# zai-org/SCAIL

Hardware: AMD Instinct MI355X
Metric: denoising-step latent tokens/sec (higher is better)
Workload: dtype bf16

## Files before the change

### include/scail_dit.h

```cpp
#ifndef SCAIL_DIT_H
#define SCAIL_DIT_H

#include "scail_hip.h"

#ifdef __cplusplus
extern "C" {
#endif

typedef struct scail_dit_config {
    int32_t hidden_size;
    int32_t num_heads;
    int32_t inner_hidden_size;
    int32_t num_layers;
    int32_t text_dim;
    int32_t clip_dim;
    int32_t time_freq_dim;
    int32_t time_embed_dim;
    float layernorm_epsilon;
} scail_dit_config;

typedef struct scail_dit_layer {
    const scail_bf16* qkv_w; const float* qkv_b;
    const scail_bf16* o_w; const float* o_b;
    const float* qn; const float* kn;
    const scail_bf16* cq_w; const float* cq_b;
    const scail_bf16* co_w; const float* co_b;
    const float* cqn;
    const float* ln_w; const float* ln_b;
    const scail_bf16* w1; const float* b1;
    const scail_bf16* w2; const float* b2;
} scail_dit_layer;

typedef struct scail_dit_weights {
    const scail_bf16* patch_w; const float* patch_b;
    const scail_bf16* pose_w; const float* pose_b;
    const scail_bf16* time0_w; const float* time0_b;
    const scail_bf16* time2_w; const float* time2_b;
    const scail_bf16* adaln_w; const float* adaln_b;
    const float* adaln_tables;
    const float* final_table;
    const scail_bf16* final_w; const float* final_b;
    const scail_dit_layer* layers;
} scail_dit_weights;

typedef struct scail_dit_cond {
    const scail_bf16* k_text;
    const scail_bf16* vt_text;
    const scail_bf16* k_clip;
    const scail_bf16* vt_clip;
    int64_t Lt, Lc, Bc;
} scail_dit_cond;

typedef struct scail_dit scail_dit;

int scail_dit_create(const scail_dit_config* cfg, const scail_dit_weights* w, scail_dit** out);
void scail_dit_destroy(scail_dit* h);

int64_t scail_dit_workspace_bytes(const scail_dit* h, int64_t B, int64_t T, int64_t H, int64_t W);

#define SCAIL_DIT_CFG_PAIR 1u
int scail_dit_step(scail_dit* h, const float* x, const float* timesteps, const scail_dit_cond* cond,
                   const scail_bf16* ref, int64_t n_ref, const scail_bf16* pose, int64_t n_pose,
                   const float* rope_cos, const float* rope_sin, float* out,
                   int64_t B, int64_t T, int64_t H, int64_t W, uint32_t flags, void* workspace, int64_t workspace_bytes, void* stream);

int64_t scail_dit_chars_workspace_bytes(const scail_dit* h, int64_t B, int64_t T, int64_t H, int64_t W, int64_t n_char);
int scail_dit_step_chars(scail_dit* h, const float* x, const float* timesteps, const scail_dit_cond* cond,
                         const scail_bf16* ref, int64_t n_ref, const scail_bf16* pose, int64_t n_pose, int64_t n_char, int64_t pose_frames,
                         const float* rope_cos, const float* rope_sin, float* out,
                         int64_t B, int64_t T, int64_t H, int64_t W, uint32_t flags, void* workspace, int64_t workspace_bytes, void* stream);

int64_t scail_dit_block_workspace_bytes(const scail_dit* h, int64_t B, int64_t Ltok);
int scail_dit_block(scail_dit* h, int64_t layer, scail_bf16* hidden, const float* mod, const scail_dit_cond* cond,
                    const float* rope_cos, const float* rope_sin, int64_t B, int64_t Ltok,
                    void* workspace, int64_t workspace_bytes, void* stream);

#define SCAIL_SP_ALLGATHER 0
#define SCAIL_SP_ULYSSES 1
#define SCAIL_SP_FWD_START 0
#define SCAIL_SP_FWD_WAIT 1
#define SCAIL_SP_BACK_START 2
#define SCAIL_SP_BACK_WAIT 3
typedef int (*scail_sp_exchange_fn)(void* user, int32_t op, int32_t layer, int32_t element, void* stream);
typedef struct scail_dit_sp {
    int32_t ranks;
    int32_t mode;
    scail_bf16* send;
    scail_bf16* recv;
    scail_bf16* ofull;
    scail_bf16* back;
    scail_sp_exchange_fn exchange;
    void* user;
    void* side_stream[2];
} scail_dit_sp;

int64_t scail_dit_sp_workspace_bytes(const scail_dit* h, int32_t mode, int32_t ranks, int64_t B, int64_t T, int64_t H, int64_t W);
int scail_dit_step_sp(scail_dit* h, const float* x, const float* timesteps, const scail_dit_cond* cond,
                      const scail_bf16* ref, int64_t n_ref, const scail_bf16* pose, int64_t n_pose,
                      const float* rope_cos, const float* rope_sin, float* out,
                      int64_t B, int64_t T, int64_t H, int64_t W, const scail_dit_sp* sp, uint32_t flags, void* workspace, int64_t workspace_bytes,
                      void* stream);

int64_t scail_dit_sp_chars_workspace_bytes(const scail_dit* h, int32_t mode, int32_t ranks, int64_t B, int64_t T, int64_t H, int64_t W,
                                           int64_t n_char);
int scail_dit_step_sp_chars(scail_dit* h, const float* x, const float* timesteps, const scail_dit_cond* cond,
                            const scail_bf16* ref, int64_t n_ref, const scail_bf16* pose, int64_t n_pose, int64_t n_char, int64_t pose_frames,
                            const float* rope_cos, const float* rope_sin, float* out,
                            int64_t B, int64_t T, int64_t H, int64_t W, const scail_dit_sp* sp, uint32_t flags, void* workspace,
                            int64_t workspace_bytes, void* stream);

int64_t scail_dit_block_sp_workspace_bytes(const scail_dit* h, int32_t mode, int32_t ranks, int64_t B, int64_t Ltok);
int scail_dit_block_sp(scail_dit* h, int64_t layer, scail_bf16* hidden, const float* mod, const scail_dit_cond* cond,
                       const float* rope_cos, const float* rope_sin, int64_t B, int64_t Ltok, const scail_dit_sp* sp,
                       void* workspace, int64_t workspace_bytes, void* stream);

#define SCAIL_DIT_PROF_SELF_ATTN 0
#define SCAIL_DIT_PROF_GEMM 1
#define SCAIL_DIT_PROF_CROSS_ATTN 2
#define SCAIL_DIT_PROF_XCH_FWD_WAIT 3
#define SCAIL_DIT_PROF_XCH_BACK_WAIT 4
#define SCAIL_DIT_PROF_ATTN_RESTARTS 5
int scail_dit_profile(scail_dit* h, int enable);
int scail_dit_profile_read(scail_dit* h, int category, double* ms_total, int64_t* launches);

#define SCAIL_DIT_FP8_QKV 1u
#define SCAIL_DIT_FP8_O 2u
#define SCAIL_DIT_FP8_CQ 4u
#define SCAIL_DIT_FP8_CO 8u
#define SCAIL_DIT_FP8_W1 16u
#define SCAIL_DIT_FP8_W2 32u
#define SCAIL_DIT_FP8_ALL 63u
int64_t scail_dit_fp8_weight_bytes(const scail_dit* h, uint32_t which);
int scail_dit_enable_fp8(scail_dit* h, uint32_t which, void* buf, int64_t bytes, void* stream);
#define SCAIL_DIT_FP8_SCALE_ROW 0
#define SCAIL_DIT_FP8_SCALE_MX 1
int64_t scail_dit_fp8_weight_bytes_scaled(const scail_dit* h, uint32_t which, int scaling);
int scail_dit_enable_fp8_scaled(scail_dit* h, uint32_t which, int scaling, void* buf, int64_t bytes, void* stream);

int scail_dit_fp8_select_layers(scail_dit* h, const uint32_t* masks);
// ... 42 lines not shown
```

### include/scail_hip.h

```cpp
#ifndef SCAIL_HIP_H
#define SCAIL_HIP_H

#include <stdint.h>

#ifdef __cplusplus
extern "C" {
#endif

typedef uint16_t scail_bf16;

const char* scail_last_error(void);
int scail_abi_version(void);

enum {
    SCAIL_EPI_BIAS = 0,
    SCAIL_EPI_GELU_TANH = 1,
    SCAIL_EPI_GELU_ERF = 2,
    SCAIL_EPI_RESID = 3
};

int scail_gemm_bf16(const scail_bf16* x, int64_t lda, const scail_bf16* w, const float* bias,
                    scail_bf16* y, int64_t ldc, int64_t M, int64_t N, int64_t K, int epilogue,
                    const scail_bf16* resid, int64_t ldr, const float* gate, int64_t gate_stride,
                    int64_t rows_per_batch, void* stream);

int scail_gemm_kernel_for(int64_t lda, int64_t ldc, int64_t ldr, int64_t M, int64_t N, int64_t K, int epilogue);
int scail_gemm_kernel_name_for(int64_t lda, int64_t ldc, int64_t ldr, int64_t M, int64_t N, int64_t K, int epilogue, int gated,
                               char* buf, int64_t len);

int scail_ln_modulate(const scail_bf16* x, int64_t ldx, scail_bf16* y, int64_t ldy,
                      const float* shift, const float* scale, int64_t mod_stride,
                      int64_t n_batch, int64_t rows_out, int64_t src_rows_per_batch,
                      int64_t src_row_offset, int64_t D, float eps, void* stream);

int scail_layernorm_affine(const scail_bf16* x, int64_t ldx, scail_bf16* y, int64_t ldy,
                           const float* w, const float* b, int64_t rows, int64_t D, float eps,
                           void* stream);

int scail_rmsnorm_rope(const scail_bf16* x, int64_t ldx, scail_bf16* y, int64_t ldy, const float* w,
                       const float* cos_tab, const float* sin_tab, int64_t rows,
                       int64_t rows_per_batch, int64_t D, int64_t head_dim, float eps, void* stream);

int scail_rmsnorm_rope_scaled(const scail_bf16* x, int64_t ldx, scail_bf16* y, int64_t ldy,
                              const float* w, const float* cos_tab, const float* sin_tab,
                              int64_t rows, int64_t rows_per_batch, int64_t D, int64_t head_dim,
                              float eps, float out_scale, void* stream);

int scail_rmsnorm_rope_slabs(const scail_bf16* x, int64_t ldx, scail_bf16* y, int64_t slab_w, int64_t slab_ld, int64_t slab_stride,
                             const float* w, const float* cos_tab, const float* sin_tab,
                             int64_t rows, int64_t rows_per_batch, int64_t D, int64_t head_dim,
                             float eps, float out_scale, void* stream);

enum {
    SCAIL_ROW_LN_MODULATE = 0,
    SCAIL_ROW_LN_AFFINE = 1,
    SCAIL_ROW_RMSNORM = 2,
    SCAIL_ROW_RMSNORM_ROPE = 3,
    SCAIL_ROW_COPY = 4
};
int scail_row_kernel_name_for(int form, int64_t n_batch, int64_t rows_out, int64_t D, int64_t head_dim, char* buf, int64_t len,
                              int64_t* workgroups);

int scail_slabs_to_rows(const scail_bf16* x, int64_t slab_w, int64_t slab_stride, scail_bf16* y, int64_t ldy,
                        int64_t rows, int64_t D, void* stream);

int scail_transpose_v(const scail_bf16* v, int64_t ldv, int64_t v_batch_stride, scail_bf16* vt,
                      int64_t n_batch, int64_t heads, int64_t head_dim, int64_t Lk, void* stream);

#define SCAIL_ATTN_Q_PRESCALED (-1.0f)
int scail_flash_attn_bf16(const scail_bf16* q, int64_t q_bs, int64_t q_rs,
                          const scail_bf16* k, int64_t k_ss, int64_t k_bs, int64_t k_rs,
                          const scail_bf16* vt, int64_t vt_ss, int64_t vt_bs,
                          scail_bf16* o, int64_t o_bs, int64_t o_rs,
                          int64_t n_batch, int64_t heads, int64_t Lq, int64_t Lk, int64_t n_seg,
                          float scale, int accumulate, void* stream);

int scail_flash_attn_kernel_for(int64_t q_rs, int64_t k_rs, int64_t o_rs, int64_t Lq, int64_t Lk, int accumulate, int prescaled);

int scail_flash_attn_kernel_name_for(int64_t q_rs, int64_t k_rs, int64_t o_rs, int64_t n_batch, int64_t heads, int64_t Lq, int64_t Lk,
                                     int accumulate, int prescaled, char* buf, int64_t len, int64_t* plan);

int scail_flash_attn_vrows_bf16(const scail_bf16* q, int64_t q_bs, int64_t q_rs,
                                const scail_bf16* k, int64_t k_bs, int64_t k_rs,
                                const scail_bf16* v, int64_t v_bs, int64_t v_rs,
                                scail_bf16* o, int64_t o_bs, int64_t o_rs,
                                int64_t n_batch, int64_t heads, int64_t Lq, int64_t Lk, float scale, void* stream);
int scail_flash_attn_vrows_for(int64_t q_rs, int64_t k_rs, int64_t v_rs, int64_t o_rs, int64_t n_batch, int64_t heads, int64_t Lq, int64_t Lk);
int scail_flash_attn_vrows_kernel_name_for(int64_t q_rs, int64_t k_rs, int64_t v_rs, int64_t o_rs, int64_t n_batch, int64_t heads, int64_t Lq,
                                           int64_t Lk, char* buf, int64_t len, int64_t* plan);

int scail_flash_attn_rows_for(int64_t n_batch, int64_t heads, int64_t Lq);

int scail_flash_attn_count_restarts(uint32_t* device_counter);

int scail_cross_attn2_kernel_for(int64_t q_rs, int64_t k1_rs, int64_t k2_rs, int64_t o_rs, int64_t Lq, int64_t Lk1, int64_t Lk2,
                                 int64_t n_batch, int64_t heads);
int scail_cross_attn2_kernel_name_for(int64_t q_rs, int64_t k1_rs, int64_t k2_rs, int64_t o_rs, int64_t Lq, int64_t Lk1, int64_t Lk2,
                                      int64_t n_batch, int64_t heads, char* buf, int64_t len, int64_t* workgroups);
int scail_cross_attn2_bf16(const scail_bf16* q, int64_t q_bs, int64_t q_rs,
                           const scail_bf16* k1, int64_t k1_bs, int64_t k1_rs, const scail_bf16* vt1, int64_t vt1_bs, int64_t Lk1,
                           const scail_bf16* k2, int64_t k2_bs, int64_t k2_rs, const scail_bf16* vt2, int64_t vt2_bs, int64_t Lk2,
                           scail_bf16* o, int64_t o_bs, int64_t o_rs,
                           int64_t n_batch, int64_t heads, int64_t Lq, float scale, void* stream);

int scail_timestep_embedding(const float* t, float* out, int64_t n, int64_t dim, void* stream);

int scail_small_linear(const float* x, const scail_bf16* w, const float* b, float* y, int64_t M,
                       int64_t N, int64_t K, int act_in, int act_out, void* stream);

int scail_adaln_table(const float* emb, const float* table, float* out, int64_t n_layers,
                      int64_t n_batch, int64_t width, void* stream);

int scail_patchify(const float* x, const scail_bf16* ref, const scail_bf16* pose, scail_bf16* tok,
                   int64_t n_batch, int64_t n_ref, int64_t n_pose, int64_t T, int64_t H, int64_t W,
                   int64_t kpad, void* stream);

int scail_patchify_chars(const float* x, const scail_bf16* ref, const scail_bf16* pose, scail_bf16* tok,
                         int64_t n_batch, int64_t n_ref, int64_t n_pose, int64_t n_char, int64_t T, int64_t H, int64_t W,
                         int64_t kpad, void* stream);

int scail_unpatchify(const scail_bf16* tok, float* out, int64_t n_batch, int64_t T, int64_t H,
                     int64_t W, void* stream);

int scail_cfg_euler(float* x, const float* v, int64_t n, float cfg_scale, float dsigma, void* stream);

int scail_tile_gather(const float* x, float* xin, const int32_t* frames, int64_t Tt, int64_t T, int64_t F, void* stream);
int scail_tile_blend_acc(float* den, const float* v, const int32_t* frames, const float* wk, int64_t Tt, int64_t T, int64_t F,
                         float cfg_scale, void* stream);
int scail_tile_finish(float* x, float* den, const float* inv_wsum, int64_t T, int64_t F, float dsigma, void* stream);



int scail_conv3d_cl(const scail_bf16* x, const scail_bf16* w, const float* bias, scail_bf16* y, int64_t ldc,
                    const scail_bf16* resid, int64_t ldr, const int32_t* geom, void* stream);

int scail_conv3d_kernel_for(const int32_t* geom, int64_t ldc, int64_t ldr, int fused_norm);
int scail_conv3d_norm_fused_for(const int32_t* geom, int64_t ldc);
int scail_conv3d_kernel_name_for(const int32_t* geom, int64_t ldc, int64_t ldr, int form, char* buf, int64_t len);

int scail_conv3d_cl_norm(const scail_bf16* x, const scail_bf16* w, const float* bias, scail_bf16* y, int64_t ldc,
                         const float* gamma, const int32_t* geom, void* stream);

int scail_conv3d_cl_resid_norm(const scail_bf16* x, const scail_bf16* w, const float* bias, scail_bf16* y, scail_bf16* y_norm, int64_t ldc,
                               const scail_bf16* resid, int64_t ldr, const float* gamma, const int32_t* geom, void* stream);

int scail_rms_silu(const scail_bf16* x, scail_bf16* y, const float* gamma, int64_t nvox, int64_t C, int silu,
                   void* stream);

int scail_softmax_rows(scail_bf16* s, int64_t ld, int64_t rows, int64_t n, float scale, void* stream);

int scail_transpose2d(const scail_bf16* in, int64_t ldi, int64_t in_bs, scail_bf16* out, int64_t ldo,
                      int64_t out_bs, int64_t R, int64_t C, int64_t batch, void* stream);

int scail_to_channels_last(const float* x, scail_bf16* y, const float* a, const float* b, int64_t C,
                           int64_t Cpad, int64_t N, void* stream);

int scail_from_channels_last(const scail_bf16* x, int64_t ldx, float* y, const float* a, const float* b,
                             int64_t C, int64_t N, float lo, float hi, void* stream);

int scail_to_channels_last_frames(const float* x, scail_bf16* y, const float* a, const float* b, int64_t C, int64_t Cpad,
                                  int64_t plane, int64_t off, int64_t N, void* stream);
int scail_from_channels_last_frames(const scail_bf16* x, int64_t ldx, float* y, const float* a, const float* b, int64_t C,
                                    int64_t plane, int64_t off, int64_t N, float lo, float hi, void* stream);

int scail_frames_u8(const scail_bf16* x, int64_t ldx, uint8_t* out, int64_t row_bytes, int64_t frame_bytes,
                    int64_t n_frames, int64_t H, int64_t W, void* stream);



int scail_attn_small(const scail_bf16* q, const scail_bf16* k, const scail_bf16* v, scail_bf16* o,
                     const int64_t* strides, int64_t n_batch, int64_t heads, int64_t Lq, int64_t Lk, int64_t head_dim,
                     float scale, const int32_t* bucket, const float* bias_tab, const int32_t* key_mask,
                     int64_t key_mask_bs, void* stream);

int scail_mul_bf16(const scail_bf16* a, const scail_bf16* b, scail_bf16* y, int64_t n, void* stream);

int scail_row_affine(const scail_bf16* x, scail_bf16* y, const float* rowscale, const scail_bf16* addrow, int64_t add_rows,
                     int64_t rows, int64_t D, void* stream);

int scail_set_option(const char* name, int value);

int scail_comm_standin(const void* src, void* dst, int64_t bytes, int32_t workgroups, int64_t min_ns, void* stream);

int scail_release_caches(void);

int scail_f32_to_bf16(const float* x, scail_bf16* y, int64_t n, void* stream);
int scail_bf16_to_f32(const scail_bf16* x, float* y, int64_t n, void* stream);
// ... 37 lines not shown
```

### scail_amd/csrc/attn.hip

```cpp
#include <algorithm>
#include <atomic>
#include <cstring>
#include "common.h"

#define HD 128
#define QBLK 256
#define KVBLK 64
#define ATT_THREADS 512
#define K_LD (HD + 8)
#define V_LD (KVBLK + 8)
#define ATT_LDS_BYTES (2 * (KVBLK * K_LD + HD * V_LD) * 2)
#define ATT_PP_LDS_BYTES (ATT_LDS_BYTES + QBLK * K_LD * 2)

struct AttnParams {
    const u16* q; int64_t q_bs, q_rs;
    const u16* k; int64_t k_ss, k_bs, k_rs;
    const u16* vt; int64_t vt_ss, vt_bs;
    u16* o; int64_t o_bs, o_rs;
    int heads, Lq, Lk, Lkp, n_seg;
    float sl2;
    int accumulate;
    int probe;
};

__device__ unsigned long long g_attn_clk[2] = {0ull, 0ull};
#ifdef SCAIL_ABLATIONS
int scail_attn_clk(unsigned long long* out2, int reset) {
    if (out2 != nullptr) {
        unsigned long long v[2];
        if (hipMemcpyFromSymbol(v, HIP_SYMBOL(g_attn_clk), 16) != hipSuccess) return 2;
        out2[0] += v[0]; out2[1] += v[1];
    }
    if (reset) {
        const unsigned long long z[2] = {0ull, 0ull};
        if (hipMemcpyToSymbol(HIP_SYMBOL(g_attn_clk), z, 16) != hipSuccess) return 2;
    }
    return 0;
}
#endif

template <int VARIANT, int NW>
__global__ __launch_bounds__(64 * NW, 2) void flash_attn_kernel(AttnParams p) {
    constexpr int NTH = 64 * NW;
    constexpr bool DMA = (VARIANT & 256) != 0;
    constexpr int KLD = DMA ? HD : K_LD, VLD = DMA ? KVBLK : V_LD;
    extern __shared__ __attribute__((aligned(16))) u16 smem[];
    u16* Ks = smem;
    u16* Vs = smem + 2 * KVBLK * KLD;

    const int tid = threadIdx.x, lane = tid & 63;
    const int wave = __builtin_amdgcn_readfirstlane(tid >> 6);
    const int ql = lane & 31, g = lane >> 5;
    const int h = blockIdx.y;
    const int64_t b = blockIdx.z;
    const int q0 = blockIdx.x * (32 * NW) + wave * 32;
    const unsigned long long clk0 = p.probe ? __builtin_amdgcn_s_memtime() : 0ull;

    bf16x8 qf[HD / 16];
    {
        const int qrow = min(q0 + ql, p.Lq - 1);
        const u16* qp = p.q + b * p.q_bs + (int64_t)qrow * p.q_rs + (int64_t)h * HD + g * 8;
#pragma unroll
        for (int ks = 0; ks < HD / 16; ++ks) qf[ks] = *reinterpret_cast<const bf16x8*>(qp + ks * 16);
    }

    constexpr int KRS = NTH / 16, VRS = NTH / 8;
    const int krow = tid >> 4, kcc = tid & 15;
    const int vrow = tid >> 3, vcc = tid & 7;
    const u16* kbase = p.k + b * p.k_bs + (int64_t)h * HD + kcc * 8;
    const u16* vbase = p.vt + b * p.vt_bs + (int64_t)h * HD * p.Lkp + vcc * 8;
    const int tps = p.Lkp / KVBLK;
    const int ntiles = tps * p.n_seg;
    uint4 kr0, kr1, kr2, kr3, vr0, vr1, vr2, vr3;
#define G_LOAD(tt_)                                                                               \
    {                                                                                             \
        const int seg_ = (tt_) / tps, t_ = (tt_) - seg_ * tps;                                    \
        const int key0_ = t_ * KVBLK;                                                             \
        const u16* kp_ = kbase + (int64_t)seg_ * p.k_ss;                                          \
        const u16* vp_ = vbase + (int64_t)seg_ * p.vt_ss + key0_;                                 \
        kr0 = *reinterpret_cast<const uint4*>(kp_ + (int64_t)min(key0_ + krow, p.Lk - 1) * p.k_rs);            \
        kr1 = *reinterpret_cast<const uint4*>(kp_ + (int64_t)min(key0_ + krow + KRS, p.Lk - 1) * p.k_rs);      \
        vr0 = *reinterpret_cast<const uint4*>(vp_ + (int64_t)vrow * p.Lkp);                       \
        vr1 = *reinterpret_cast<const uint4*>(vp_ + (int64_t)(vrow + VRS) * p.Lkp);               \
        if (NW == 4) {                                                                            \
            kr2 = *reinterpret_cast<const uint4*>(kp_ + (int64_t)min(key0_ + krow + 2 * KRS, p.Lk - 1) * p.k_rs);  \
// ... 116 lines not shown
            for (int r = 0; r < 16; ++r) {
                const float pv = __builtin_amdgcn_exp2f(s[f][r] * sl2 - msc);
                s[f][r] = pv;
                rs += pv;
            }
        l_run = l_run * alpha + rs;
        if (!(VARIANT & 2) || !__all(m_new == m_run)) {
#pragma unroll
            for (int d = 0; d < HD / 32; ++d)
#pragma unroll
                for (int e = 0; e < 16; ++e) o[d][e] *= alpha;
        }
        m_run = m_new;
        } else { l_run = 1.f; }
        bf16x8 pf[4];
#pragma unroll
        for (int ks = 0; ks < 4; ++ks) {
            uint4 u;
            const int f = ks >> 1, r0 = (ks & 1) * 8;
            u.x = pack_bf16x2(s[f][r0 + 0], s[f][r0 + 1]);
            u.y = pack_bf16x2(s[f][r0 + 2], s[f][r0 + 3]);
            u.z = pack_bf16x2(s[f][r0 + 4], s[f][r0 + 5]);
            u.w = pack_bf16x2(s[f][r0 + 6], s[f][r0 + 7]);
            pf[ks] = __builtin_bit_cast(bf16x8, u);
        }
        const u16* vs_ = Vs + (cur * HD + ql) * VLD;
        if (VARIANT & 1) __builtin_amdgcn_s_setprio(1);
#pragma unroll
        for (int ks = 0; ks < 4; ++ks) {
#pragma unroll
            for (int d = 0; d < HD / 32; ++d) {
                const bf16x8 vf = *reinterpret_cast<const bf16x8*>(vs_ + d * 32 * VLD + voff[ks]);
                o[d] = __builtin_amdgcn_mfma_f32_32x32x16_bf16(vf, pf[ks], o[d], 0, 0, 0);
            }
        }
        if (VARIANT & 1) __builtin_amdgcn_s_setprio(0);
        if (!(VARIANT & 32)) {
            if (!DMA) { if (tt + 1 < ntiles) { S_STORE(cur ^ 1) } }
            __syncthreads();
        }
    }

    const float l_tot = l_run + __shfl_xor(l_run, 32, 64);
    const float inv = 1.0f / l_tot;
    const int qrow = q0 + ql;
    if (qrow < p.Lq) {
        u16* op = p.o + b * p.o_bs + (int64_t)qrow * p.o_rs + (int64_t)h * HD + 4 * g;
#pragma unroll
        for (int d = 0; d < HD / 32; ++d) {
#pragma unroll
            for (int rr = 0; rr < 4; ++rr) {
                float v[4];
#pragma unroll
                for (int e = 0; e < 4; ++e) v[e] = o[d][4 * rr + e] * inv;
                uint2* dst = reinterpret_cast<uint2*>(op + d * 32 + rr * 8);
                if (p.accumulate) {
                    const uint2 old = *dst;
                    v[0] += bf_lo(old.x); v[1] += bf_hi(old.x);
                    v[2] += bf_lo(old.y); v[3] += bf_hi(old.y);
                }
                uint2 w;
                w.x = pack_bf16x2(v[0], v[1]);
                w.y = pack_bf16x2(v[2], v[3]);
                *dst = w;
            }
        }
    }
    if (p.probe && tid == 0) {
        atomicAdd(&g_attn_clk[0], (unsigned long long)__builtin_amdgcn_s_memtime() - clk0);
        atomicAdd(&g_attn_clk[1], 1ull);
    }
}


struct Cross2Params {
    const u16* q; int64_t q_bs, q_rs;
    const u16* k0; int64_t k0_bs, k0_rs; const u16* vt0; int64_t vt0_bs; int Lk0, Lkp0;
    const u16* k1; int64_t k1_bs, k1_rs; const u16* vt1; int64_t vt1_bs; int Lk1, Lkp1;
    u16* o; int64_t o_bs, o_rs;
    int heads, Lq;
    float sl2;
};

#define X2_THREADS 256
#define X2_LDS_BYTES (2 * (KVBLK * HD + HD * KVBLK) * 2)
__global__ __launch_bounds__(X2_THREADS, 2) void cross_attn2_kernel(Cross2Params p) {
    extern __shared__ __attribute__((aligned(16))) u16 smem[];
    u16* Ks = smem;
    u16* Vs = smem + 2 * KVBLK * HD;

    const int tid = threadIdx.x, lane = tid & 63;
    const int wave = __builtin_amdgcn_readfirstlane(tid >> 6);
    const int ql = lane & 31, g = lane >> 5;
    const int h = blockIdx.y;
    const int64_t b = blockIdx.z;
    const int q0 = blockIdx.x * 128 + wave * 32;

    bf16x8 qf[HD / 16];
    {
        const int qrow = min(q0 + ql, p.Lq - 1);
        const u16* qp = p.q + b * p.q_bs + (int64_t)qrow * p.q_rs + (int64_t)h * HD + g * 8;
#pragma unroll
        for (int ks = 0; ks < HD / 16; ++ks) qf[ks] = *reinterpret_cast<const bf16x8*>(qp + ks * 16);
    }

    const int dk_row = lane >> 4, dk_c = lane & 15, dv_row = lane >> 3, dv_c = lane & 7;
    const u16* kb0 = p.k0 + b * p.k0_bs + (int64_t)h * HD;
    const u16* kb1 = p.k1 + b * p.k1_bs + (int64_t)h * HD;
    const u16* vb0 = p.vt0 + b * p.vt0_bs + (int64_t)h * HD * p.Lkp0;
    const u16* vb1 = p.vt1 + b * p.vt1_bs + (int64_t)h * HD * p.Lkp1;
    const int n0 = p.Lkp0 / KVBLK, n1 = p.Lkp1 / KVBLK, ntiles = n0 + n1;
#define X2_ISSUE(tt_, buf_)                                                                                 \
    {                                                                                                       \
        const bool s1_ = (tt_) >= n0;                                                                       \
        const int key0_ = ((tt_) - (s1_ ? n0 : 0)) * KVBLK;                                                 \
        const u16* kp_ = s1_ ? kb1 : kb0;                                                                   \
        const int64_t krs_ = s1_ ? p.k1_rs : p.k0_rs;                                                       \
        const int last_ = (s1_ ? p.Lk1 : p.Lk0) - 1;                                                        \
        const int lkp_ = s1_ ? p.Lkp1 : p.Lkp0;                                                             \
        const u16* vp_ = (s1_ ? vb1 : vb0) + key0_;                                                         \
        _Pragma("unroll") for (int i_ = 0; i_ < 4; ++i_) {                                                  \
            const int j_ = wave * 4 + i_;                                                                   \
            const int kr_ = 4 * j_ + dk_row;                                                                \
            const u16* ks_src = kp_ + (int64_t)min(key0_ + kr_, last_) * krs_ + ((dk_c ^ (kr_ & 15)) << 3); \
            __builtin_amdgcn_global_load_lds((const __attribute__((address_space(1))) void*)ks_src,          \
                (__attribute__((address_space(3))) void*)(Ks + ((buf_) * KVBLK + 4 * j_) * HD), 16, 0, 0);   \
            const int vr_ = 8 * j_ + dv_row;                                                                \
            const u16* vs_src = vp_ + (int64_t)vr_ * lkp_ + ((dv_c ^ ((vr_ >> 1) & 7)) << 3);               \
            __builtin_amdgcn_global_load_lds((const __attribute__((address_space(1))) void*)vs_src,          \
                (__attribute__((address_space(3))) void*)(Vs + ((buf_) * HD + 8 * j_) * KVBLK), 16, 0, 0);   \
        }                                                                                                   \
    }
    int koff[HD / 16], voff[4];
#pragma unroll
    for (int ks = 0; ks < HD / 16; ++ks) koff[ks] = ((2 * ks + g) ^ (ql & 15)) << 3;
#pragma unroll
    for (int ks = 0; ks < 4; ++ks) voff[ks] = ((2 * ks + g) ^ ((ql >> 1) & 7)) << 3;

    f32x16 o[HD / 32];
#pragma unroll
    for (int d = 0; d < HD / 32; ++d)
#pragma unroll
        for (int e = 0; e < 16; ++e) o[d][e] = 0.f;
    uint2 o1[HD / 32][4];
    float m_run = -INFINITY, l_run = 0.f;
    const float sl2 = p.sl2;

    X2_ISSUE(0, 0)
    __builtin_amdgcn_s_waitcnt(0x0F70);
    __syncthreads();
    for (int tt = 0; tt < ntiles; ++tt) {
        const int cur = tt & 1;
        if (tt + 1 < ntiles) X2_ISSUE(tt + 1, cur ^ 1)
        if (tt == n0) {
            const float inv1 = 1.0f / (l_run + __shfl_xor(l_run, 32, 64));
#pragma unroll
            for (int d = 0; d < HD / 32; ++d)
#pragma unroll
                for (int rr = 0; rr < 4; ++rr) {
                    o1[d][rr].x = pack_bf16x2(o[d][4 * rr + 0] * inv1, o[d][4 * rr + 1] * inv1);
                    o1[d][rr].y = pack_bf16x2(o[d][4 * rr + 2] * inv1, o[d][4 * rr + 3] * inv1);
#pragma unroll
                    for (int e = 0; e < 4; ++e) o[d][4 * rr + e] = 0.f;
                }
            m_run = -INFINITY;
            l_run = 0.f;
        }
        f32x16 s[2];
#pragma unroll
        for (int f = 0; f < 2; ++f)
#pragma unroll
            for (int e = 0; e < 16; ++e) s[f][e] = 0.f;
        const u16* ks_ = Ks + (cur * KVBLK + ql) * HD;
#pragma unroll
        for (int ks = 0; ks < HD / 16; ++ks) {
#pragma unroll
            for (int f = 0; f < 2; ++f) {
                const bf16x8 kf = *reinterpret_cast<const bf16x8*>(ks_ + f * 32 * HD + koff[ks]);
                s[f] = __builtin_amdgcn_mfma_f32_32x32x16_bf16(kf, qf[ks], s[f], 0, 0, 0);
            }
        }
        {
            const bool s1 = tt >= n0;
            const int t = tt - (s1 ? n0 : 0), ns = s1 ? n1 : n0;
            const int tail = (s1 ? p.Lk1 : p.Lk0) - (ns - 1) * KVBLK;
            if (t == ns - 1 && tail < KVBLK) {
#pragma unroll
                for (int f = 0; f < 2; ++f)
#pragma unroll
                    for (int r = 0; r < 16; ++r) {
                        const int key = 32 * f + (r & 3) + 8 * (r >> 2) + 4 * g;
                        if (key >= tail) s[f][r] = -INFINITY;
                    }
            }
        }
        float mx = s[0][0];
#pragma unroll
        for (int f = 0; f < 2; ++f)
#pragma unroll
            for (int r = 0; r < 16; ++r) mx = fmaxf(mx, s[f][r]);
        mx = fmaxf(mx, __shfl_xor(mx, 32, 64));
        const float m_new = fmaxf(m_run, mx);
        const float alpha = __builtin_amdgcn_exp2f((m_run - m_new) * sl2);
        const float msc = m_new * sl2;
        float rs = 0.f;
#pragma unroll
        for (int f = 0; f < 2; ++f)
#pragma unroll
            for (int r = 0; r < 16; ++r) {
                const float pv = __builtin_amdgcn_exp2f(s[f][r] * sl2 - msc);
                s[f][r] = pv;
                rs += pv;
            }
        l_run = l_run * alpha + rs;
        if (!__all(m_new == m_run)) {
#pragma unroll
            for (int d = 0; d < HD / 32; ++d)
#pragma unroll
                for (int e = 0; e < 16; ++e) o[d][e] *= alpha;
        }
        m_run = m_new;
        bf16x8 pf[4];
#pragma unroll
        for (int ks = 0; ks < 4; ++ks) {
            uint4 u;
            const int f = ks >> 1, r0 = (ks & 1) * 8;
            u.x = pack_bf16x2(s[f][r0 + 0], s[f][r0 + 1]);
            u.y = pack_bf16x2(s[f][r0 + 2], s[f][r0 + 3]);
            u.z = pack_bf16x2(s[f][r0 + 4], s[f][r0 + 5]);
            u.w = pack_bf16x2(s[f][r0 + 6], s[f][r0 + 7]);
            pf[ks] = __builtin_bit_cast(bf16x8, u);
        }
        const u16* vs_ = Vs + (cur * HD + ql) * KVBLK;
#pragma unroll
        for (int ks = 0; ks < 4; ++ks) {
#pragma unroll
            for (int d = 0; d < HD / 32; ++d) {
                const bf16x8 vf = *reinterpret_cast<const bf16x8*>(vs_ + d * 32 * KVBLK + voff[ks]);
                o[d] = __builtin_amdgcn_mfma_f32_32x32x16_bf16(vf, pf[ks], o[d], 0, 0, 0);
            }
        }
        __builtin_amdgcn_s_waitcnt(0x0F70);
        __syncthreads();
    }

    const float inv = 1.0f / (l_run + __shfl_xor(l_run, 32, 64));
    const int qrow = q0 + ql;
    if (qrow < p.Lq) {
        u16* op = p.o + b * p.o_bs + (int64_t)qrow * p.o_rs + (int64_t)h * HD + 4 * g;
#pragma unroll
        for (int d = 0; d < HD / 32; ++d) {
#pragma unroll
            for (int rr = 0; rr < 4; ++rr) {
                uint2 w;
                w.x = pack_bf16x2(o[d][4 * rr + 0] * inv + bf_lo(o1[d][rr].x), o[d][4 * rr + 1] * inv + bf_hi(o1[d][rr].x));
                w.y = pack_bf16x2(o[d][4 * rr + 2] * inv + bf_lo(o1[d][rr].y), o[d][4 * rr + 3] * inv + bf_hi(o1[d][rr].y));
                *reinterpret_cast<uint2*>(op + d * 32 + rr * 8) = w;
            }
        }
    }
}

#define PP_QK(S_, slot_)                                                                          \
    {                                                                                             \
        _Pragma("unroll") for (int f = 0; f < 2; ++f)                                             \
            _Pragma("unroll") for (int e = 0; e < 16; ++e) S_[f][e] = 0.f;                        \
        const u16* ks_ = Ks + ((slot_) * KVBLK + ql) * K_LD + g * 8;                              \
        _Pragma("unroll") for (int ks = 0; ks < HD / 16; ++ks) {                                  \
            const bf16x8 qfr = *reinterpret_cast<const bf16x8*>(qs_ + ks * 16);                   \
            _Pragma("unroll") for (int f = 0; f < 2; ++f) {                                       \
                const bf16x8 kf = *reinterpret_cast<const bf16x8*>(ks_ + f * 32 * K_LD + ks * 16); \
                if (SWP_ABL & 1) {              \
                    const bf16x8 kd_ = *reinterpret_cast<const bf16x8*>(ks_ + (f ^ 1) * 32 * K_LD + ks * 16 + 8 * K_LD); \
                    asm volatile("" :: "v"(kd_));                                                 \
                }                                                                                 \
                S_[f] = __builtin_amdgcn_mfma_f32_32x32x16_bf16(kf, qfr, S_[f], 0, 0, 0);         \
            }                                                                                     \
        }                                                                                         \
    }
#define PP_PV(slot_)                                                                              \
    {                                                                                             \
        const u16* vs_ = Vs + ((slot_) * HD + ql) * V_LD + g * 8;                                 \
        _Pragma("unroll") for (int ks = 0; ks < 4; ++ks) {                                        \
            _Pragma("unroll") for (int d = 0; d < HD / 32; ++d) {                                 \
// ... 166 lines not shown
    __syncthreads();

    int t = 0;
    for (; t + 2 < ntiles; t += 2) {
        SWP_ITER(sa, sb, mxa, mxb, t, true)
        SWP_ITER(sb, sa, mxb, mxa, t + 1, true)
    }
    if (ntiles - t == 2) {
        SWP_ITER(sa, sb, mxa, mxb, t, true)
        SWP_ITER(sb, sa, mxb, mxa, t + 1, false)
    } else {
        SWP_ITER(sa, sb, mxa, mxb, t, false)
    }

    const float l_tot = l_run + __shfl_xor(l_run, 32, 64);
    const float inv = 1.0f / l_tot;
    const int qrow = q0 + ql;
    if (qrow < p.Lq) {
        u16* op = p.o + b * p.o_bs + (int64_t)qrow * p.o_rs + (int64_t)h * HD + 4 * g;
#pragma unroll
        for (int d = 0; d < HD / 32; ++d) {
#pragma unroll
            for (int rr = 0; rr < 4; ++rr) {
                float v[4];
#pragma unroll
                for (int e = 0; e < 4; ++e) v[e] = o[d][4 * rr + e] * inv;
                uint2* dst = reinterpret_cast<uint2*>(op + d * 32 + rr * 8);
                if (p.accumulate) {
                    const uint2 old = *dst;
                    v[0] += bf_lo(old.x); v[1] += bf_hi(old.x);
                    v[2] += bf_lo(old.y); v[3] += bf_hi(old.y);
                }
                uint2 w;
                w.x = pack_bf16x2(v[0], v[1]);
                w.y = pack_bf16x2(v[2], v[3]);
                *dst = w;
            }
        }
    }
    if (p.probe && tid == 0) {
        atomicAdd(&g_attn_clk[0], (unsigned long long)__builtin_amdgcn_s_memtime() - clk0);
        atomicAdd(&g_attn_clk[1], 1ull);
    }
}



static const unsigned char k_attn4_hsaco[] = {
#include "attn4_hsaco.inc"
};
static const unsigned char k_attn4v_hsaco[] = {
#include "attn4v_hsaco.inc"
};
struct Attn4Args {
    const void* q; const void* k; const void* vt; void* o;
    int64_t q_bs, q_rs, k_ss, k_bs, k_rs, vt_ss, vt_bs, o_bs, o_rs;
    int32_t heads, Lq, Lk, Lkp, n_seg;
    float sl2, thr;
    int32_t nqb;
    uint32_t magic_nqb, magic_heads;
    int32_t xcd_mode;
    int32_t items_per_xcd;
    int32_t n_items, item0;
    uint32_t* restarts;
};
static_assert(sizeof(Attn4Args) == 168, "Attn4Args must match asmgen/attn4.py KERNARG_SIZE");
static const char* const k_attn4_default = "scail_attn4_m16f";
static std::string g_attn4_name = k_attn4_default;
static std::atomic<float> g_attn4_thr_log2{8.0f};
static std::atomic<int> g_attn4_xcd{1};

int scail_attn4_preload() {
    hipFunction_t fn;
    for (const char* name : {"scail_attn4_m16f", "scail_attn4_m16f_q3", "scail_attn4_x2"})
        if (int rc = scail_module_function("attn4", k_attn4_hsaco, name, &fn)) return rc;
    for (const char* name : {"scail_attn4_m16f_vr", "scail_attn4_m16f_q3_vr"})
        if (int rc = scail_module_function("attn4v", k_attn4v_hsaco, name, &fn)) return rc;
    return scail_device_cus() > 0 ? 0 : 2;
}

static std::atomic<int> g_attn4_mode{1};
static std::atomic<int> g_attn_vrows{1};
static std::atomic<int> g_cross4{2};
constexpr int64_t k_cross4_min_tiles = 21;
static std::atomic<int> g_attn4_rows{0};
static std::atomic<int> g_attn4_cus{0};
static thread_local int g_attn4_rows_hint = 0;
static thread_local uint32_t* g_attn4_restart_ctr = nullptr;
extern "C" int scail_flash_attn_count_restarts(uint32_t* device_counter) {
    SCAIL_REQUIRE((reinterpret_cast<uintptr_t>(device_counter) & 3) == 0, "the restart counter must be 4-byte aligned");
    g_attn4_restart_ctr = device_counter;
    return 0;
}
static const double k_attn4_q3_cost = 0.79;
struct Attn4Launch {
    int rows;
    int64_t item0, n_items;
    int xcd_mode;
    int64_t grid;
};
static int attn4_plan(int64_t n_batch, int64_t heads, int64_t Lq, Attn4Launch out[2]) {
    const int64_t P = heads * n_batch, n4 = (Lq + 255) / 256, n3 = (Lq + 191) / 192, W4 = P * n4, W3 = P * n3;
    const int opt = g_attn4_rows.load(std::memory_order_relaxed);
    const int forced = opt ? opt : g_attn4_rows_hint;
    if (forced == 192) { out[0] = {192, 0, W3}; return 1; }
    if (forced == 256) { out[0] = {256, 0, W4}; return 1; }
    int64_t cus = scail_device_cus();
    if (cus <= 0) return 0;
    const int avail = g_attn4_cus.load(std::memory_order_relaxed);
    if (avail > 0 && avail < cus) cus = avail;
    auto rounds = [&](int64_t w) { return (double)((w + cus - 1) / cus); };
    double best = rounds(W4);
    out[0] = {256, 0, W4};
    int n = 1;
    if (rounds(W3) * k_attn4_q3_cost < best * 0.985) {
        best = rounds(W3) * k_attn4_q3_cost;
        out[0] = {192, 0, W3};
    }
    const double gap = 0.02;
    for (int64_t kk = W4 / cus; kk >= 1 && kk >= W4 / cus - 4; --kk) {
        const int64_t amax = kk * cus, p = amax / n4, c = (amax % n4) / 3;
        if (p >= P) continue;
        const int64_t a = p * n4 + 3 * c, i3 = p * n3 + 4 * c, b = W3 - i3;
        if (a <= 0 || b <= 0) continue;
        const double cost = rounds(a) + rounds(b) * k_attn4_q3_cost + gap;
        if (cost < best * 0.985) {
            best = cost;
            out[0] = {256, 0, a};
            out[1] = {192, i3, b};
            n = 2;
        }
    }
    return n;
}
void scail_attn4_rows_hint(int rows) { g_attn4_rows_hint = rows; }
static bool attn4_eligible(int64_t q_rs, int64_t k_rs, int64_t o_rs, int64_t Lq, int64_t Lk, int accumulate) {
    const int64_t lim = (1ll << 30);
    return Lk >= 512 && accumulate == 0 && Lq * q_rs < lim && Lk * k_rs < lim && Lq * o_rs < lim && 128 * (Lk + 63) < lim;
}
static bool attn4_allowed(int64_t n_batch, int64_t heads, int64_t Lq) {
    const int64_t nqb = (Lq + 191) / 192, lim = 1ll << 31;
    return g_attn4_mode && heads < (1 << 15) && n_batch < (1 << 15) && nqb * heads * n_batch < lim / nqb && heads * n_batch < lim / heads;
}
static std::string attn4_vrows_refusal(int64_t q_rs, int64_t k_rs, int64_t v_rs, int64_t o_rs, int64_t n_batch, int64_t heads, int64_t Lq, int64_t Lk) {
    const int64_t lim = (1ll << 30);
    auto n = [](int64_t v) { return std::to_string(v); };
    if (!g_attn_vrows) return "option attn_vrows is 0";
    if (!g_attn4_mode) return "option attn4 is 0: the 8-wave kernel reads a V^T image";
    if (g_attn4_name != k_attn4_default) return "the timing ablation " + g_attn4_name + " has no V-rows form";
    if (Lk < 512) return "Lk = " + n(Lk) + " is below the 512 keys the 4-wave kernel starts at";
    if (v_rs < heads * HD || v_rs % 8 != 0) return "v_rs = " + n(v_rs) + " must be a multiple of 8 and at least heads * 128 = " + n(heads * HD);
    if (Lk * v_rs >= lim) return "Lk * v_rs = " + n(Lk * v_rs) + " elements is beyond the 32-bit byte offsets of the kernel (2^30 elements)";
    if (Lk * k_rs >= lim) return "Lk * k_rs = " + n(Lk * k_rs) + " elements is beyond the 32-bit byte offsets of the kernel (2^30 elements)";
    if (Lq * q_rs >= lim) return "Lq * q_rs = " + n(Lq * q_rs) + " elements is beyond the 32-bit byte offsets of the kernel (2^30 elements)";
    if (Lq * o_rs >= lim) return "Lq * o_rs = " + n(Lq * o_rs) + " elements is beyond the 32-bit byte offsets of the kernel (2^30 elements)";
    if (!attn4_allowed(n_batch, heads, Lq))
        return "n_batch = " + n(n_batch) + ", heads = " + n(heads) + ", Lq = " + n(Lq) + " is beyond the kernel's workgroup-id decode";
    return "";
}

enum AttnFamily { ATTN_NONE,
                  ATTN_GEN,
                  ATTN_W8,
                  ATTN_VARIANT };
struct AttnKernel {
    int (*launch)(const char* what, int lds_max, dim3 grid, dim3 block, size_t lds, void* stream, const AttnParams& p);
// ... 68 lines not shown
    }
#ifdef SCAIL_ABLATIONS
    if (g_attn_variant != (8 | (2 << 12))) {
        c.family = ATTN_VARIANT;
        c.variant = g_attn_variant;
        for (const auto& v : k_attn_variants)
            if ((c.variant & v.mask) == v.value) { c.hip = v.k; break; }
    }
#endif
    return c;
}

static std::string attn_choice_name(const AttnChoice& c, int li) {
    if (c.family == ATTN_NONE) return "none";
    if (c.family == ATTN_GEN) return std::string(c.name) + (li >= 0 && c.launch[li].rows == 192 ? "_q3" : "") + (c.vrows ? "_vr" : "");
    return c.family == ATTN_VARIANT ? "attn_variant " + std::to_string(c.variant) + ": " + c.hip.name : c.hip.name;
}

extern "C" int scail_flash_attn_rows_for(int64_t n_batch, int64_t heads, int64_t Lq) {
    if (n_batch <= 0 || heads <= 0 || Lq <= 0) return 256;
    Attn4Launch pl[2];
    const int n = attn4_plan(n_batch, heads, Lq, pl);
    return n == 0 ? -1 : (n == 2 ? 448 : pl[0].rows);
}

extern "C" int scail_flash_attn_kernel_for(int64_t q_rs, int64_t k_rs, int64_t o_rs, int64_t Lq, int64_t Lk, int accumulate, int prescaled) {
    return attn_choose(q_rs, k_rs, o_rs, 1, 1, Lq, Lk, accumulate, prescaled != 0, false).family == ATTN_GEN ? 4 : 8;
}

static int attn_choice_report(const AttnChoice& c, int64_t n_batch, int64_t heads, int64_t Lq, char* buf, int64_t len, int64_t* plan);
extern "C" int scail_flash_attn_kernel_name_for(int64_t q_rs, int64_t k_rs, int64_t o_rs, int64_t n_batch, int64_t heads, int64_t Lq, int64_t Lk,
                                                int accumulate, int prescaled, char* buf, int64_t len, int64_t* plan) {
    SCAIL_REQUIRE(buf != nullptr, "null argument");
    SCAIL_REQUIRE(n_batch >= 1 && heads >= 1 && Lq >= 1 && Lk >= 1, "need at least one pair, one query and one key");
    return attn_choice_report(attn_choose(q_rs, k_rs, o_rs, n_batch, heads, Lq, Lk, accumulate, prescaled != 0, plan != nullptr), n_batch, heads, Lq,
                              buf, len, plan);
}

extern "C" int scail_flash_attn_vrows_for(int64_t q_rs, int64_t k_rs, int64_t v_rs, int64_t o_rs, int64_t n_batch, int64_t heads, int64_t Lq, int64_t Lk) {
    return v_rs > 0 && n_batch >= 1 && heads >= 1 && Lq >= 1 && attn_choose(q_rs, k_rs, o_rs, n_batch, heads, Lq, Lk, 0, true, false, v_rs).family == ATTN_GEN;
}

extern "C" int scail_flash_attn_vrows_kernel_name_for(int64_t q_rs, int64_t k_rs, int64_t v_rs, int64_t o_rs, int64_t n_batch, int64_t heads, int64_t Lq,
                                                      int64_t Lk, char* buf, int64_t len, int64_t* plan) {
    SCAIL_REQUIRE(buf != nullptr, "null argument");
    SCAIL_REQUIRE(n_batch >= 1 && heads >= 1 && Lq >= 1 && Lk >= 1 && v_rs >= 1, "need at least one pair, one query, one key and a row stride of v");
    return attn_choice_report(attn_choose(q_rs, k_rs, o_rs, n_batch, heads, Lq, Lk, 0, true, plan != nullptr, v_rs), n_batch, heads, Lq, buf, len, plan);
}

static int attn_choice_report(const AttnChoice& c, int64_t n_batch, int64_t heads, int64_t Lq, char* buf, int64_t len, int64_t* plan) {
    if (c.n_launch < 0) return 2;
    std::string name = attn_choice_name(c, c.n_launch > 0 ? 0 : -1);
    if (c.n_launch == 2) name += " + " + attn_choice_name(c, 1);
    SCAIL_REQUIRE((int64_t)name.size() < len, "buffer too small");
    std::memcpy(buf, name.c_str(), name.size() + 1);
    if (plan == nullptr) return 0;
    std::fill(plan, plan + 9, (int64_t)0);
    if (c.family == ATTN_NONE) return 0;
    if (c.family != ATTN_GEN) {
        const int64_t v[5] = {1, c.hip.qblk, 0, (Lq + c.hip.qblk - 1) / c.hip.qblk * heads * n_batch, 0};
        std::copy(v, v + 5, plan);
        return 0;
    }
    plan[0] = c.n_launch;
    for (int li = 0; li < c.n_launch; ++li) {
        const Attn4Launch& pl = c.launch[li];
        const int64_t v[4] = {pl.rows, pl.item0, pl.n_items, pl.xcd_mode};
        std::copy(v, v + 4, plan + 1 + 4 * li);
    }
    return 0;
}

int scail_gemm4_enable(int on);
int scail_conv4_enable(int v);
int scail_row_wave_enable(int v);
int scail_conv_direct_enable(int v);
int scail_conv4_cont_enable(int v);
int scail_conv4_resnorm_enable(int v);
int scail_conv_s2_enable(int v);
extern "C" int scail_set_option(const char* name, int value) {
    const std::string k(name ? name : "");
    if (k == "attn4") { g_attn4_mode = value != 0; return 0; }
    if (k == "attn_vrows") { g_attn_vrows = value != 0; return 0; }
    if (k == "cross4") {
        SCAIL_REQUIRE(value >= 0 && value <= 2, "cross4 must be 0, 1 or 2");
        g_cross4 = value;
        return 0;
    }
    if (k == "attn4_rows") {
        SCAIL_REQUIRE(value == 0 || value == 192 || value == 256, "attn4_rows must be 0 (automatic), 192 or 256");
        g_attn4_rows = value;
        return 0;
    }
    if (k == "attn4_xcd") {
        g_attn4_xcd = value != 0;
        return 0;
    }
    if (k == "attn4_cus") {
        SCAIL_REQUIRE(value >= 0 && value <= 4096, "attn4_cus must be in [0, 4096]");
        g_attn4_cus = value;
        return 0;
    }
    if (k == "gemm4") return scail_gemm4_enable(value);
    if (k == "conv4") return scail_conv4_enable(value);
    if (k == "row_wave") return scail_row_wave_enable(value);
    if (k == "conv_direct") return scail_conv_direct_enable(value);
    if (k == "conv4_cont") return scail_conv4_cont_enable(value);
    if (k == "conv_s2") return scail_conv_s2_enable(value);
    if (k == "conv4_resnorm") return scail_conv4_resnorm_enable(value);
    if (k == "attn4_thr") {
        SCAIL_REQUIRE(value >= 0 && value <= 64, "attn4_thr must be in [0, 64] (log2 units)");
        g_attn4_thr_log2 = (float)value;
        return 0;
    }
    scail_set_error(std::string("scail_set_option: unknown option ") + k);
    return 1;
}

#ifdef SCAIL_ABLATIONS
int scail_gemm_tune(int v);
int scail_gemm4_knob(const char* knob, int value);
int scail_gemm_group_m(int v);
int scail_conv_tune(int v);
int scail_conv4_kernel(const char* suffix);
extern "C" int scail_tune_set(const char* knob, int value) {
    if (std::string(knob) == "attn_variant") {
        if (value & (512 | 1024 | 2048)) {
            scail_set_error("scail_tune_set: attn_variant " + std::to_string(value) + " selects a removed kernel (half-tile pipelines)");
            return 1;
        }
        g_attn_variant = value;
        return 0;
    }
    if (std::string(knob) == "attn4" || std::string(knob) == "attn4_xcd") return scail_set_option(knob, value);
    if (std::string(knob) == "attn4_thr") { g_attn4_thr_log2 = (float)value; return 0; }
    if (std::string(knob).rfind("attn4_kernel", 0) == 0) {
        std::string k(knob), name = k_attn4_default;
        if (k.size() > 13) name = "scail_attn4_" + k.substr(13);
        g_attn4_name = name;
        hipFunction_t fn;
        return scail_module_function("attn4", k_attn4_hsaco, name, &fn);
    }
    if (std::string(knob).rfind("gemm4", 0) == 0) return scail_gemm4_knob(knob, value);
    if (std::string(knob) == "gemm_tile") return scail_gemm_tune(value);
    if (std::string(knob) == "conv_halo") return scail_conv_tune(value);
    if (std::string(knob).rfind("conv4_kernel", 0) == 0) return scail_conv4_kernel(std::string(knob).size() > 13 ? knob + 12 : "");
    if (std::string(knob) == "gemm_group_m") return scail_gemm_group_m(value);
    scail_set_error(std::string("scail_tune_set: unknown knob ") + knob);
    return 1;
}

#endif

static void attn4_fill(Attn4Args& a, const void* q, int64_t q_bs, int64_t q_rs, const void* k, int64_t k_ss, int64_t k_bs, int64_t k_rs,
                       const void* vt, int64_t vt_ss, int64_t vt_bs, void* o, int64_t o_bs, int64_t o_rs, int64_t heads, int64_t Lq, int64_t Lk,
                       int64_t n_seg, const Attn4Launch& pl) {
    a.q = q; a.k = k; a.vt = vt; a.o = o;
    a.q_bs = q_bs; a.q_rs = q_rs; a.k_ss = k_ss; a.k_bs = k_bs; a.k_rs = k_rs; a.vt_ss = vt_ss; a.vt_bs = vt_bs;
    a.o_bs = o_bs; a.o_rs = o_rs;
    a.heads = (int32_t)heads; a.Lq = (int32_t)Lq; a.Lk = (int32_t)Lk; a.Lkp = (int32_t)((Lk + 63) / 64 * 64); a.n_seg = (int32_t)n_seg;
    a.nqb = (int32_t)((Lq + pl.rows - 1) / pl.rows);
    a.magic_nqb = (uint32_t)(((1ull << 31) + a.nqb - 1) / a.nqb);
    a.magic_heads = (uint32_t)(((1ull << 31) + heads - 1) / heads);
    a.xcd_mode = pl.xcd_mode;
    a.n_items = (int32_t)pl.n_items;
    a.item0 = (int32_t)pl.item0;
// ... 52 lines not shown
                                     float scale, int accumulate, void* stream) {
    SCAIL_REQUIRE(Lk >= 1 && n_seg >= 1, "need at least one key");
    SCAIL_REQUIRE(q_rs % 8 == 0 && k_rs % 8 == 0 && o_rs % 4 == 0 && q_bs % 8 == 0 && k_bs % 8 == 0 &&
                      k_ss % 8 == 0 && vt_ss % 8 == 0 && o_bs % 4 == 0,
                  "strides must keep 16-byte (q,k,vt) / 8-byte (o) alignment");
    SCAIL_REQUIRE((reinterpret_cast<uintptr_t>(q) & 15) == 0 && (reinterpret_cast<uintptr_t>(k) & 15) == 0 &&
                      (reinterpret_cast<uintptr_t>(vt) & 15) == 0 && (reinterpret_cast<uintptr_t>(o) & 7) == 0,
                  "pointer alignment");
    const bool prescaled = scale == SCAIL_ATTN_Q_PRESCALED;
    SCAIL_REQUIRE(prescaled || (scale > 0.0f && scale < 3.0e38f), "scale must be a positive finite number or SCAIL_ATTN_Q_PRESCALED");
    const float sl2 = prescaled ? 1.0f : scale * 1.4426950408889634f;
    const int64_t Lkp = (Lk + 63) / 64 * 64;
    SCAIL_REQUIRE(vt_bs == 0 || vt_bs == heads * HD * Lkp, "vt batch stride must be 0 or heads*128*ceil64(Lk)");
    SCAIL_REQUIRE(Lq < (1ll << 31) && Lkp * n_seg < (1ll << 31), "sequence too long");
    if (Lq == 0 || n_batch == 0) return 0;
    const AttnChoice c = attn_choose(q_rs, k_rs, o_rs, n_batch, heads, Lq, Lk, accumulate, prescaled, true);
    if (c.family == ATTN_GEN)
        return attn4_launch(c, q, q_bs, q_rs, k, k_ss, k_bs, k_rs, vt, vt_ss, vt_bs, o, o_bs, o_rs, n_batch, heads, Lq, Lk, n_seg, prescaled ? 0.0f : sl2, stream);
    AttnParams p;
    p.q = q; p.q_bs = q_bs; p.q_rs = q_rs;
    p.k = k; p.k_ss = k_ss; p.k_bs = k_bs; p.k_rs = k_rs;
    p.vt = vt; p.vt_ss = vt_ss; p.vt_bs = vt_bs;
    p.o = o; p.o_bs = o_bs; p.o_rs = o_rs;
    p.heads = (int)heads; p.Lq = (int)Lq; p.Lk = (int)Lk; p.Lkp = (int)Lkp; p.n_seg = (int)n_seg;
    p.sl2 = sl2;
    p.accumulate = accumulate;
    p.probe = (c.variant >> 20) & 1;
    const dim3 grid((unsigned)((Lq + c.hip.qblk - 1) / c.hip.qblk), (unsigned)heads, (unsigned)n_batch);
    return c.hip.launch("flash_attn", c.hip.lds, grid, dim3(c.hip.threads), c.hip.lds, stream, p);
}

struct Attn4X2Args {
    Attn4Args base;
    const void* k2; const void* vt2;
    int64_t k2_bs, vt2_bs;
    int32_t Lk2, Lkp2, n_wgs, pad;
};
static_assert(sizeof(Attn4X2Args) == 216, "Attn4X2Args must match asmgen/attn4.py X2_KERNARG_SIZE");

struct CrossChoice {
    bool generated = false;
    const char* name = "cross_attn2_kernel";
    int64_t n_items = 0;
    int64_t grid = 0;
};

static CrossChoice cross_choose(int64_t q_rs, int64_t k1_rs, int64_t k2_rs, int64_t o_rs, int64_t Lq, int64_t Lk1, int64_t Lk2, int64_t n_batch,
                                int64_t heads, bool want_grid) {
    CrossChoice c;
    c.grid = (Lq + 127) / 128 * heads * n_batch;
    const int64_t lim = (1ll << 30);
    const int mode = g_cross4;
    const bool want = mode == 1 || (mode == 2 && (Lk1 + 63) / 64 + (Lk2 + 63) / 64 >= k_cross4_min_tiles);
    if (!(want && k1_rs == k2_rs && Lk1 >= 64 && Lk2 >= 64 && Lq * q_rs < lim && Lq * o_rs < lim && Lk1 * k1_rs < lim && Lk2 * k2_rs < lim &&
          128 * (Lk1 + 63) < lim && 128 * (Lk2 + 63) < lim && attn4_allowed(n_batch, heads, Lq)))
        return c;
    c.generated = true;
    c.name = "scail_attn4_x2";
    c.n_items = (Lq + 255) / 256 * heads * n_batch;
    c.grid = 0;
    if (!want_grid) return c;
    const int cus = scail_device_cus();
    c.grid = cus <= 0 ? -1 : std::min<int64_t>(c.n_items, cus);
    return c;
}

extern "C" int scail_cross_attn2_kernel_for(int64_t q_rs, int64_t k1_rs, int64_t k2_rs, int64_t o_rs, int64_t Lq, int64_t Lk1, int64_t Lk2,
                                            int64_t n_batch, int64_t heads) {
    return cross_choose(q_rs, k1_rs, k2_rs, o_rs, Lq, Lk1, Lk2, n_batch, heads, false).generated ? 4 : 2;
}

extern "C" int scail_cross_attn2_kernel_name_for(int64_t q_rs, int64_t k1_rs, int64_t k2_rs, int64_t o_rs, int64_t Lq, int64_t Lk1, int64_t Lk2,
                                                 int64_t n_batch, int64_t heads, char* buf, int64_t len, int64_t* workgroups) {
    SCAIL_REQUIRE(buf != nullptr, "null argument");
    SCAIL_REQUIRE(n_batch >= 1 && heads >= 1 && Lq >= 1 && Lk1 >= 1 && Lk2 >= 1, "need at least one pair, one query and one key per set");
    const CrossChoice c = cross_choose(q_rs, k1_rs, k2_rs, o_rs, Lq, Lk1, Lk2, n_batch, heads, workgroups != nullptr);
    if (c.grid < 0) return 2;
    SCAIL_REQUIRE((int64_t)std::strlen(c.name) < len, "buffer too small");
    std::strcpy(buf, c.name);
    if (workgroups != nullptr) *workgroups = c.grid;
    return 0;
}

extern "C" int scail_cross_attn2_bf16(const scail_bf16* q, int64_t q_bs, int64_t q_rs,
                                      const scail_bf16* k1, int64_t k1_bs, int64_t k1_rs, const scail_bf16* vt1, int64_t vt1_bs, int64_t Lk1,
                                      const scail_bf16* k2, int64_t k2_bs, int64_t k2_rs, const scail_bf16* vt2, int64_t vt2_bs, int64_t Lk2,
                                      scail_bf16* o, int64_t o_bs, int64_t o_rs,
                                      int64_t n_batch, int64_t heads, int64_t Lq, float scale, void* stream) {
    SCAIL_REQUIRE(Lk1 >= 1 && Lk2 >= 1 && Lk1 < (1ll << 30) && Lk2 < (1ll << 30), "cross_attn2: each key set needs at least one key");
    SCAIL_REQUIRE(heads >= 1 && heads < 65536 && n_batch < 65536 && Lq < (1ll << 31) - 256, "cross_attn2: grid limits");
    SCAIL_REQUIRE(q_rs % 8 == 0 && k1_rs % 8 == 0 && k2_rs % 8 == 0 && o_rs % 4 == 0 && q_bs % 8 == 0 && k1_bs % 8 == 0 && k2_bs % 8 == 0 &&
                      vt1_bs % 8 == 0 && vt2_bs % 8 == 0 && o_bs % 4 == 0,
                  "cross_attn2: strides must keep 16-byte (q, k, vt) / 8-byte (o) alignment");
    SCAIL_REQUIRE((reinterpret_cast<uintptr_t>(q) & 15) == 0 && (reinterpret_cast<uintptr_t>(k1) & 15) == 0 && (reinterpret_cast<uintptr_t>(k2) & 15) == 0 &&
                      (reinterpret_cast<uintptr_t>(vt1) & 15) == 0 && (reinterpret_cast<uintptr_t>(vt2) & 15) == 0 && (reinterpret_cast<uintptr_t>(o) & 7) == 0,
                  "cross_attn2: pointer alignment");
    if (n_batch == 0 || Lq == 0) return 0;
    const bool prescaled = scale == SCAIL_ATTN_Q_PRESCALED;
    SCAIL_REQUIRE(prescaled || (scale > 0.0f && scale < 3.0e38f), "cross_attn2: scale must be a positive finite number or SCAIL_ATTN_Q_PRESCALED");
    const CrossChoice c = cross_choose(q_rs, k1_rs, k2_rs, o_rs, Lq, Lk1, Lk2, n_batch, heads, true);
    if (c.generated) {
        hipFunction_t fn;
        if (int rc = scail_module_function("attn4", k_attn4_hsaco, c.name, &fn)) return rc;
        if (c.grid < 0) return 2;
        Attn4X2Args a;
        attn4_fill(a.base, q, q_bs, q_rs, k1, 0, k1_bs, k1_rs, vt1, 0, vt1_bs, o, o_bs, o_rs, heads, Lq, Lk1, 1, Attn4Launch{256, 0, c.n_items, 0, c.grid});
        a.base.sl2 = prescaled ? 0.0f : scale * 1.4426950408889634f;
        a.base.thr = g_attn4_thr_log2;
        a.base.restarts = nullptr;
        a.k2 = k2; a.vt2 = vt2; a.k2_bs = k2_bs; a.vt2_bs = vt2_bs; a.Lk2 = (int32_t)Lk2; a.Lkp2 = (int32_t)((Lk2 + 63) / 64 * 64);
        a.n_wgs = (int32_t)c.grid;
        a.pad = 0;
        return scail_module_launch("cross_attn2 (attn4_x2)", fn, (unsigned)a.n_wgs, 256, a, stream);
    }
    Cross2Params p;
    p.q = q; p.q_bs = q_bs; p.q_rs = q_rs;
    p.k0 = k1; p.k0_bs = k1_bs; p.k0_rs = k1_rs; p.vt0 = vt1; p.vt0_bs = vt1_bs; p.Lk0 = (int)Lk1; p.Lkp0 = (int)((Lk1 + KVBLK - 1) / KVBLK * KVBLK);
    p.k1 = k2; p.k1_bs = k2_bs; p.k1_rs = k2_rs; p.vt1 = vt2; p.vt1_bs = vt2_bs; p.Lk1 = (int)Lk2; p.Lkp1 = (int)((Lk2 + KVBLK - 1) / KVBLK * KVBLK);
    p.o = o; p.o_bs = o_bs; p.o_rs = o_rs;
    p.heads = (int)heads; p.Lq = (int)Lq;
    p.sl2 = prescaled ? 1.0f : scale * 1.44269504088896340736f;
    const dim3 grid((unsigned)((Lq + 127) / 128), (unsigned)heads, (unsigned)n_batch);
    return scail_launch_lds<cross_attn2_kernel>("cross_attn2", X2_LDS_BYTES, grid, dim3(X2_THREADS), X2_LDS_BYTES, stream, p);
}
```

### scail_amd/csrc/dit_step.hip

```cpp
#include <algorithm>
#include <array>
#include <cmath>
#include <vector>

#include "common.h"
int scail_attn4_preload();
void scail_attn4_rows_hint(int rows);
int scail_gemm4_preload();
#include "../../include/scail_dit.h"

constexpr int PROF_CATS = 5;
struct ProfPool {
    std::vector<hipEvent_t> ev;
    size_t used = 0;
};

struct scail_dit {
    scail_dit_config cfg;
    scail_dit_weights w;
    std::vector<scail_dit_layer> layers;
    bool prof = false;
    ProfPool pool[PROF_CATS];
    hipEvent_t sp_ev[3] = {nullptr, nullptr, nullptr};
    uint32_t* restart_ctr = nullptr;
    uint32_t fp8 = 0;
    int fp8_scaling = SCAIL_DIT_FP8_SCALE_ROW;
    struct Fp8W { const uint8_t* q; const float* s; const uint8_t* e; };
    std::vector<std::array<Fp8W, 6>> fp8w;
    std::vector<uint32_t> fp8_sel;
    double* probe_table = nullptr;
    scail_bf16 *probe_y16 = nullptr, *probe_y8 = nullptr;
    int64_t probe_rows = 0;
};

namespace {

constexpr int64_t KPAD = 128;

inline int64_t align256(int64_t n) { return (n + 255) / 256 * 256; }

struct Carve {
    int64_t off = 0;
    int64_t take(int64_t bytes) { const int64_t o = off; off += align256(bytes); return o; }
};

int64_t vt_elems(const scail_dit_config& c, int64_t B, int64_t Ltok, int sp_mode, int64_t ranks) {
    const int64_t nh = c.num_heads;
    if (sp_mode < 0) return B * nh * 128 * ((Ltok + 63) / 64 * 64);
    const int64_t Lfp = (ranks * Ltok + 63) / 64 * 64;
    return B * (sp_mode == SCAIL_SP_ULYSSES ? nh / ranks : nh) * 128 * Lfp;
}

struct TokLens {
    int64_t Lref, Lnoise, Lpose, Ltok;
};
TokLens tok_lens(int64_t C, int64_t T, int64_t H, int64_t W) {
    const int64_t hp = H / 2, wp = W / 2;
    TokLens l;
    l.Lref = C * hp * wp;
    l.Lnoise = T * hp * wp;
    l.Lpose = C * T * (H / 4) * (W / 4);
    l.Ltok = l.Lref + l.Lnoise + l.Lpose;
    return l;
}
constexpr int64_t MAX_KEYS = (1ll << 31) - 64;
int shape_fault(int64_t B, int64_t T, int64_t H, int64_t W, int64_t C, int64_t ranks) {
    if (B <= 0 || T <= 0 || H <= 0 || W <= 0 || H % 4 != 0 || W % 4 != 0 || C < 1 || C > 64 || ranks < 1) return 1;
    if (T >= (1 << 15) || H >= (1 << 15) || W >= (1 << 15)) return 2;
    return ranks * tok_lens(C, T, H, W).Ltok < MAX_KEYS ? 0 : 2;
}
bool sp_group_ok(const scail_dit_config& c, int32_t mode, int64_t ranks) {
    if (ranks < 2 || (mode != SCAIL_SP_ALLGATHER && mode != SCAIL_SP_ULYSSES)) return false;
    return mode != SCAIL_SP_ULYSSES || c.num_heads % ranks == 0;
}

int chars_check(const char* who, int64_t n_char, int64_t pose_frames, int64_t T) {
    if (n_char < 1 || n_char > 64) {
        scail_set_error(std::string(who) + ": n_char must be 1..64, got " + std::to_string(n_char));
        return 1;
    }
    if (pose_frames != n_char * T) {
        scail_set_error(std::string(who) + ": pose must hold n_char * T = " + std::to_string(n_char) + " * " + std::to_string(T) + " frames, got " +
                        std::to_string(pose_frames));
        return 1;
    }
    return 0;
}

__global__ void dup_rows_kernel(const float* __restrict__ in, float* __restrict__ out, int64_t rows, int64_t w) {
    const int64_t i = (int64_t)blockIdx.x * blockDim.x + threadIdx.x;
    if (i >= rows * w) return;
    const int64_t b = i / w, j = i - b * w;
    const float v = in[i];
    out[b * 2 * w + j] = v;
    out[b * 2 * w + w + j] = v;
}

}

#define DIT_TRY(call_)                  \
    {                                   \
        const int rc_ = (call_);        \
        if (rc_ != 0) return rc_;       \
    }

static int prof_mark(scail_dit* h, int cat, void* stream) {
    ProfPool& p = h->pool[cat];
    if (p.used == p.ev.size()) {
        hipEvent_t e;
        if (hipEventCreate(&e) != hipSuccess) {
            scail_set_error("scail_dit_profile: hipEventCreate failed");
            return 2;
        }
        p.ev.push_back(e);
    }
    if (hipEventRecord(p.ev[p.used++], (hipStream_t)stream) != hipSuccess) {
// ... 99 lines not shown
struct Ws {
    int64_t tok, h, xf, tokout, temb, e1, emb, adaln, mod, emb2, fin, total;
    BlockWs blk;
};
static Ws layout(const scail_dit* h, int64_t B, int64_t T, int64_t H, int64_t W, int64_t C, int sp_mode = -1, int64_t ranks = 1) {
    const scail_dit_config& c = h->cfg;
    const int64_t D = c.hidden_size;
    const TokLens tl = tok_lens(C, T, H, W);
    Ws s;
    Carve cv;
    s.tok = cv.take(B * tl.Ltok * KPAD * 2);
    s.h = cv.take(B * tl.Ltok * D * 2);
    s.blk = block_ws(h, B, tl.Ltok, sp_mode, ranks, cv.off);
    cv.off = s.blk.end;
    s.xf = cv.take(B * tl.Lnoise * D * 2);
    s.tokout = cv.take(B * tl.Lnoise * 64 * 2);
    s.temb = cv.take(B * c.time_freq_dim * 4);
    s.e1 = cv.take(B * c.time_embed_dim * 4);
    s.emb = cv.take(B * c.time_embed_dim * 4);
    s.adaln = cv.take(B * 6 * D * 4);
    s.mod = cv.take((int64_t)c.num_layers * B * 6 * D * 4);
    s.emb2 = cv.take(B * 2 * D * 4);
    s.fin = cv.take(B * 2 * D * 4);
    s.total = cv.off;
    return s;
}
struct SampleWs {
    int64_t xin, v, den, total;
};
static SampleWs sample_ws(int64_t step, int64_t Tv, int64_t H, int64_t W, int64_t Tden = 0) {
    const int64_t F = 16 * H * W, pair = align256(2 * Tv * F * 4);
    return {step, step + pair, step + 2 * pair, step + 2 * pair + align256(Tden * F * 4)};
}

enum { CACHE_NONE = 0 };
struct CacheWs {
    int64_t r, emb, total;
};
static CacheWs cache_ws(const scail_dit_config& c, int64_t B, int64_t Lnoise) {
    Carve cv;
    CacheWs s;
    s.r = cv.take(B * Lnoise * c.hidden_size * 2);
    s.emb = cv.take(B * Lnoise * c.hidden_size * 2);
    s.total = cv.off;
    return s;
}

static int fp8_quant_gemm(const scail_dit* h, const scail_dit::Fp8W& f, const BlockBufs& bf, const scail_bf16* x, int64_t lda, const float* bias,
                          scail_bf16* y, int64_t ldc, int64_t M, int64_t N, int64_t K, int epi, const scail_bf16* resid, int64_t ldr,
                          const float* gate, int64_t gs, int64_t rpb, void* stream) {
    if (h->fp8_scaling == SCAIL_DIT_FP8_SCALE_MX) {
        DIT_TRY(scail_quant_mxfp8_rows(x, lda, bf.xq, K, bf.ex(), K / 32, M, K, stream));
        return scail_gemm_mxfp8(bf.xq, K, bf.ex(), K / 32, f.q, f.e, bias, y, ldc, M, N, K, epi, resid, ldr, gate, gs, rpb, stream);
    }
    DIT_TRY(scail_quant_fp8_rows(x, lda, bf.xq, K, bf.sx, M, K, stream));
    return scail_gemm_fp8(bf.xq, K, bf.sx, f.q, f.s, bias, y, ldc, M, N, K, epi, resid, ldr, gate, gs, rpb, stream);
}

static int dit_gemm(scail_dit* h, int64_t i, int g, const BlockBufs& bf, const scail_bf16* x, int64_t lda, const float* bias, scail_bf16* y,
                    int64_t ldc, int64_t M, int64_t N, int64_t K, int epi, const scail_bf16* resid, int64_t ldr, const float* gate, int64_t gs,
                    int64_t rpb, void* stream) {
    const bool quantised = (h->fp8 & (1u << g)) != 0;
    if (quantised && h->probe_table != nullptr) {
        const scail_dit::Fp8W& f = h->fp8w[i][g];
        DIT_TRY(scail_gemm_bf16(x, lda, gemm_weight(h->layers[i], g), bias, h->probe_y16, N, M, N, K, SCAIL_EPI_BIAS, nullptr, 0, nullptr, 0, 0, stream));
        DIT_TRY(fp8_quant_gemm(h, f, bf, x, lda, bias, h->probe_y8, N, M, N, K, SCAIL_EPI_BIAS, nullptr, 0, nullptr, 0, 0, stream));
        DIT_TRY(scail_rel_err_rows(h->probe_y16, N, h->probe_y8, N, h->probe_table + (i * G_COUNT + g) * 4, M, N, stream));
    } else if (quantised && fp8_in_force(h, i, g)) {
        return fp8_quant_gemm(h, h->fp8w[i][g], bf, x, lda, bias, y, ldc, M, N, K, epi, resid, ldr, gate, gs, rpb, stream);
    }
    return scail_gemm_bf16(x, lda, gemm_weight(h->layers[i], g), bias, y, ldc, M, N, K, epi, resid, ldr, gate, gs, rpb, stream);
}

constexpr float ATTN_SCALE = 0.08838834764831845f;
constexpr float ATTN_LOG2_SCALE = ATTN_SCALE * 1.4426950408889634f;

static int block_attn_out(scail_dit* h, int64_t i, scail_bf16* hid, scail_bf16* att, const float* m, int64_t nb, int64_t rpb, const BlockBufs& bf,
                          void* stream) {
    const int64_t D = h->cfg.hidden_size;
    const scail_dit_layer& lw = h->layers[i];
    DIT_PROF(SCAIL_DIT_PROF_GEMM, dit_gemm(h, i, G_O, bf, att, D, lw.o_b, hid, D, nb * rpb, D, D, SCAIL_EPI_RESID, hid, D, m + 2 * D, 6 * D, rpb, stream));
    return 0;
}
static int block_cross_mlp(scail_dit* h, int64_t i, scail_bf16* hid, scail_bf16* att, scail_bf16* q3, scail_bf16* xn, scail_bf16* ff,
                           const float* m, const scail_dit_cond* cond, int64_t Btot, int64_t b0, int64_t nb, int64_t rpb, const BlockBufs& bf,
                           void* stream) {
    const scail_dit_config& c = h->cfg;
    const int64_t D = c.hidden_size, FF = c.inner_hidden_size, nh = c.num_heads;
    const float eps = c.layernorm_epsilon;
    const int64_t Ltp = (cond->Lt + 63) / 64 * 64, Lcp = (cond->Lc + 63) / 64 * 64;
    const int64_t M = nb * rpb;
    const scail_dit_layer& lw = h->layers[i];
    DIT_TRY(scail_layernorm_affine(hid, D, xn, D, lw.ln_w, lw.ln_b, M, D, eps, stream));
    DIT_PROF(SCAIL_DIT_PROF_GEMM, dit_gemm(h, i, G_CQ, bf, xn, D, lw.cq_b, q3, 3 * D, M, D, D, SCAIL_EPI_BIAS, nullptr, 0, nullptr, 0, 0, stream));
    DIT_TRY(scail_rmsnorm_rope_scaled(q3, 3 * D, q3, 3 * D, lw.cqn, nullptr, nullptr, M, M, D, 128, eps, ATTN_LOG2_SCALE, stream));
    const bool shared_clip = cond->Bc == 1;
    const scail_bf16* kt = cond->k_text + (i * Btot + b0) * cond->Lt * D;
    const scail_bf16* vtt = cond->vt_text + (i * Btot + b0) * nh * 128 * Ltp;
    const scail_bf16* kc = cond->k_clip + (i * cond->Bc + (shared_clip ? 0 : b0)) * cond->Lc * D;
    const scail_bf16* vtc = cond->vt_clip + (i * cond->Bc + (shared_clip ? 0 : b0)) * nh * 128 * Lcp;
    DIT_PROF(SCAIL_DIT_PROF_CROSS_ATTN, scail_cross_attn2_bf16(q3, rpb * 3 * D, 3 * D, kt, cond->Lt * D, D, vtt, nh * 128 * Ltp, cond->Lt,
                                                               kc, shared_clip ? 0 : cond->Lc * D, D, vtc, shared_clip ? 0 : nh * 128 * Lcp, cond->Lc,
                                                               att, rpb * D, D, nb, nh, rpb, SCAIL_ATTN_Q_PRESCALED, stream));
    DIT_PROF(SCAIL_DIT_PROF_GEMM, dit_gemm(h, i, G_CO, bf, att, D, lw.co_b, hid, D, M, D, D, SCAIL_EPI_RESID, hid, D, nullptr, 0, 0, stream));
    DIT_TRY(scail_ln_modulate(hid, D, xn, D, m + 3 * D, m + 4 * D, 6 * D, nb, rpb, rpb, 0, D, eps, stream));
    DIT_PROF(SCAIL_DIT_PROF_GEMM, dit_gemm(h, i, G_W1, bf, xn, D, lw.b1, ff, FF, M, FF, D, SCAIL_EPI_GELU_TANH, nullptr, 0, nullptr, 0, 0, stream));
    DIT_PROF(SCAIL_DIT_PROF_GEMM, dit_gemm(h, i, G_W2, bf, ff, FF, lw.b2, hid, D, M, D, FF, SCAIL_EPI_RESID, hid, D, m + 5 * D, 6 * D, rpb, stream));
    return 0;
}
static int block_tail(scail_dit* h, int64_t i, scail_bf16* hid, const float* m, const scail_dit_cond* cond, int64_t B, int64_t Ltok,
                      const BlockBufs& bf, int64_t row0, int64_t rows, bool pair, void* stream) {
    const int64_t D = h->cfg.hidden_size;
    scail_bf16 *att = bf.att, *q = bf.qkv, *xn = bf.xn, *ff = bf.ff;
    if (pair) {
        DIT_TRY(block_attn_out(h, i, hid + row0 * D, att + row0 * D, m, 1, rows, bf, stream));
        if (hipMemcpyAsync(hid + Ltok * D, hid, (size_t)Ltok * D * 2, hipMemcpyDeviceToDevice, (hipStream_t)stream) != hipSuccess) {
            scail_set_error("scail_dit (cfg pair): hipMemcpyAsync failed");
            return 2;
        }
    }
    if (rows == Ltok) {
        if (!pair) DIT_TRY(block_attn_out(h, i, hid, att, m, B, Ltok, bf, stream));
        return block_cross_mlp(h, i, hid, att, q, xn, ff, m, cond, B, 0, B, Ltok, bf, stream);
    }
    for (int64_t b = 0; b < B; ++b) {
        const int64_t r = b * Ltok + row0;
        if (!pair) DIT_TRY(block_attn_out(h, i, hid + r * D, att + r * D, m + b * 6 * D, 1, rows, bf, stream));
        DIT_TRY(block_cross_mlp(h, i, hid + r * D, att + r * D, q + r * 3 * D, xn, ff, m + b * 6 * D, cond, B, b, 1, rows, bf, stream));
    }
    return 0;
}

static int dit_block(scail_dit* h, int64_t i, scail_bf16* hid, const float* m, const scail_dit_cond* cond,
                     const float* rope_cos, const float* rope_sin, int64_t B, int64_t Ltok, const BlockBufs& bf,
                     int64_t row0, int64_t rows, bool pair, void* stream) {
    const scail_dit_config& c = h->cfg;
    const int64_t D = c.hidden_size, nh = c.num_heads;
    const float eps = c.layernorm_epsilon;
    const int64_t Lp = (Ltok + 63) / 64 * 64;
    const int64_t Bs = pair ? 1 : B;
    const int64_t M = Bs * Ltok;
    scail_bf16 *qkv = bf.qkv, *q = qkv, *k = qkv + D, *v = qkv + 2 * D;
    const scail_dit_layer& lw = h->layers[i];
    DIT_TRY(scail_ln_modulate(hid, D, bf.xn, D, m, m + D, 6 * D, Bs, Ltok, Ltok, 0, D, eps, stream));
    DIT_PROF(SCAIL_DIT_PROF_GEMM, dit_gemm(h, i, G_QKV, bf, bf.xn, D, lw.qkv_b, qkv, 3 * D, M, 3 * D, D, SCAIL_EPI_BIAS, nullptr, 0, nullptr, 0, 0, stream));
    DIT_TRY(scail_rmsnorm_rope(k, 3 * D, k, 3 * D, lw.kn, rope_cos, rope_sin, M, Ltok, D, 128, eps, stream));
    const bool vrows = scail_flash_attn_vrows_for(3 * D, 3 * D, 3 * D, D, Bs, nh, rows, Ltok) != 0;
    if (!vrows) DIT_TRY(scail_transpose_v(v, 3 * D, Ltok * 3 * D, bf.vt, Bs, nh, 128, Ltok, stream));
    DIT_TRY(scail_rmsnorm_rope_scaled(q, 3 * D, q, 3 * D, lw.qn, rope_cos, rope_sin, M, Ltok, D, 128, eps, ATTN_LOG2_SCALE, stream));
    if (vrows) {
        DIT_PROF(SCAIL_DIT_PROF_SELF_ATTN, scail_flash_attn_vrows_bf16(q + row0 * 3 * D, Ltok * 3 * D, 3 * D, k, Ltok * 3 * D, 3 * D, v, Ltok * 3 * D, 3 * D,
                                                                       bf.att + row0 * D, Ltok * D, D, Bs, nh, rows, Ltok, SCAIL_ATTN_Q_PRESCALED, stream));
        return block_tail(h, i, hid, m, cond, B, Ltok, bf, row0, rows, pair, stream);
    }
    DIT_PROF(SCAIL_DIT_PROF_SELF_ATTN, scail_flash_attn_bf16(q + row0 * 3 * D, Ltok * 3 * D, 3 * D, k, 0, Ltok * 3 * D, 3 * D, bf.vt, 0, nh * 128 * Lp,
                                                             bf.att + row0 * D, Ltok * D, D, Bs, nh, rows, Ltok, 1, SCAIL_ATTN_Q_PRESCALED, 0, stream));
    return block_tail(h, i, hid, m, cond, B, Ltok, bf, row0, rows, pair, stream);
}

static int sp_exchange(const scail_dit_sp* sp, int op, int64_t layer, int64_t b, void* stream) {
    const int rc = sp->exchange(sp->user, (int32_t)op, (int32_t)layer, (int32_t)b, stream);
    if (rc != 0) {
        scail_set_error("scail_dit (sequence parallel): the host's exchange callback failed (op " + std::to_string(op) + ", layer " +
                        std::to_string(layer) + ", element " + std::to_string(b) + ", status " + std::to_string(rc) + ")");
        return 3;
    }
    return 0;
}

static int sp_check(const scail_dit* h, const scail_dit_sp* sp) {
    SCAIL_REQUIRE(h->fp8 == 0, "fp8 GEMMs are enabled on this handle; sequence-parallel ranks run bf16 only (scail_dit_enable_fp8(h, 0, ...) first)");
    SCAIL_REQUIRE(sp != nullptr && sp->exchange != nullptr, "null sequence-parallel descriptor / exchange callback");
    SCAIL_REQUIRE(sp->ranks >= 2 && sp->ranks <= 64, "ranks must be 2..64");
    SCAIL_REQUIRE(sp->mode == SCAIL_SP_ALLGATHER || sp->mode == SCAIL_SP_ULYSSES, "unknown exchange mode");
    SCAIL_REQUIRE(sp->send != nullptr && sp->recv != nullptr, "null send / recv buffer");
    if (sp->mode == SCAIL_SP_ULYSSES) {
        SCAIL_REQUIRE(h->cfg.num_heads % sp->ranks == 0, "ulysses needs heads divisible by the group size");
        SCAIL_REQUIRE(sp->ofull != nullptr && sp->back != nullptr, "ulysses needs the ofull / back buffers");
    }
    SCAIL_REQUIRE((sp->side_stream[0] == nullptr) == (sp->side_stream[1] == nullptr), "give both side streams or none");
    return 0;
}

namespace {
struct SideJoin {
    scail_dit* h;
// ... 52 lines not shown
        }
        for (int64_t b = 0; b < B; ++b) {
            void* s = st(b);
            DIT_PROF_S(SCAIL_DIT_PROF_XCH_FWD_WAIT, s, sp_exchange(sp, SCAIL_SP_FWD_WAIT, i, b, s));
            const scail_bf16* recv = sp->recv + b * 3 * N * slab;
            scail_bf16* vt = bf.vt + b * Hn * 128 * Lfp;
            scail_bf16* of = sp->ofull + b * N * slab;
            const bool vrows = scail_flash_attn_vrows_for(3 * Dn, 3 * Dn, 3 * Dn, Dn, 1, Hn, Lf, Lf) != 0;
            if (!vrows) DIT_TRY(scail_transpose_v(recv + 2 * Dn, 3 * Dn, 0, vt, 1, Hn, 128, Lf, s));
            struct Hint { Hint(int r) { scail_attn4_rows_hint(r); } ~Hint() { scail_attn4_rows_hint(0); } } hint(side && B > 1 ? 256 : 0);
            if (vrows) {
                DIT_PROF_S(SCAIL_DIT_PROF_SELF_ATTN, s, scail_flash_attn_vrows_bf16(recv, 0, 3 * Dn, recv + Dn, 0, 3 * Dn, recv + 2 * Dn, 0, 3 * Dn, of, 0, Dn, 1, Hn,
                                                                                    Lf, Lf, SCAIL_ATTN_Q_PRESCALED, s));
            } else {
                DIT_PROF_S(SCAIL_DIT_PROF_SELF_ATTN, s, scail_flash_attn_bf16(recv, 0, 3 * Dn, recv + Dn, 0, 0, 3 * Dn, vt, 0, 0, of, 0, Dn, 1, Hn, Lf, Lf, 1,
                                                                              SCAIL_ATTN_Q_PRESCALED, 0, s));
            }
            DIT_TRY(sp_exchange(sp, SCAIL_SP_BACK_START, i, b, s));
        }
        for (int64_t b = 0; b < B; ++b) {
            void* s = st(b);
            DIT_PROF_S(SCAIL_DIT_PROF_XCH_BACK_WAIT, s, sp_exchange(sp, SCAIL_SP_BACK_WAIT, i, b, s));
            DIT_TRY(scail_slabs_to_rows(sp->back + b * N * slab, Dn, slab, bf.att + b * Ltok * D, D, Ltok, D, s));
        }
        if (sj.join() != 0) {
            scail_set_error("scail_dit (sequence parallel): joining the side streams failed");
            return 2;
        }
    } else {
        const int64_t rowsD = Ltok * D;
        for (int64_t b = 0; b < B; ++b) {
            scail_bf16* qb = qkv + b * Ltok * 3 * D;
            scail_bf16* send = sp->send + b * 2 * rowsD;
            const scail_bf16* xb = bf.xn + b * rowsD;
            DIT_PROF(SCAIL_DIT_PROF_GEMM, scail_gemm_bf16(xb, D, lw.qkv_w + D * D, lw.qkv_b + D, qb + D, 3 * D, Ltok, D, D, SCAIL_EPI_BIAS, nullptr, 0, nullptr, 0, 0, stream));
            DIT_PROF(SCAIL_DIT_PROF_GEMM, scail_gemm_bf16(xb, D, lw.qkv_w + 2 * D * D, lw.qkv_b + 2 * D, send + D, 2 * D, Ltok, D, D, SCAIL_EPI_BIAS, nullptr, 0, nullptr, 0, 0, stream));
            DIT_TRY(scail_rmsnorm_rope(qb + D, 3 * D, send, 2 * D, lw.kn, rope_cos, rope_sin, Ltok, Ltok, D, 128, eps, stream));
            DIT_TRY(sp_exchange(sp, SCAIL_SP_FWD_START, i, b, stream));
        }
        if (rows == Ltok) {
            DIT_PROF(SCAIL_DIT_PROF_GEMM, scail_gemm_bf16(bf.xn, D, lw.qkv_w, lw.qkv_b, q, 3 * D, B * Ltok, D, D, SCAIL_EPI_BIAS, nullptr, 0, nullptr, 0, 0, stream));
            DIT_TRY(scail_rmsnorm_rope_scaled(q, 3 * D, q, 3 * D, lw.qn, rope_cos, rope_sin, B * Ltok, Ltok, D, 128, eps, ATTN_LOG2_SCALE, stream));
        } else {
            for (int64_t b = 0; b < B; ++b) {
                scail_bf16* qr = q + (b * Ltok + row0) * 3 * D;
                DIT_PROF(SCAIL_DIT_PROF_GEMM, scail_gemm_bf16(bf.xn + (b * Ltok + row0) * D, D, lw.qkv_w, lw.qkv_b, qr, 3 * D, rows, D, D, SCAIL_EPI_BIAS, nullptr, 0, nullptr, 0, 0, stream));
                DIT_TRY(scail_rmsnorm_rope_scaled(qr, 3 * D, qr, 3 * D, lw.qn, rope_cos + row0 * 64, rope_sin + row0 * 64, rows, rows, D, 128, eps, ATTN_LOG2_SCALE, stream));
            }
        }
        for (int64_t b = 0; b < B; ++b) {
            DIT_PROF(SCAIL_DIT_PROF_XCH_FWD_WAIT, sp_exchange(sp, SCAIL_SP_FWD_WAIT, i, b, stream));
            const scail_bf16* recv = sp->recv + b * 2 * N * rowsD;
            scail_bf16* vt = bf.vt + b * nh * 128 * Lfp;
            if (scail_flash_attn_vrows_for(3 * D, 2 * D, 2 * D, D, 1, nh, rows, Lf) != 0) {
                DIT_PROF(SCAIL_DIT_PROF_SELF_ATTN, scail_flash_attn_vrows_bf16(q + (b * Ltok + row0) * 3 * D, 0, 3 * D, recv, 0, 2 * D, recv + D, 0, 2 * D,
                                                                               bf.att + b * rowsD + row0 * D, 0, D, 1, nh, rows, Lf, SCAIL_ATTN_Q_PRESCALED, stream));
                continue;
            }
            DIT_TRY(scail_transpose_v(recv + D, 2 * D, 0, vt, 1, nh, 128, Lf, stream));
            DIT_PROF(SCAIL_DIT_PROF_SELF_ATTN, scail_flash_attn_bf16(q + (b * Ltok + row0) * 3 * D, 0, 3 * D, recv, 0, 0, 2 * D, vt, 0, 0, bf.att + b * rowsD + row0 * D, 0, D,
                                                                     1, nh, rows, Lf, 1, SCAIL_ATTN_Q_PRESCALED, 0, stream));
        }
    }
    return block_tail(h, i, hid, m, cond, Btot, Ltok, bf, row0, rows, pair, stream);
}

extern "C" int64_t scail_dit_block_workspace_bytes(const scail_dit* h, int64_t B, int64_t Ltok) {
    if (h == nullptr || B <= 0 || Ltok <= 0) return -1;
    return block_ws(h, B, Ltok).end;
}
extern "C" int64_t scail_dit_block_sp_workspace_bytes(const scail_dit* h, int32_t mode, int32_t ranks, int64_t B, int64_t Ltok) {
    if (h == nullptr || B <= 0 || Ltok <= 0 || !sp_group_ok(h->cfg, mode, ranks)) return -1;
    return block_ws(h, B, Ltok, mode, ranks).end;
}
extern "C" int scail_dit_block_sp(scail_dit* h, int64_t layer, scail_bf16* hidden, const float* mod, const scail_dit_cond* cond,
                                  const float* rope_cos, const float* rope_sin, int64_t B, int64_t Ltok, const scail_dit_sp* sp,
                                  void* workspace, int64_t workspace_bytes, void* stream) {
    SCAIL_REQUIRE(h != nullptr && hidden != nullptr && mod != nullptr && cond != nullptr, "null argument");
    SCAIL_REQUIRE(layer >= 0 && layer < h->cfg.num_layers && B > 0 && Ltok > 0, "bad layer / shape");
    DIT_TRY(sp_check(h, sp));
    const BlockWs s = block_ws(h, B, Ltok, sp->mode, sp->ranks);
    SCAIL_REQUIRE(workspace != nullptr && workspace_bytes >= s.end && (reinterpret_cast<uintptr_t>(workspace) & 255) == 0,
                  "workspace too small or not 256-byte aligned (scail_dit_block_sp_workspace_bytes)");
    return dit_block_sp(h, layer, hidden, mod, cond, rope_cos, rope_sin, B, Ltok, s.bufs(workspace), sp, 0, Ltok, false, stream);
}
extern "C" int scail_dit_block(scail_dit* h, int64_t layer, scail_bf16* hidden, const float* mod, const scail_dit_cond* cond,
                               const float* rope_cos, const float* rope_sin, int64_t B, int64_t Ltok,
                               void* workspace, int64_t workspace_bytes, void* stream) {
    SCAIL_REQUIRE(h != nullptr && hidden != nullptr && mod != nullptr && cond != nullptr, "null argument");
    SCAIL_REQUIRE(layer >= 0 && layer < h->cfg.num_layers && B > 0 && Ltok > 0, "bad layer / shape");
    const BlockWs s = block_ws(h, B, Ltok);
    SCAIL_REQUIRE(workspace != nullptr && workspace_bytes >= s.end && (reinterpret_cast<uintptr_t>(workspace) & 255) == 0,
                  "workspace too small or not 256-byte aligned (scail_dit_block_workspace_bytes)");
    DIT_TRY(probe_check(h, B * Ltok));
    return dit_block(h, layer, hidden, mod, cond, rope_cos, rope_sin, B, Ltok, s.bufs(workspace), 0, Ltok, false, stream);
}

extern "C" int scail_dit_create(const scail_dit_config* cfg, const scail_dit_weights* w, scail_dit** out) {
    SCAIL_REQUIRE(cfg != nullptr && w != nullptr && out != nullptr, "null argument");
    SCAIL_REQUIRE(cfg->hidden_size > 0 && cfg->hidden_size % 128 == 0 && cfg->num_heads * 128 == cfg->hidden_size,
                  "hidden_size must be heads * 128");
    SCAIL_REQUIRE(cfg->num_layers > 0 && cfg->inner_hidden_size % 64 == 0 && cfg->time_embed_dim > 0 && cfg->time_freq_dim > 0,
                  "bad layer count / widths");
    SCAIL_REQUIRE(w->layers != nullptr, "weights.layers is null");
    scail_dit* h = new scail_dit;
    h->cfg = *cfg;
    h->w = *w;
    if (int rc = scail_attn4_preload()) { delete h; return rc; }
    if (int rc = scail_gemm4_preload()) { delete h; return rc; }
    h->layers.assign(w->layers, w->layers + cfg->num_layers);
    h->w.layers = h->layers.data();
    *out = h;
    return 0;
}

extern "C" void scail_dit_destroy(scail_dit* h) {
    if (h != nullptr) {
        for (ProfPool& p : h->pool)
            for (hipEvent_t e : p.ev) (void)hipEventDestroy(e);
        for (hipEvent_t e : h->sp_ev)
            if (e != nullptr) (void)hipEventDestroy(e);
        if (h->restart_ctr != nullptr) (void)hipFree(h->restart_ctr);
    }
    delete h;
}

static int64_t fp8_scale_bytes(int scaling, int64_t N, int64_t K) { return scaling == SCAIL_DIT_FP8_SCALE_MX ? N * (K / 32) : N * 4; }
static int fp8_scaling_check(const char* fn, int scaling) {
    if (scaling == SCAIL_DIT_FP8_SCALE_ROW || scaling == SCAIL_DIT_FP8_SCALE_MX) return 0;
    scail_set_error(std::string(fn) + ": unknown scaling " + std::to_string(scaling) + " (SCAIL_DIT_FP8_SCALE_ROW = 0 or SCAIL_DIT_FP8_SCALE_MX = 1)");
    return 1;
}
static int64_t fp8_weight_bytes(const scail_dit_config& c, uint32_t which, int scaling) {
    int64_t per_layer = 0;
    for (int g = 0; g < G_COUNT; ++g)
        if (which & (1u << g)) {
            int64_t N, K;
            gemm_shape(c, g, &N, &K);
            per_layer += align256(N * K) + align256(fp8_scale_bytes(scaling, N, K));
        }
    return per_layer * c.num_layers;
}
extern "C" int64_t scail_dit_fp8_weight_bytes_scaled(const scail_dit* h, uint32_t which, int scaling) {
    if (h == nullptr || (which & ~(uint32_t)SCAIL_DIT_FP8_ALL) != 0 || fp8_scaling_check("scail_dit_fp8_weight_bytes_scaled", scaling)) return -1;
    return fp8_weight_bytes(h->cfg, which, scaling);
}
extern "C" int64_t scail_dit_fp8_weight_bytes(const scail_dit* h, uint32_t which) {
    return scail_dit_fp8_weight_bytes_scaled(h, which, SCAIL_DIT_FP8_SCALE_ROW);
}
extern "C" int scail_dit_enable_fp8_scaled(scail_dit* h, uint32_t which, int scaling, void* buf, int64_t bytes, void* stream) {
    if (fp8_scaling_check("scail_dit_enable_fp8_scaled", scaling)) return 1;
    SCAIL_REQUIRE(h != nullptr, "null handle");
    SCAIL_REQUIRE((which & ~(uint32_t)SCAIL_DIT_FP8_ALL) == 0, "unknown SCAIL_DIT_FP8_* bit");
    h->fp8_sel.clear();
    probe_off(h);
    if (which == 0 || buf == nullptr) {
        h->fp8 = 0;
        h->fp8_scaling = SCAIL_DIT_FP8_SCALE_ROW;
        h->fp8w.clear();
        return 0;
    }
    for (int g = 0; g < G_COUNT; ++g)
        if (which & (1u << g)) {
            int64_t N, K;
            gemm_shape(h->cfg, g, &N, &K);
            if (N % 128 != 0 || K % 128 != 0) {
                scail_set_error("scail_dit_enable_fp8: the " + std::string(k_gemm_names[g]) + " GEMM (N x K = " + std::to_string(N) + " x " +
                                std::to_string(K) + ") is outside scail_gemm_fp8's limits (N % 128 == 0, K % 128 == 0)");
                return 1;
            }
        }
    SCAIL_REQUIRE(bytes >= fp8_weight_bytes(h->cfg, which, scaling), "buffer too small (scail_dit_fp8_weight_bytes_scaled)");
    SCAIL_REQUIRE((reinterpret_cast<uintptr_t>(buf) & 255) == 0, "buffer must be 256-byte aligned");
    h->fp8 = 0;
    h->fp8_scaling = SCAIL_DIT_FP8_SCALE_ROW;
    const bool mx = scaling == SCAIL_DIT_FP8_SCALE_MX;
    h->fp8w.assign(h->cfg.num_layers, {});
    char* p = static_cast<char*>(buf);
    for (int64_t i = 0; i < h->cfg.num_layers; ++i)
        for (int g = 0; g < G_COUNT; ++g) {
            if (!(which & (1u << g))) continue;
            int64_t N, K;
            gemm_shape(h->cfg, g, &N, &K);
            uint8_t* q = reinterpret_cast<uint8_t*>(p);
            float* sc = reinterpret_cast<float*>(p + align256(N * K));
            uint8_t* ec = reinterpret_cast<uint8_t*>(sc);
            p += align256(N * K) + align256(fp8_scale_bytes(scaling, N, K));
            if (int rc = mx ? scail_quant_mxfp8_rows(gemm_weight(h->layers[i], g), K, q, K, ec, K / 32, N, K, stream)
                            : scail_quant_fp8_rows(gemm_weight(h->layers[i], g), K, q, K, sc, N, K, stream)) {
                h->fp8w.clear();
                return rc;
            }
            h->fp8w[i][g] = {q, mx ? nullptr : sc, mx ? ec : nullptr};
        }
    h->fp8 = which;
    h->fp8_scaling = scaling;
    return 0;
}
extern "C" int scail_dit_enable_fp8(scail_dit* h, uint32_t which, void* buf, int64_t bytes, void* stream) {
    return scail_dit_enable_fp8_scaled(h, which, SCAIL_DIT_FP8_SCALE_ROW, buf, bytes, stream);
}

extern "C" int scail_dit_fp8_select_layers(scail_dit* h, const uint32_t* masks) {
    SCAIL_REQUIRE(h != nullptr, "null handle");
    if (masks == nullptr) {
        h->fp8_sel.clear();
        return 0;
// ... 49 lines not shown
        }
    }
    return 0;
}

extern "C" int scail_dit_profile_read(scail_dit* h, int category, double* ms_total, int64_t* launches) {
    SCAIL_REQUIRE(h != nullptr && ms_total != nullptr && launches != nullptr, "null argument");
    if (category == SCAIL_DIT_PROF_ATTN_RESTARTS) {
        ProfPool& pa = h->pool[SCAIL_DIT_PROF_SELF_ATTN];
        uint32_t n = 0;
        if ((pa.used >= 2 && hipEventSynchronize(pa.ev[pa.used - 1]) != hipSuccess) || h->restart_ctr == nullptr ||
            hipDeviceSynchronize() != hipSuccess || hipMemcpy(&n, h->restart_ctr, sizeof(n), hipMemcpyDeviceToHost) != hipSuccess) {
            scail_set_error("scail_dit_profile_read: reading the restart counter failed (was profiling enabled?)");
            return 2;
        }
        *ms_total = 0.0;
        *launches = (int64_t)n;
        return 0;
    }
    SCAIL_REQUIRE(category >= 0 && category < PROF_CATS, "unknown category");
    ProfPool& p = h->pool[category];
    SCAIL_REQUIRE(p.used % 2 == 0, "unbalanced event pairs (a step failed between the marks)");
    double sum = 0.0;
    for (size_t i = 0; i + 1 < p.used; i += 2) {
        if (hipEventSynchronize(p.ev[i + 1]) != hipSuccess) {
            scail_set_error("scail_dit_profile_read: hipEventSynchronize failed");
            return 2;
        }
        float ms = 0.0f;
        if (hipEventElapsedTime(&ms, p.ev[i], p.ev[i + 1]) != hipSuccess) {
            scail_set_error("scail_dit_profile_read: hipEventElapsedTime failed");
            return 2;
        }
        sum += ms;
    }
    *ms_total = sum;
    *launches = (int64_t)(p.used / 2);
    return 0;
}

extern "C" int64_t scail_dit_chars_workspace_bytes(const scail_dit* h, int64_t B, int64_t T, int64_t H, int64_t W, int64_t n_char) {
    if (h == nullptr || shape_fault(B, T, H, W, n_char, 1) != 0) return -1;
    return layout(h, B, T, H, W, n_char).total;
}
extern "C" int64_t scail_dit_workspace_bytes(const scail_dit* h, int64_t B, int64_t T, int64_t H, int64_t W) {
    return scail_dit_chars_workspace_bytes(h, B, T, H, W, 1);
}
extern "C" int64_t scail_dit_sp_chars_workspace_bytes(const scail_dit* h, int32_t mode, int32_t ranks, int64_t B, int64_t T, int64_t H, int64_t W,
                                                      int64_t n_char) {
    if (h == nullptr || !sp_group_ok(h->cfg, mode, ranks) || shape_fault(B, T, H, W, n_char, ranks) != 0) return -1;
    return layout(h, B, T, H, W, n_char, mode, ranks).total;
}
extern "C" int64_t scail_dit_sp_workspace_bytes(const scail_dit* h, int32_t mode, int32_t ranks, int64_t B, int64_t T, int64_t H, int64_t W) {
    return scail_dit_sp_chars_workspace_bytes(h, mode, ranks, B, T, H, W, 1);
}

static int dit_step_impl(scail_dit* h, const float* x, const float* timesteps, const scail_dit_cond* cond,
                         const scail_bf16* ref, int64_t n_ref, const scail_bf16* pose, int64_t n_pose, int64_t n_char, int64_t pose_frames,
                         const float* rope_cos, const float* rope_sin, float* out,
                         int64_t B, int64_t T, int64_t H, int64_t W, const scail_dit_sp* sp, uint32_t flags, void* workspace, int64_t workspace_bytes,
                         void* stream, int mode = CACHE_NONE, void* cache = nullptr) {
    DIT_TRY(chars_check("scail_dit_step", n_char, pose_frames, T));
    const bool reuse = mode == SCAIL_DIT_CACHE_REUSE;
    SCAIL_REQUIRE(h != nullptr && (cond != nullptr || reuse), "null handle / conditioning");
    SCAIL_REQUIRE((flags & ~(uint32_t)SCAIL_DIT_CFG_PAIR) == 0, "unknown step flag");
    SCAIL_REQUIRE(!(flags & SCAIL_DIT_CFG_PAIR) || (B == 2 && n_ref == 1 && n_pose == 1),
                  "SCAIL_DIT_CFG_PAIR needs B == 2 with one shared ref / pose (element 1 = element 0 except for the conditioning)");
    const int64_t ranks = sp ? sp->ranks : 1;
    const int bad_shape = shape_fault(B, T, H, W, n_char, ranks);
    SCAIL_REQUIRE(B <= 8 && bad_shape != 1, "latent batch must be 1..8, H and W multiples of 4");
    if (bad_shape != 0) {
        scail_set_error("scail_dit_step: the self-attention takes fewer than 2^31 - 64 keys, got Ltok = " + std::to_string(tok_lens(n_char, T, H, W).Ltok) +
                        " tokens x " + std::to_string(ranks) + " rank(s) (T, H, W must be below 32768)");
        return 1;
    }
    SCAIL_REQUIRE((n_ref == 1 || n_ref == B) && (n_pose == 1 || n_pose == B), "ref / pose batch must be 1 or B");
    SCAIL_REQUIRE(reuse || cond->Bc == 1 || cond->Bc == B, "clip batch must be 1 or B");
    const scail_dit_config& c = h->cfg;
    const Ws s = sp ? layout(h, B, T, H, W, n_char, sp->mode, sp->ranks) : layout(h, B, T, H, W, n_char);
    SCAIL_REQUIRE(c.time_embed_dim == c.hidden_size, "final-layer table add needs time_embed_dim == hidden_size");
    SCAIL_REQUIRE(workspace != nullptr && workspace_bytes >= s.total, "workspace too small (scail_dit_workspace_bytes)");
    SCAIL_REQUIRE((reinterpret_cast<uintptr_t>(workspace) & 255) == 0, "workspace must be 256-byte aligned");
    if (sp == nullptr && !reuse) DIT_TRY(probe_check(h, B * tok_lens(n_char, T, H, W).Ltok));

    const int64_t D = c.hidden_size, nl = c.num_layers;
    const float eps = c.layernorm_epsilon;
    const TokLens tl = tok_lens(n_char, T, H, W);
    const int64_t Lref = tl.Lref, Lnoise = tl.Lnoise, Lpose = tl.Lpose, Ltok = tl.Ltok, Lrn = Lref + Lnoise;
    char* base = static_cast<char*>(workspace);
    auto B16 = [&](int64_t off) { return reinterpret_cast<scail_bf16*>(base + off); };
    auto F32 = [&](int64_t off) { return reinterpret_cast<float*>(base + off); };
    scail_bf16 *tok = B16(s.tok), *hid = B16(s.h), *xf = B16(s.xf), *tokout = B16(s.tokout);
    float *temb = F32(s.temb), *e1 = F32(s.e1), *emb = F32(s.emb), *adaln = F32(s.adaln), *mod = F32(s.mod);
    float *emb2 = F32(s.emb2), *fin = F32(s.fin);
    const scail_dit_weights& w = h->w;

    DIT_TRY(scail_timestep_embedding(timesteps, temb, B, c.time_freq_dim, stream));
    DIT_TRY(scail_small_linear(temb, w.time0_w, w.time0_b, e1, B, c.time_embed_dim, c.time_freq_dim, 0, 1, stream));
    DIT_TRY(scail_small_linear(e1, w.time2_w, w.time2_b, emb, B, c.time_embed_dim, c.time_embed_dim, 0, 0, stream));
    DIT_TRY(scail_small_linear(emb, w.adaln_w, w.adaln_b, adaln, B, 6 * D, c.time_embed_dim, 1, 0, stream));
    DIT_TRY(scail_adaln_table(adaln, w.adaln_tables, mod, nl, B, 6 * D, stream));
    {
        const int64_t n = B * D;
        hipLaunchKernelGGL(dup_rows_kernel, dim3((unsigned)((n + 255) / 256)), dim3(256), 0, (hipStream_t)stream, emb, emb2, B, D);
        DIT_TRY(scail_check_launch("dit_step.dup_rows"));
    }
    DIT_TRY(scail_adaln_table(emb2, w.final_table, fin, 1, B, 2 * D, stream));

    const bool pair = (flags & SCAIL_DIT_CFG_PAIR) != 0 && nl > 1;
    const int64_t Be = pair ? 1 : B;
    if (n_char == 1) {
        DIT_TRY(scail_patchify(x, ref, pose, tok, Be, n_ref, n_pose, T, H, W, KPAD, stream));
    } else {
        DIT_TRY(scail_patchify_chars(x, ref, pose, tok, Be, n_ref, n_pose, n_char, T, H, W, KPAD, stream));
    }
    const CacheWs cw = cache_ws(c, B, Lnoise);
    scail_bf16* cache_r = mode == CACHE_NONE ? nullptr : reinterpret_cast<scail_bf16*>(static_cast<char*>(cache) + cw.r);
    scail_bf16* cache_emb = mode == CACHE_NONE ? nullptr : reinterpret_cast<scail_bf16*>(static_cast<char*>(cache) + cw.emb);
    scail_bf16* hid_noise = hid + Lref * D;
    if (reuse) {
        for (int64_t b = 0; b < Be; ++b)
            DIT_TRY(scail_gemm_bf16(tok + (b * Ltok + Lref) * KPAD, KPAD, w.patch_w, w.patch_b, hid_noise + b * Ltok * D, D, Lnoise, D, KPAD,
                                    SCAIL_EPI_BIAS, nullptr, 0, nullptr, 0, 0, stream));
        DIT_TRY(scail_resid_apply(hid_noise, pair ? 0 : Ltok * D, cache_r, hid_noise, Ltok * D, B, Lnoise, D, stream));
    }
    for (int64_t b = 0; b < (reuse ? 0 : Be); ++b) {
        DIT_TRY(scail_gemm_bf16(tok + b * Ltok * KPAD, KPAD, w.patch_w, w.patch_b, hid + b * Ltok * D, D, Lrn, D, KPAD,
                                SCAIL_EPI_BIAS, nullptr, 0, nullptr, 0, 0, stream));
        DIT_TRY(scail_gemm_bf16(tok + (b * Ltok + Lrn) * KPAD, KPAD, w.pose_w, w.pose_b, hid + (b * Ltok + Lrn) * D, D, Lpose, D,
                                KPAD, SCAIL_EPI_BIAS, nullptr, 0, nullptr, 0, 0, stream));
    }

    if (mode == SCAIL_DIT_CACHE_FILL)
        for (int64_t b = 0; b < Be; ++b)
            if (hipMemcpyAsync(cache_emb + b * Lnoise * D, hid_noise + b * Ltok * D, (size_t)Lnoise * D * 2, hipMemcpyDeviceToDevice, (hipStream_t)stream) !=
                hipSuccess) {
                scail_set_error("scail_dit_step_cached: hipMemcpyAsync failed");
                return 2;
            }

    const BlockBufs bf = s.blk.bufs(workspace);
    for (int64_t i = 0; i < (reuse ? 0 : nl); ++i) {
        const bool last = i == nl - 1;
        const int64_t row0 = last ? Lref : 0, rows = last ? Lnoise : Ltok;
        if (sp != nullptr) {
            DIT_TRY(dit_block_sp(h, i, hid, mod + i * B * 6 * D, cond, rope_cos, rope_sin, B, Ltok, bf, sp, row0, rows, pair && i == 0, stream));
        } else {
            DIT_TRY(dit_block(h, i, hid, mod + i * B * 6 * D, cond, rope_cos, rope_sin, B, Ltok, bf, row0, rows, pair && i == 0, stream));
        }
    }

    if (mode == SCAIL_DIT_CACHE_FILL) DIT_TRY(scail_resid_store(hid_noise, Ltok * D, cache_emb, pair ? 0 : Lnoise * D, cache_r, B, Lnoise, D, stream));

    DIT_TRY(scail_ln_modulate(hid, D, xf, D, fin, fin + D, 2 * D, B, Lnoise, Ltok, Lref, D, eps, stream));
    DIT_TRY(scail_gemm_bf16(xf, D, w.final_w, w.final_b, tokout, 64, B * Lnoise, 64, D, SCAIL_EPI_BIAS, nullptr, 0, nullptr, 0, 0, stream));
    DIT_TRY(scail_unpatchify(tokout, out, B, T, H, W, stream));
    return 0;
}

extern "C" int scail_dit_step_chars(scail_dit* h, const float* x, const float* timesteps, const scail_dit_cond* cond,
                                    const scail_bf16* ref, int64_t n_ref, const scail_bf16* pose, int64_t n_pose, int64_t n_char, int64_t pose_frames,
                                    const float* rope_cos, const float* rope_sin, float* out,
                                    int64_t B, int64_t T, int64_t H, int64_t W, uint32_t flags, void* workspace, int64_t workspace_bytes,
                                    void* stream) {
    return dit_step_impl(h, x, timesteps, cond, ref, n_ref, pose, n_pose, n_char, pose_frames, rope_cos, rope_sin, out, B, T, H, W, nullptr, flags,
                         workspace, workspace_bytes, stream);
// ... 272 lines not shown
```

### scail_amd/csrc/rowops.hip

```cpp
#include "common.h"
#include <algorithm>
#include <atomic>
#include <cstring>

#define ROW_THREADS 256
#define ROW_MAXV 3

template <int MODE>
__global__ __launch_bounds__(ROW_THREADS) void ln_kernel(
    const u16* __restrict__ x, int64_t ldx, u16* __restrict__ y, int64_t ldy,
    const float* __restrict__ p0, const float* __restrict__ p1, int64_t mod_stride,
    int64_t rows_out, int64_t src_rows_per_batch, int64_t src_row_offset, int D, float eps) {
    __shared__ float red[4];
    const int64_t r = blockIdx.x;
    const int64_t b = r / rows_out;
    const int64_t i = r - b * rows_out;
    const u16* xr = x + (b * src_rows_per_batch + src_row_offset + i) * ldx;
    u16* yr = y + r * ldy;
    const int nvec = D >> 3;
    float v[ROW_MAXV][8];
    float s = 0.f;
#pragma unroll
    for (int j = 0; j < ROW_MAXV; ++j) {
        const int c = threadIdx.x + j * ROW_THREADS;
// ... 970 lines not shown
    double d = 0.0, m = 0.0;
    for (int64_t j = t; j < n; j += 256) {
        const double bj = (double)b[j];
        d += fabs((double)a[j] - bj);
        m += fabs(bj);
    }
    sd[t] = d;
    sb[t] = m;
    __syncthreads();
    for (int s = 128; s > 0; s >>= 1) {
        if (t < s) {
            sd[t] += sd[t + s];
            sb[t] += sb[t + s];
        }
        __syncthreads();
    }
    if (t == 0) {
        out[0] = sd[0];
        out[1] = sb[0];
    }
}

static int resid_check(const char* who, int64_t n_batch, int64_t rows, int64_t D, int64_t bs0, const char* bs0_name, int64_t bs1,
                       const char* bs1_name, const void* p0, const void* p1, const void* p2) {
    auto fail = [&](const std::string& msg) {
        scail_set_error(std::string(who) + ": " + msg);
        return 1;
    };
    if (n_batch < 0 || n_batch > 64) return fail("n_batch must be 0..64, got " + std::to_string(n_batch));
    if (rows < 0 || rows >= (1ll << 31)) return fail("rows must be 0 .. 2^31 - 1, got " + std::to_string(rows));
    if (D < 8 || D % 8 != 0 || D >= (1 << 20)) return fail("D must be a multiple of 8 in 8 .. 2^20 - 8 (16-byte loads), got " + std::to_string(D));
    if (bs0 < 0 || bs0 % 8 != 0) return fail(std::string(bs0_name) + " must be a non-negative multiple of 8 elements, got " + std::to_string(bs0));
    if (bs1 < 0 || bs1 % 8 != 0) return fail(std::string(bs1_name) + " must be a non-negative multiple of 8 elements, got " + std::to_string(bs1));
    if (n_batch == 0 || rows == 0) return 0;
    if (p0 == nullptr || p1 == nullptr || p2 == nullptr) return fail("null pointer");
    if (!aligned16(p0) || !aligned16(p1) || !aligned16(p2)) return fail("every base pointer must be 16-byte aligned");
    return 0;
}

extern "C" int scail_resid_store(const scail_bf16* h_out, int64_t out_bs, const scail_bf16* h_in, int64_t in_bs, scail_bf16* r,
                                 int64_t n_batch, int64_t rows, int64_t D, void* stream) {
    if (int rc = resid_check("scail_resid_store", n_batch, rows, D, out_bs, "out_bs", in_bs, "in_bs", h_out, h_in, r)) return rc;
    if (n_batch == 0 || rows == 0) return 0;
    const int64_t per_b8 = rows * (D / 8), total8 = n_batch * per_b8;
    const int64_t wgs = std::min<int64_t>((total8 + 255) / 256, RESID_MAX_WGS);
    hipLaunchKernelGGL(resid_store_kernel, dim3((unsigned)wgs), dim3(256), 0, (hipStream_t)stream, h_out, out_bs, h_in, in_bs, r, per_b8, total8);
    return scail_check_launch("resid_store");
}

extern "C" int scail_resid_apply(const scail_bf16* h_in, int64_t in_bs, const scail_bf16* r, scail_bf16* h, int64_t h_bs,
                                 int64_t n_batch, int64_t rows, int64_t D, void* stream) {
    if (int rc = resid_check("scail_resid_apply", n_batch, rows, D, h_bs, "h_bs", in_bs, "in_bs", h_in, r, h)) return rc;
    if (n_batch == 0 || rows == 0) return 0;
    const int64_t span = rows * D, per_b8 = rows * (D / 8);
    if (n_batch > 1 && h_bs < span) {
        scail_set_error("scail_resid_apply: h_bs = " + std::to_string(h_bs) + " is smaller than one element's rows * D = " + std::to_string(span) +
                        " (the output elements would overlap)");
        return 1;
    }
    const int64_t in_lo = (int64_t)reinterpret_cast<uintptr_t>(h_in), in_hi = in_lo + ((n_batch - 1) * in_bs + span) * 2;
    const int64_t h_lo = (int64_t)reinterpret_cast<uintptr_t>(h), h_hi = h_lo + ((n_batch - 1) * h_bs + span) * 2;
    if (in_lo < h_hi && h_lo < in_hi && !(h == h_in && (in_bs == 0 || in_bs == h_bs))) {
        scail_set_error("scail_resid_apply: h overlaps h_in without being h_in (h - h_in = " + std::to_string((h_lo - in_lo) / 2) + " elements, in_bs " +
                        std::to_string(in_bs) + ", h_bs " + std::to_string(h_bs) + "): in place means h == h_in with in_bs == 0 or in_bs == h_bs");
        return 1;
    }
    const int64_t wgs = std::min<int64_t>((per_b8 + 255) / 256, RESID_MAX_WGS);
    hipLaunchKernelGGL(resid_apply_kernel, dim3((unsigned)wgs), dim3(256), 0, (hipStream_t)stream, h_in, in_bs, r, h, h_bs, n_batch, per_b8);
    return scail_check_launch("resid_apply");
}

extern "C" int scail_abs_diff_sums(const float* a, const float* b, int64_t n, double* out, void* stream) {
    if (n < 0 || n >= (1ll << 31)) {
        scail_set_error("scail_abs_diff_sums: n must be 0 .. 2^31 - 1, got " + std::to_string(n));
        return 1;
    }
    SCAIL_REQUIRE(out != nullptr && (reinterpret_cast<uintptr_t>(out) & 7) == 0, "out must be an 8-byte aligned device pointer");
    SCAIL_REQUIRE(n == 0 || (a != nullptr && b != nullptr), "null pointer");
    SCAIL_REQUIRE(((reinterpret_cast<uintptr_t>(a) | reinterpret_cast<uintptr_t>(b)) & 3) == 0, "a and b must be 4-byte aligned");
    hipLaunchKernelGGL(abs_diff_sums_kernel, dim3(1), dim3(256), 0, (hipStream_t)stream, a, b, n, out);
    return scail_check_launch("abs_diff_sums");
}

#define SA_ROWS 32
__global__ __launch_bounds__(256) void attn_small_kernel(
    const u16* __restrict__ q, const u16* __restrict__ k, const u16* __restrict__ v, u16* __restrict__ o,
    int64_t q_bs, int64_t q_rs, int64_t k_bs, int64_t k_rs, int64_t v_bs, int64_t v_rs, int64_t o_bs, int64_t o_rs,
    int Lq, int Lk, int hd, float scale, const int* __restrict__ bucket, const float* __restrict__ bias_tab, int n_heads_tab,
    const int* __restrict__ kmask, int64_t kmask_bs) {
    extern __shared__ __attribute__((aligned(16))) unsigned char sm_raw[];
    const int ldk = hd + 8;
    u16* Ks = reinterpret_cast<u16*>(sm_raw);
    u16* Vs = Ks + (size_t)Lk * ldk;
    float* Ps = reinterpret_cast<float*>(Vs + (size_t)Lk * hd);
    float* Qs = Ps + 4 * Lk;
    const int h = blockIdx.y;
    const int64_t b = blockIdx.z;
    const int tid = threadIdx.x, lane = tid & 63, wave = tid >> 6;
    const int cpr = hd >> 3;
    for (int c = tid; c < Lk * cpr; c += 256) {
        const int j = c / cpr, cc = c - j * cpr;
        *reinterpret_cast<uint4*>(Ks + j * ldk + cc * 8) = *reinterpret_cast<const uint4*>(k + b * k_bs + (int64_t)j * k_rs + h * hd + cc * 8);
        *reinterpret_cast<uint4*>(Vs + j * hd + cc * 8) = *reinterpret_cast<const uint4*>(v + b * v_bs + (int64_t)j * v_rs + h * hd + cc * 8);
    }
    __syncthreads();
    float* P = Ps + wave * Lk;
    float* Q = Qs + wave * hd;
    const int i0 = blockIdx.x * SA_ROWS;
    for (int ii = wave; ii < SA_ROWS; ii += 4) {
        const int i = i0 + ii;
        if (i >= Lq) break;
        for (int d = lane; d < hd; d += 64) Q[d] = bf2f(q[b * q_bs + (int64_t)i * q_rs + h * hd + d]) * scale;
        __builtin_amdgcn_s_waitcnt(0xC07F);
        float mx = -INFINITY;
        for (int j = lane; j < Lk; j += 64) {
            float s = 0.f;
            for (int c = 0; c < cpr; ++c) {
                float kf[8];
                unpack8(*reinterpret_cast<const uint4*>(Ks + j * ldk + c * 8), kf);
#pragma unroll
                for (int e = 0; e < 8; ++e) s += Q[c * 8 + e] * kf[e];
            }
            if (bias_tab != nullptr) s += bias_tab[bucket[(int64_t)i * Lk + j] * n_heads_tab + h];
            if (kmask != nullptr && kmask[b * kmask_bs + j] == 0) s = -INFINITY;
            P[j] = s;
            mx = fmaxf(mx, s);
        }
#pragma unroll
        for (int of = 32; of > 0; of >>= 1) mx = fmaxf(mx, __shfl_xor(mx, of, 64));
        float sum = 0.f;
        for (int j = lane; j < Lk; j += 64) {
            const float pv = __expf(P[j] - mx);
            P[j] = pv;
            sum += pv;
        }
        sum = wave_sum(sum);
        __builtin_amdgcn_s_waitcnt(0xC07F);
        const float inv = 1.0f / sum;
        for (int d = lane; d < hd; d += 64) {
            float acc = 0.f;
            for (int j = 0; j < Lk; ++j) acc += P[j] * bf2f(Vs[j * hd + d]);
            o[b * o_bs + (int64_t)i * o_rs + h * hd + d] = f2bf(acc * inv);
        }
    }
}

__global__ void mul_bf16_kernel(const u16* __restrict__ a, const u16* __restrict__ b, u16* __restrict__ y, int64_t n8) {
    const int64_t i = (int64_t)blockIdx.x * blockDim.x + threadIdx.x;
    if (i >= n8) return;
    float fa[8], fb[8], fo[8];
    unpack8(*reinterpret_cast<const uint4*>(a + i * 8), fa);
    unpack8(*reinterpret_cast<const uint4*>(b + i * 8), fb);
#pragma unroll
    for (int e = 0; e < 8; ++e) fo[e] = fa[e] * fb[e];
    *reinterpret_cast<uint4*>(y + i * 8) = pack8(fo);
}

__global__ void row_affine_kernel(const u16* __restrict__ x, u16* __restrict__ y, const float* __restrict__ rowscale,
                                  const u16* __restrict__ addrow, int64_t add_rows, int64_t rows, int D8) {
    const int64_t i = (int64_t)blockIdx.x * blockDim.x + threadIdx.x;
    if (i >= rows * D8) return;
    const int64_t r = i / D8;
    const int c = (int)(i - r * D8);
    float f[8], a[8];
    unpack8(*reinterpret_cast<const uint4*>(x + i * 8), f);
    const float s = rowscale ? rowscale[r] : 1.f;
// ... 52 lines not shown
```

### scail_amd/cstep.py

```python
from __future__ import annotations

import ctypes as C
from typing import Dict

import torch

from . import lib as L

_p, _i64 = C.c_void_p, C.c_int64


class DitConfig(C.Structure):
    _fields_ = [("hidden_size", C.c_int32), ("num_heads", C.c_int32), ("inner_hidden_size", C.c_int32),
                ("num_layers", C.c_int32), ("text_dim", C.c_int32), ("clip_dim", C.c_int32),
                ("time_freq_dim", C.c_int32), ("time_embed_dim", C.c_int32), ("layernorm_epsilon", C.c_float)]


_LAYER_FIELDS = ["qkv_w", "qkv_b", "o_w", "o_b", "qn", "kn", "cq_w", "cq_b", "co_w", "co_b", "cqn", "ln_w", "ln_b",
                 "w1", "b1", "w2", "b2"]


class DitLayer(C.Structure):
    _fields_ = [(n, _p) for n in _LAYER_FIELDS]

# ... 42 lines not shown
                       W["adaln_tables"].data_ptr(), W["final_table"].data_ptr(), W["final_w"].data_ptr(),
                       W["final_b"].data_ptr(), layers)
        h = _p()
        L.call("scail_dit_create", C.byref(cfg), C.byref(w), C.byref(h))
        self._h = h
        self._ws = None
        self._cache = None
        self._fp8_buf = None
        self._probe = None
        self.num_layers = net.num_layers
        self.fp8_scaling = getattr(net, "fp8_scaling", "row")
        if getattr(net, "fp8_mask", 0):
            self.enable_fp8(net.fp8_mask, W["patch_w"].device)
            if getattr(net, "fp8_layer_masks", None) is not None:
                self.select_fp8_layers(net.fp8_layer_masks)

    def enable_fp8(self, which: int, device, scaling=None) -> None:
        lib = L.load()
        scaling = self.fp8_scaling if scaling is None else scaling
        if scaling not in L.FP8_SCALINGS:
            raise L.ScailHipError(f"enable_fp8: scaling must be one of {sorted(L.FP8_SCALINGS)}, got {scaling!r}")
        sc = L.FP8_SCALINGS[scaling]
        self._probe = None
        if not which:
            L.call("scail_dit_enable_fp8", self._h, 0, None, 0, torch.cuda.current_stream(device).cuda_stream)
            self._fp8_buf = None
            return
        nbytes = lib.scail_dit_fp8_weight_bytes_scaled(self._h, which, sc)
        if nbytes < 0:
            raise L.ScailHipError(f"scail_dit_fp8_weight_bytes_scaled: bad mask {which}")
        buf = torch.empty(nbytes, device=device, dtype=torch.uint8)
        L.call("scail_dit_enable_fp8_scaled", self._h, which, sc, buf.data_ptr(), nbytes, torch.cuda.current_stream(device).cuda_stream)
        self._fp8_buf = buf
        self.fp8_scaling = scaling

    def select_fp8_layers(self, masks) -> None:
        if masks is None:
            L.call("scail_dit_fp8_select_layers", self._h, None)
            return
        masks = [int(m) for m in masks]
        if len(masks) != self.num_layers:
            raise L.ScailHipError(f"select_fp8_layers: need one mask per layer ({self.num_layers}), got {len(masks)}")
        if any(m < 0 or m > 0xffffffff for m in masks):
            raise L.ScailHipError(f"select_fp8_layers: masks must be unsigned 32-bit values, got {masks}")
        L.call("scail_dit_fp8_select_layers", self._h, (C.c_uint32 * len(masks))(*masks))

    def fp8_probe_on(self, B: int, Ltok: int, device) -> torch.Tensor:
        need = L.load().scail_dit_fp8_probe_bytes(self._h, B, Ltok)
        if need < 0:
            raise L.ScailHipError(f"scail_dit_fp8_probe_bytes: bad shape (B {B}, Ltok {Ltok})")
        table = torch.zeros(self.num_layers, 6, 4, device=device, dtype=torch.float64)
        scratch = torch.empty(max(need, 256), device=device, dtype=torch.uint8)
        L.call("scail_dit_fp8_probe", self._h, table.data_ptr(), scratch.data_ptr(), scratch.numel())
        self._probe = (table, scratch)
        return table

    def fp8_probe_off(self) -> None:
        L.call("scail_dit_fp8_probe", self._h, None, None, 0)
        self._probe = None

    def close(self):
        if self._h is not None:
            L.load().scail_dit_destroy(self._h)
            self._h = None

    def __del__(self):
        try:
            self.close()
        except Exception:
            pass

    PROF_SELF_ATTN, PROF_GEMM, PROF_CROSS_ATTN = 0, 1, 2
    PROF_XCH_FWD_WAIT, PROF_XCH_BACK_WAIT = 3, 4
    PROF_ATTN_RESTARTS = 5

    def profile(self, enable: bool) -> None:
        L.call("scail_dit_profile", self._h, 1 if enable else 0)

    def profile_read(self, category: int):
        ms, n = C.c_double(0.0), C.c_int64(0)
        L.call("scail_dit_profile_read", self._h, category, C.byref(ms), C.byref(n))
        return ms.value, n.value

    def _ws_for(self, need: int, device, what: str) -> torch.Tensor:
        if need < 0:
            raise L.ScailHipError(f"{what}: the executor has no workspace for this request (bad shape / mode)")
        if self._ws is None or self._ws.numel() < need or self._ws.device != device:
            self._ws = torch.empty(need, device=device, dtype=torch.uint8)
        return self._ws

    @staticmethod
    def _schedule(sigmas, device):
        sig = sigmas.float().cpu()
        n = sig.numel() - 1
        ts = (sig[:-1] * 1000.0).repeat_interleave(2).to(device).contiguous()
        return ts, (C.c_float * n)(*[float(v) for v in (sig[1:] - sig[:-1])]), n

    def workspace_bytes(self, B, T, H, W, n_char: int = 1) -> int:
        n = L.load().scail_dit_chars_workspace_bytes(self._h, B, T, H, W, n_char)
        if n < 0:
            raise L.ScailHipError(f"scail_dit_chars_workspace_bytes: bad shape (B {B}, T {T}, H {H}, W {W}, n_char {n_char})")
        return n

    CFG_PAIR = 1

    def step(self, x32, t32, cond: Dict, ref, pose, cos, sin, cfg_pair: bool = False, n_char: int = 1) -> torch.Tensor:
        B, T, _, H, W = x32.shape
        ws = self._ws_for(self.workspace_bytes(B, T, H, W, n_char), x32.device, "scail_dit_chars_workspace_bytes")
        cc = _cond_struct(cond)
        out = torch.empty(B, T, 16, H, W, device=x32.device, dtype=torch.float32)
        L.call("scail_dit_step_chars", self._h, x32.data_ptr(), t32.data_ptr(), C.byref(cc), ref.data_ptr(), ref.shape[0],
               pose.data_ptr(), pose.shape[0], n_char, pose.shape[1], cos.data_ptr(), sin.data_ptr(), out.data_ptr(), B, T, H, W,
               self.CFG_PAIR if cfg_pair else 0, ws.data_ptr(), ws.numel(), torch.cuda.current_stream().cuda_stream)
        return out

    def sample(self, x32, sigmas, cfg_scale, cond: Dict, ref, pose, cos, sin, n_char: int = 1) -> torch.Tensor:
        _, T, _, H, W = x32.shape
        ws = self._ws_for(L.load().scail_dit_sample_chars_workspace_bytes(self._h, T, H, W, n_char), x32.device,
                          f"scail_dit_sample_chars_workspace_bytes (T {T}, H {H}, W {W}, n_char {n_char})")
        ts, dsa, n = self._schedule(sigmas, x32.device)
        cc = _cond_struct(cond)
        assert x32.is_contiguous() and x32.dtype == torch.float32 and ref.shape[0] == 1 and pose.shape[0] == 1
        L.call("scail_dit_sample_chars", self._h, x32.data_ptr(), ts.data_ptr(), C.cast(dsa, C.c_void_p), n, float(cfg_scale),
               C.byref(cc), ref.data_ptr(), pose.data_ptr(), n_char, pose.shape[1], cos.data_ptr(), sin.data_ptr(), T, H, W,
               ws.data_ptr(), ws.numel(), torch.cuda.current_stream().cuda_stream)
        return x32

    def step_cache_bytes(self, B, T, H, W) -> int:
        n = L.load().scail_dit_step_cache_bytes(self._h, B, T, H, W)
        if n < 0:
            raise L.ScailHipError(f"scail_dit_step_cache_bytes: bad shape (B {B}, T {T}, H {H}, W {W})")
        return n

    def _cache_for(self, B, T, H, W, device, fill: bool) -> torch.Tensor:
        key = (B, T, H, W, torch.device(device))
        if self._cache is None or self._cache[0] != key:
            if not fill:
                raise L.ScailHipError(f"step cache: a 'reuse' evaluation of (B {B}, T {T}, H {H}, W {W}) needs a 'fill' evaluation of that shape first")
            ws, self._ws = self._ws, None
            try:
                buf = self._ws_for(self.step_cache_bytes(B, T, H, W), device, f"scail_dit_step_cache_bytes (B {B}, T {T}, H {H}, W {W})")
            finally:
                self._ws = ws
            self._cache = (key, buf)
        return self._cache[1]

    def step_cache_residual(self, B, T, H, W, D) -> torch.Tensor:
        assert self._cache is not None and self._cache[0][:4] == (B, T, H, W), "no cache of this shape"
        n = B * T * (H // 2) * (W // 2) * D
        return self._cache[1][:2 * n].view(torch.bfloat16).view(B, -1, D)

    def step_cached(self, x32, t32, cond, ref, pose, cos, sin, mode: str, cfg_pair: bool = False, n_char: int = 1) -> torch.Tensor:
        if mode not in L.CACHE_MODES:
            raise L.ScailHipError(f"step_cached: mode must be one of {sorted(L.CACHE_MODES)}, got {mode!r}")
        B, T, _, H, W = x32.shape
        cache = self._cache_for(B, T, H, W, x32.device, mode == "fill")
        ws = self._ws_for(self.workspace_bytes(B, T, H, W, n_char), x32.device, "scail_dit_chars_workspace_bytes")
        cc = None if cond is None else _cond_struct(cond)
        out = torch.empty(B, T, 16, H, W, device=x32.device, dtype=torch.float32)
        L.call("scail_dit_step_cached", self._h, x32.data_ptr(), t32.data_ptr(), None if cc is None else C.byref(cc), ref.data_ptr(), ref.shape[0],
               pose.data_ptr(), pose.shape[0], n_char, pose.shape[1], cos.data_ptr(), sin.data_ptr(), out.data_ptr(), B, T, H, W,
               self.CFG_PAIR if cfg_pair else 0, ws.data_ptr(), ws.numel(), L.CACHE_MODES[mode], cache.data_ptr(), cache.numel(),
               torch.cuda.current_stream().cuda_stream)
        return out

    def sample_cached(self, x32, sigmas, cfg_scale, cond: Dict, ref, pose, cos, sin, reuse, n_char: int = 1) -> torch.Tensor:
# ... 100 lines not shown
```

### scail_amd/dit.py

```python
from __future__ import annotations

import os

import math
from functools import reduce
from operator import mul
from typing import Dict, Optional

import torch
from torch import nn

from . import lib as L
from . import ops, rope

_STR2DTYPE = {"fp32": torch.float32, "fp16": torch.float16, "bf16": torch.bfloat16}


def _get(args, name, default=None):
    if args is None:
        return default
    if isinstance(args, dict):
        return args.get(name, default)
    return getattr(args, name, default)

# ... 491 lines not shown
        self.fp8_probe_table = table.cpu()
        return fp8_rel_err(self.fp8_probe_table)

    def _check_chars(self, n_char, T, pose_frames):
        if pose_frames != n_char * T:
            raise L.ScailHipError(f"concat_smpl_render needs {n_char} x {T} frames for {n_char} reference frame(s), got {pose_frames}")

    def _sample_prelude(self, x32, ctx, clip, cond_key, T_rope, n_char):
        dev = x32.device
        cond = self._conditioning(_as_bf16(ctx, dev), _as_bf16(clip, dev), cond_key)
        cos, sin = self._rope(T_rope, x32.shape[3] // 2, x32.shape[4] // 2, 0, 0, dev, n_char)
        return self._executor(), cond, cos, sin, x32.float().contiguous().clone()

    def sample_c(self, x32, sigmas, cfg_scale, ctx, ref, pose, clip, cond_key=None, reuse=None):
        T, n_char, dev = x32.shape[1], ref.shape[1], x32.device
        self._check_chars(n_char, T, pose.shape[1])
        if reuse is not None:
            self._step_cache_ok()
        ex, cond, cos, sin, x = self._sample_prelude(x32, ctx, clip, cond_key, T, n_char)
        if reuse is not None:
            return ex.sample_cached(x, sigmas, cfg_scale, cond, _as_bf16(ref, dev), _as_bf16(pose, dev), cos, sin, reuse, n_char=n_char)
        return ex.sample(x, sigmas, cfg_scale, cond, _as_bf16(ref, dev), _as_bf16(pose, dev), cos, sin, n_char=n_char)

    def sample_tiled_c(self, x32, sigmas, cfg_scale, ctx, ref, pose_tiles, clip, tile_indices, tile_w, inv_wsum, cond_key=None):
        dev, Tt = x32.device, len(tile_indices[0])
        if ref.shape[1] != 1:
            raise L.ScailHipError(f"temporal tiles take one reference frame (tiles and several characters are not combined), got {ref.shape[1]}")
        if pose_tiles.dim() != 6 or pose_tiles.shape[1] != len(tile_indices) or pose_tiles.shape[2] != Tt:
            raise L.ScailHipError(f"smpl_tiled must be (1, n_tiles = {len(tile_indices)}, Tt = {Tt}, 16, H/2, W/2), got "
                                  f"{tuple(pose_tiles.shape)}")
        ex, cond, cos, sin, x = self._sample_prelude(x32, ctx, clip, cond_key, Tt, 1)
        return ex.sample_tiled(x, sigmas, cfg_scale, cond, _as_bf16(ref, dev), _as_bf16(pose_tiles, dev), tile_indices, tile_w, inv_wsum, cos, sin)

    def _run(self, x32, t32, ctx, ref, pose, clip, H_shift=0, W_shift=0, cond_key=None, cfg_pair=False, step_cache=None):
        if step_cache is not None:
            self._step_cache_ok()
        W = self.prepare()
        dev = x32.device
        B, T, _, H, Wd = x32.shape
        D, nh, eps = self.hidden_size, self.num_attention_heads, self.layernorm_epsilon
        hp, wp = H // 2, Wd // 2
        n_char = ref.shape[1]
        self._check_chars(n_char, T, pose.shape[1])
        Lref1, Lnoise, Lpose1 = hp * wp, T * hp * wp, T * (H // 4) * (Wd // 4)
        Lref, Lpose = n_char * Lref1, n_char * Lpose1
        Ltok = Lref + Lnoise + Lpose
        if ctx.shape[0] != B:
            raise L.ScailHipError("context batch must equal the (CFG-doubled) input batch")
        cond = self._conditioning(ctx, clip, cond_key)
        cos, sin = self._rope(T, hp, wp, H_shift, W_shift, dev, n_char)
        sp = self.sp if (self.sp is not None and self.sp.size > 1) else None
        use_c = self.executor_ok()
        if self.fp8_mask and (sp is not None or not use_c):
            raise NotImplementedError("gemm_precision='fp8' runs in the C executor on a single rank only: not on sequence-parallel ranks, "
                                      "not on the per-op path (SCAIL_C_STEP=0, _tap, kernel_timer)")
        ex = self._executor() if use_c else None
        xch = sp.c_exchange(nh, D, B, Ltok, dev) if (use_c and sp is not None) else None
        if use_c and not self._c_blocks:
            if step_cache is not None:
                return ex.step_cached(x32, t32, cond, ref.contiguous(), pose.contiguous(), cos, sin, step_cache, cfg_pair=cfg_pair, n_char=n_char)
            if sp is None:
                return ex.step(x32, t32, cond, ref.contiguous(), pose.contiguous(), cos, sin, cfg_pair=cfg_pair, n_char=n_char)
            return ex.step_sp(x32, t32, cond, ref.contiguous(), pose.contiguous(), cos, sin, xch, cfg_pair=cfg_pair, n_char=n_char)
        ws = self._workspace(B, Ltok, Lnoise, dev, blocks_in_c=use_c)

        temb = ops.timestep_embedding(t32, self.time_freq_dim)
        e1 = ops.small_linear(temb, W["time_embed.0.w"], W["time_embed.0.b"], act_out=L.ACT_SILU)
        emb = ops.small_linear(e1, W["time_embed.2.w"], W["time_embed.2.b"])
        adaln = ops.small_linear(emb, W["adaln_projection.1.w"], W["adaln_projection.1.b"], act_in=L.ACT_SILU)
        mod = ops.adaln_table(adaln, W["adaln_tables"])
        fin = ops.adaln_table(emb.repeat(1, 2).contiguous(), W["final_table"])[0]

        tok = ops.patchify(x32, ref.contiguous(), pose.contiguous(), kpad=128, out=ws["tok"], n_char=n_char)
        h = ws["h"]
        Lrn = Lref + Lnoise
        for b in range(B):
            ops.gemm(tok[b, :Lrn], W["patch_w"], W["patch_b"], out=h[b, :Lrn])
            ops.gemm(tok[b, Lrn:], W["pose_w"], W["pose_b"], out=h[b, Lrn:])
        if self._tap is not None:
            self._tap(-1, h)

        xn, qkv, att, ff, vt = ws["xn"], ws["qkv"], ws["att"], ws["ff"], ws["vt"]
        q, k, v = (None, None, None) if use_c else (qkv[..., :D], qkv[..., D:2 * D], qkv[..., 2 * D:])
        for i, lw in enumerate(W["layers"]):
            m = mod[i]
            if use_c:
                if sp is None:
                    ex.block(i, h, m, cond, cos, sin)
                else:
                    ex.block_sp(i, h, m, cond, cos, sin, xch)
                continue
            sh_a, sc_a, g_a = m[:, 0:D], m[:, D:2 * D], m[:, 2 * D:3 * D]
            sh_m, sc_m, g_m = m[:, 3 * D:4 * D], m[:, 4 * D:5 * D], m[:, 5 * D:6 * D]
            ops.ln_modulate(h, sh_a, sc_a, out=xn, eps=eps)
            if sp is None:
                ops.gemm(xn, lw["qkv_w"], lw["qkv_b"], out=qkv)
                ops.rmsnorm_rope(k, lw["kn"], cos, sin, rows_per_batch=Ltok, eps=eps)
                ops.transpose_v(v, nh, out=vt)
                ops.rmsnorm_rope(q, lw["qn"], cos, sin, rows_per_batch=Ltok, eps=eps, out_scale=ops.ATTN_LOG2_SCALE)
                self._timed("self_attn", ops.flash_attn, q, k, vt, out=att, q_prescaled=True)
            else:
                sp.self_attention(self, lw, xn, qkv, vt, cos, sin, att, Ltok, eps)
            ops.gemm(att, lw["o_w"], lw["o_b"], out=h, epilogue=L.EPI_RESID, resid=h, gate=g_a, rows_per_batch=Ltok)
            ops.layernorm_affine(h, lw["ln_w"], lw["ln_b"], out=xn, eps=eps)
            cq = qkv[..., :D]
            ops.gemm(xn, lw["cq_w"], lw["cq_b"], out=cq)
            ops.rmsnorm_rope(cq, lw["cqn"], eps=eps, out_scale=ops.ATTN_LOG2_SCALE)
            ops.cross_attn2(cq, cond["k_text"][i], cond["vt_text"][i], cond["k_clip"][i], cond["vt_clip"][i], out=att, q_prescaled=True)
            ops.gemm(att, lw["co_w"], lw["co_b"], out=h, epilogue=L.EPI_RESID, resid=h)
            ops.ln_modulate(h, sh_m, sc_m, out=xn, eps=eps)
            ops.gemm(xn, lw["w1"], lw["b1"], out=ff, epilogue=L.EPI_GELU_TANH)
            ops.gemm(ff, lw["w2"], lw["b2"], out=h, epilogue=L.EPI_RESID, resid=h, gate=g_m, rows_per_batch=Ltok)
            if self._tap is not None:
                self._tap(i, h)

        ops.ln_modulate(h, fin[:, :D], fin[:, D:], out=ws["xf"], eps=eps, rows_out=Lnoise, src_row_offset=Lref)
        ops.gemm(ws["xf"], W["final_w"], W["final_b"], out=ws["tokout"])
        return ops.unpatchify(ws["tokout"], T, H, Wd)
```

### scail_amd/lib.py

```python
from __future__ import annotations

import ctypes as C
import os

_HERE = os.path.dirname(os.path.abspath(__file__))
LIB_PATH = os.path.join(_HERE, "libscail_hip_abl.so" if os.environ.get("SCAIL_ABLATIONS", "0") not in ("", "0") else "libscail_hip.so")

_p = C.c_void_p
_i64 = C.c_int64
_i = C.c_int
_f = C.c_float

SIGNATURES = {
    "scail_gemm_bf16": [_p, _i64, _p, _p, _p, _i64, _i64, _i64, _i64, _i, _p, _i64, _p, _i64, _i64, _p],
    "scail_ln_modulate": [_p, _i64, _p, _i64, _p, _p, _i64, _i64, _i64, _i64, _i64, _i64, _f, _p],
    "scail_layernorm_affine": [_p, _i64, _p, _i64, _p, _p, _i64, _i64, _f, _p],
    "scail_rmsnorm_rope": [_p, _i64, _p, _i64, _p, _p, _p, _i64, _i64, _i64, _i64, _f, _p],
    "scail_rmsnorm_rope_scaled": [_p, _i64, _p, _i64, _p, _p, _p, _i64, _i64, _i64, _i64, _f, _f, _p],
    "scail_rmsnorm_rope_slabs": [_p, _i64, _p, _i64, _i64, _i64, _p, _p, _p, _i64, _i64, _i64, _i64, _f, _f, _p],
    "scail_row_kernel_name_for": [_i, _i64, _i64, _i64, _i64, _p, _i64, _p],
    "scail_slabs_to_rows": [_p, _i64, _i64, _p, _i64, _i64, _i64, _p],
    "scail_transpose_v": [_p, _i64, _i64, _p, _i64, _i64, _i64, _i64, _p],
    "scail_flash_attn_bf16": [_p, _i64, _i64, _p, _i64, _i64, _i64, _p, _i64, _i64, _p, _i64, _i64,
                              _i64, _i64, _i64, _i64, _i64, _f, _i, _p],
    "scail_flash_attn_kernel_for": [_i64, _i64, _i64, _i64, _i64, _i, _i],
    "scail_flash_attn_kernel_name_for": [_i64, _i64, _i64, _i64, _i64, _i64, _i64, _i, _i, _p, _i64, _p],
    "scail_flash_attn_vrows_bf16": [_p, _i64, _i64, _p, _i64, _i64, _p, _i64, _i64, _p, _i64, _i64, _i64, _i64, _i64, _i64, _f, _p],
    "scail_flash_attn_vrows_for": [_i64, _i64, _i64, _i64, _i64, _i64, _i64, _i64],
    "scail_flash_attn_vrows_kernel_name_for": [_i64, _i64, _i64, _i64, _i64, _i64, _i64, _i64, _p, _i64, _p],
    "scail_flash_attn_rows_for": [_i64, _i64, _i64],
    "scail_flash_attn_count_restarts": [_p],
    "scail_comm_standin": [_p, _p, _i64, C.c_int32, _i64, _p],
    "scail_cross_attn2_kernel_for": [_i64, _i64, _i64, _i64, _i64, _i64, _i64, _i64, _i64],
    "scail_cross_attn2_kernel_name_for": [_i64, _i64, _i64, _i64, _i64, _i64, _i64, _i64, _i64, _p, _i64, _p],
    "scail_gemm_kernel_for": [_i64, _i64, _i64, _i64, _i64, _i64, _i],
    "scail_gemm_kernel_name_for": [_i64, _i64, _i64, _i64, _i64, _i64, _i, _i, _p, _i64],
    "scail_conv3d_kernel_for": [_p, _i64, _i64, _i],
    "scail_conv3d_norm_fused_for": [_p, _i64],
    "scail_conv3d_kernel_name_for": [_p, _i64, _i64, _i, _p, _i64],
    "scail_cross_attn2_bf16": [_p, _i64, _i64, _p, _i64, _i64, _p, _i64, _i64, _p, _i64, _i64, _p, _i64, _i64, _p, _i64, _i64,
                               _i64, _i64, _i64, _f, _p],
    "scail_timestep_embedding": [_p, _p, _i64, _i64, _p],
    "scail_small_linear": [_p, _p, _p, _p, _i64, _i64, _i64, _i, _i, _p],
    "scail_adaln_table": [_p, _p, _p, _i64, _i64, _i64, _p],
    "scail_patchify": [_p, _p, _p, _p, _i64, _i64, _i64, _i64, _i64, _i64, _i64, _p],
    "scail_patchify_chars": [_p, _p, _p, _p, _i64, _i64, _i64, _i64, _i64, _i64, _i64, _i64, _p],
    "scail_unpatchify": [_p, _p, _i64, _i64, _i64, _i64, _p],
    "scail_cfg_euler": [_p, _p, _i64, _f, _f, _p],
    "scail_tile_gather": [_p, _p, _p, _i64, _i64, _i64, _p],
    "scail_tile_blend_acc": [_p, _p, _p, _p, _i64, _i64, _i64, _f, _p],
    "scail_tile_finish": [_p, _p, _p, _i64, _i64, _f, _p],
    "scail_conv3d_cl": [_p, _p, _p, _p, _i64, _p, _i64, _p, _p],
    "scail_conv3d_cl_norm": [_p, _p, _p, _p, _i64, _p, _p, _p],
    "scail_conv3d_cl_resid_norm": [_p, _p, _p, _p, _p, _i64, _p, _i64, _p, _p, _p],
    "scail_rms_silu": [_p, _p, _p, _i64, _i64, _i, _p],
    "scail_softmax_rows": [_p, _i64, _i64, _i64, _f, _p],
    "scail_transpose2d": [_p, _i64, _i64, _p, _i64, _i64, _i64, _i64, _i64, _p],
    "scail_to_channels_last": [_p, _p, _p, _p, _i64, _i64, _i64, _p],
    "scail_from_channels_last": [_p, _i64, _p, _p, _p, _i64, _i64, _f, _f, _p],
    "scail_to_channels_last_frames": [_p, _p, _p, _p, _i64, _i64, _i64, _i64, _i64, _p],
    "scail_from_channels_last_frames": [_p, _i64, _p, _p, _p, _i64, _i64, _i64, _i64, _f, _f, _p],
    "scail_frames_u8": [_p, _i64, _p, _i64, _i64, _i64, _i64, _i64, _p],
    "scail_attn_small": [_p, _p, _p, _p, _p, _i64, _i64, _i64, _i64, _i64, _f, _p, _p, _p, _i64, _p],
    "scail_mul_bf16": [_p, _p, _p, _i64, _p],
    "scail_row_affine": [_p, _p, _p, _p, _i64, _i64, _i64, _p],
    "scail_set_option": [C.c_char_p, _i],
    "scail_release_caches": [],
    "scail_f32_to_bf16": [_p, _p, _i64, _p],
    "scail_bf16_to_f32": [_p, _p, _i64, _p],
    "scail_quant_fp8_rows": [_p, _i64, _p, _i64, _p, _i64, _i64, _p],
    "scail_gemm_fp8": [_p, _i64, _p, _p, _p, _p, _p, _i64, _i64, _i64, _i64, _i, _p, _i64, _p, _i64, _i64, _p],
    "scail_rel_err_rows": [_p, _i64, _p, _i64, _p, _i64, _i64, _p],
    "scail_resid_store": [_p, _i64, _p, _i64, _p, _i64, _i64, _i64, _p],
    "scail_resid_apply": [_p, _i64, _p, _p, _i64, _i64, _i64, _i64, _p],
    "scail_abs_diff_sums": [_p, _p, _i64, _p, _p],
    "scail_quant_mxfp8_rows": [_p, _i64, _p, _i64, _p, _i64, _i64, _i64, _p],
    "scail_gemm_mxfp8": [_p, _i64, _p, _i64, _p, _p, _p, _p, _i64, _i64, _i64, _i64, _i, _p, _i64, _p, _i64, _i64, _p],
    "scail_resize_crop_aa": [_p, _i, _p, _i64, _i64, _i64, _i64, _i64, _i64, _i64, _i64, _i64, _i64, _p],
    "scail_pose_half": [_p, _p, _i64, _i64, _p, _i64, _i64, _i64, _i64, _p],
    "scail_dit_create": [_p, _p, _p],
    "scail_dit_destroy": [_p],
    "scail_dit_workspace_bytes": [_p, _i64, _i64, _i64, _i64],
    "scail_dit_step": [_p, _p, _p, _p, _p, _i64, _p, _i64, _p, _p, _p, _i64, _i64, _i64, _i64, C.c_uint32, _p, _i64, _p],
    "scail_dit_chars_workspace_bytes": [_p, _i64, _i64, _i64, _i64, _i64],
    "scail_dit_step_chars": [_p, _p, _p, _p, _p, _i64, _p, _i64, _i64, _i64, _p, _p, _p, _i64, _i64, _i64, _i64, C.c_uint32, _p, _i64, _p],
    "scail_dit_sp_chars_workspace_bytes": [_p, C.c_int32, C.c_int32, _i64, _i64, _i64, _i64, _i64],
    "scail_dit_step_sp_chars": [_p, _p, _p, _p, _p, _i64, _p, _i64, _i64, _i64, _p, _p, _p, _i64, _i64, _i64, _i64, _p, C.c_uint32, _p, _i64, _p],
    "scail_dit_sample_chars_workspace_bytes": [_p, _i64, _i64, _i64, _i64],
    "scail_dit_sample_chars": [_p, _p, _p, _p, _i64, _f, _p, _p, _p, _i64, _i64, _p, _p, _i64, _i64, _i64, _p, _i64, _p],
    "scail_dit_profile": [_p, _i],
    "scail_dit_profile_read": [_p, _i, _p, _p],
    "scail_dit_block_workspace_bytes": [_p, _i64, _i64],
    "scail_dit_block": [_p, _i64, _p, _p, _p, _p, _p, _i64, _i64, _p, _i64, _p],
    "scail_dit_sp_workspace_bytes": [_p, C.c_int32, C.c_int32, _i64, _i64, _i64, _i64],
    "scail_dit_step_sp": [_p, _p, _p, _p, _p, _i64, _p, _i64, _p, _p, _p, _i64, _i64, _i64, _i64, _p, C.c_uint32, _p, _i64, _p],
    "scail_dit_block_sp_workspace_bytes": [_p, C.c_int32, C.c_int32, _i64, _i64],
    "scail_dit_block_sp": [_p, _i64, _p, _p, _p, _p, _p, _i64, _i64, _p, _p, _i64, _p],
    "scail_dit_sample_workspace_bytes": [_p, _i64, _i64, _i64],
    "scail_dit_sample": [_p, _p, _p, _p, _i64, _f, _p, _p, _p, _p, _p, _i64, _i64, _i64, _p, _i64, _p],
    "scail_dit_sample_tiled_workspace_bytes": [_p, _i64, _i64, _i64, _i64],
    "scail_dit_sample_tiled": [_p, _p, _p, _p, _i64, _f, _p, _p, _p, _p, _p, _p, _i64, _i64, _i64, _p, _p, _i64, _i64, _p, _i64, _p],
    "scail_dit_fp8_weight_bytes": [_p, C.c_uint32],
    "scail_dit_enable_fp8": [_p, C.c_uint32, _p, _i64, _p],
    "scail_dit_fp8_weight_bytes_scaled": [_p, C.c_uint32, _i],
    "scail_dit_enable_fp8_scaled": [_p, C.c_uint32, _i, _p, _i64, _p],
    "scail_dit_fp8_select_layers": [_p, _p],
    "scail_dit_fp8_probe_bytes": [_p, _i64, _i64],
    "scail_dit_fp8_probe": [_p, _p, _p, _i64],
    "scail_dit_step_cache_bytes": [_p, _i64, _i64, _i64, _i64],
    "scail_dit_step_cached": [_p, _p, _p, _p, _p, _i64, _p, _i64, _i64, _i64, _p, _p, _p, _i64, _i64, _i64, _i64, C.c_uint32, _p, _i64,
                              _i, _p, _i64, _p],
    "scail_dit_sample_cached": [_p, _p, _p, _p, _i64, _f, _p, _p, _p, _i64, _i64, _p, _p, _i64, _i64, _i64, _p, _i64, _p, _p, _i64, _p],
    "scail_dit_time_distances_bytes": [_p, _i],
    "scail_dit_time_distances": [_p, _p, _i64, _i, _p, _p, _i64, _p],
    "scail_vae_create": [_p, _p],
    "scail_vae_destroy": [_p],
    "scail_vae_set_trace": [_p, _p, _p],
    "scail_vae_workspace_bytes": [_p, _i64, _i64, _i64],
    "scail_vae_encode": [_p, _p, _p, _i64, _i64, _i64, _p, _i64, _p],
    "scail_vae_decode": [_p, _p, _p, _i64, _i64, _i64, _p, _i64, _p],
    "scail_vae_decode_stream_workspace_bytes": [_p, _i64, _i64, _i64],
    "scail_vae_decode_stream": [_p, _p, _p, _i64, _i64, _i64, _i64, _p, _i64, _p],
    "scail_vae_decode_u8": [_p, _p, _p, _i64, _i64, _i64, _p, _i64, _p],
    "scail_vae_decode_stream_u8": [_p, _p, _p, _i64, _i64, _i64, _i64, _p, _i64, _p],
}
RESTYPES = {"scail_dit_destroy": None, "scail_vae_destroy": None, "scail_dit_fp8_weight_bytes_scaled": _i64,
            **{n: _i64 for n in SIGNATURES if n.endswith("_bytes")}}

ABLATION_SIGNATURES = {
    "scail_tune_set": [C.c_char_p, _i],
    "scail_debug_cycles": [C.c_void_p, _i],
}
ABLATIONS = LIB_PATH.endswith("_abl.so")

EPI_BIAS, EPI_GELU_TANH, EPI_GELU_ERF, EPI_RESID = 0, 1, 2, 3
ACT_NONE, ACT_SILU, ACT_GELU_TANH = 0, 1, 2
ROW_LN_MODULATE, ROW_LN_AFFINE, ROW_RMSNORM, ROW_RMSNORM_ROPE, ROW_COPY = 0, 1, 2, 3, 4
FP8_GEMMS = {"qkv": 1, "o": 2, "cq": 4, "co": 8, "w1": 16, "w2": 32}
FP8_ALL = 63
FP8_SCALINGS = {"row": 0, "mx": 1}
CACHE_MODES = {"fill": 1, "reuse": 2}
CACHE_SIGNALS = {"time": 0, "modulation": 1}
SRC_U8_NHWC, SRC_F32_NCHW = 0, 1
RESIZE_MAX_SCALE = 16
ABI_VERSION = 8

_lib = None


class ScailHipError(RuntimeError):
    pass


def load() -> C.CDLL:
    global _lib
    if _lib is not None:
        return _lib
    if not os.path.exists(LIB_PATH):
        raise ScailHipError(
            f"{LIB_PATH} not found: build it with `python -m scail_amd.build` (hipcc, gfx950). "
            "scail_amd has no CPU/torch fallback.")
    lib = C.CDLL(LIB_PATH)
    lib.scail_last_error.restype = C.c_char_p
    lib.scail_last_error.argtypes = []
# ... 37 lines not shown
```

### scail_amd/ops.py

```python
from __future__ import annotations

import math
from typing import Optional

import torch

from . import lib as L

bf16 = torch.bfloat16
f32 = torch.float32


def _stream() -> int:
    return torch.cuda.current_stream().cuda_stream


def _chk(t: torch.Tensor, dtype, name: str):
    if not t.is_cuda:
        raise L.ScailHipError(f"{name}: tensor must be on the GPU (scail_amd has no CPU path)")
    if t.dtype != dtype:
        raise L.ScailHipError(f"{name}: expected {dtype}, got {t.dtype}")


def _ptr(t: Optional[torch.Tensor]) -> Optional[int]:
# ... 235 lines not shown
    else:
        rows_per_batch = rows if rows_per_batch is None else rows_per_batch
    L.call("scail_rmsnorm_rope_scaled", x.data_ptr(), ldx, out.data_ptr(), ldy, w.data_ptr(), _ptr(cos), _ptr(sin), rows,
           rows_per_batch, D, head_dim, eps, float(out_scale), _stream())
    return out


def rmsnorm_rope_slabs(x, w, out, cos=None, sin=None, rows_per_batch=None, head_dim=128, eps=1e-6, out_scale=1.0):
    _chk(x, bf16, "rmsnorm_rope_slabs.x"); _chk(out, bf16, "rmsnorm_rope_slabs.out")
    rows, D, ldx = _rowmajor2d(x, "rmsnorm_rope_slabs.x")
    if out.dim() != 3 or out.stride(2) != 1 or out.shape[1] != rows or out.shape[0] * out.shape[2] != D:
        raise L.ScailHipError(f"rmsnorm_rope_slabs.out must be a (n_slabs, {rows}, {D} / n_slabs) tensor with a contiguous last dim, got {tuple(out.shape)}")
    if w is not None:
        _chk(w, f32, "w")
    if cos is not None:
        _chk(cos, f32, "cos"); _chk(sin, f32, "sin")
        assert cos.is_contiguous() and sin.is_contiguous() and cos.shape[1] == head_dim // 2
        rows_per_batch = cos.shape[0] if rows_per_batch is None else rows_per_batch
    else:
        rows_per_batch = rows if rows_per_batch is None else rows_per_batch
    L.call("scail_rmsnorm_rope_slabs", x.data_ptr(), ldx, out.data_ptr(), out.shape[2], out.stride(1), out.stride(0), _ptr(w), _ptr(cos),
           _ptr(sin), rows, rows_per_batch, D, head_dim, eps, float(out_scale), _stream())
    return out


def transpose_v(v, heads, head_dim=128, out=None):
    _chk(v, bf16, "transpose_v.v")
    B, Lk, D = v.shape
    assert D == heads * head_dim and v.stride(2) == 1
    Lkp = (Lk + 63) // 64 * 64
    if out is None:
        out = torch.empty(B, heads, head_dim, Lkp, device=v.device, dtype=bf16)
    assert out.is_contiguous() and out.shape == (B, heads, head_dim, Lkp)
    L.call("scail_transpose_v", v.data_ptr(), v.stride(1), v.stride(0), out.data_ptr(), B, heads, head_dim, Lk,
           _stream())
    return out


def flash_attn(q, k, vt, out=None, scale=None, accumulate=False, n_seg=1, k_seg_stride=0, vt_seg_stride=0,
               k_broadcast=False, q_prescaled=False):
    _chk(q, bf16, "flash_attn.q"); _chk(k, bf16, "k"); _chk(vt, bf16, "vt")
    B, Lq, D = q.shape
    H = D // 128
    assert D == H * 128 and q.stride(2) == 1 and k.stride(2) == 1
    Lk = k.shape[1]
    Lkp = (Lk + 63) // 64 * 64
    assert vt.shape[-1] == Lkp and vt.shape[-2] == 128 and vt.shape[-3] == H, (vt.shape, Lkp, H)
    assert vt[0].is_contiguous()
    if out is None:
        out = torch.empty(B, Lq, D, device=q.device, dtype=bf16)
    _chk(out, bf16, "flash_attn.out")
    assert out.stride(2) == 1
    k_bs = 0 if (k_broadcast or k.shape[0] == 1) else k.stride(0)
    vt_bs = 0 if (k_broadcast or vt.shape[0] == 1) else vt.stride(0)
    if scale is None:
        scale = 1.0 / math.sqrt(128)
    if q_prescaled:
        scale = ATTN_Q_PRESCALED
    L.call("scail_flash_attn_bf16", q.data_ptr(), q.stride(0), q.stride(1), k.data_ptr(), k_seg_stride, k_bs,
           k.stride(1), vt.data_ptr(), vt_seg_stride, vt_bs, out.data_ptr(), out.stride(0), out.stride(1), B, H, Lq,
           Lk, n_seg, scale, 1 if accumulate else 0, _stream())
    return out


def flash_attn_vrows(q, k, v, out=None, scale=None, q_prescaled=False):
    _chk(q, bf16, "flash_attn_vrows.q"); _chk(k, bf16, "k"); _chk(v, bf16, "v")
    B, Lq, D = q.shape
    H = D // 128
    assert D == H * 128 and q.stride(2) == 1 and k.stride(2) == 1 and v.stride(2) == 1 and v.shape == k.shape
    if out is None:
        out = torch.empty(B, Lq, D, device=q.device, dtype=bf16)
    _chk(out, bf16, "flash_attn_vrows.out")
    assert out.stride(2) == 1
    if scale is None:
        scale = 1.0 / math.sqrt(128)
    if q_prescaled:
        scale = ATTN_Q_PRESCALED
    L.call("scail_flash_attn_vrows_bf16", q.data_ptr(), q.stride(0), q.stride(1), k.data_ptr(), 0 if k.shape[0] == 1 else k.stride(0), k.stride(1),
           v.data_ptr(), 0 if v.shape[0] == 1 else v.stride(0), v.stride(1), out.data_ptr(), out.stride(0), out.stride(1), B, H, Lq, k.shape[1], scale,
           _stream())
    return out


def cross_attn2(q, k1, vt1, k2, vt2, out=None, scale=None, q_prescaled=False):
    _chk(q, bf16, "cross_attn2.q")
    B, Lq, D = q.shape
    H = D // 128
    assert D == H * 128 and q.stride(2) == 1
    if out is None:
        out = torch.empty(B, Lq, D, device=q.device, dtype=bf16)
    _chk(out, bf16, "cross_attn2.out")
    assert out.stride(2) == 1 and out.shape == (B, Lq, D)
    sets = []
    for k, vt in ((k1, vt1), (k2, vt2)):
        _chk(k, bf16, "cross_attn2.k"); _chk(vt, bf16, "cross_attn2.vt")
        Lk = k.shape[1]
        assert k.shape[0] in (1, B) and vt.shape[0] == k.shape[0] and k.shape[2] == D and k.stride(2) == 1
        assert vt.shape[1:] == (H, 128, (Lk + 63) // 64 * 64) and vt[0].is_contiguous(), (vt.shape, Lk)
        sets += [k.data_ptr(), 0 if k.shape[0] == 1 else k.stride(0), k.stride(1), vt.data_ptr(), 0 if vt.shape[0] == 1 else vt.stride(0), Lk]
    if scale is None:
        scale = 1.0 / math.sqrt(128)
    if q_prescaled:
        scale = ATTN_Q_PRESCALED
    L.call("scail_cross_attn2_bf16", q.data_ptr(), q.stride(0), q.stride(1), *sets, out.data_ptr(), out.stride(0), out.stride(1),
           B, H, Lq, scale, _stream())
    return out


def timestep_embedding(t, dim):
    _chk(t, f32, "timestep_embedding.t")
    out = torch.empty(t.shape[0], dim, device=t.device, dtype=f32)
    L.call("scail_timestep_embedding", t.data_ptr(), out.data_ptr(), t.shape[0], dim, _stream())
    return out


def small_linear(x, w, b=None, act_in=L.ACT_NONE, act_out=L.ACT_NONE):
    _chk(x, f32, "small_linear.x"); _chk(w, bf16, "small_linear.w")
    assert x.is_contiguous() and w.is_contiguous()
    M, K = x.shape
    N = w.shape[0]
    y = torch.empty(M, N, device=x.device, dtype=f32)
    L.call("scail_small_linear", x.data_ptr(), w.data_ptr(), _ptr(b), y.data_ptr(), M, N, K, act_in, act_out,
           _stream())
    return y


def adaln_table(emb, table):
    _chk(emb, f32, "adaln_table.emb"); _chk(table, f32, "adaln_table.table")
    assert emb.is_contiguous() and table.is_contiguous()
    out = torch.empty(table.shape[0], emb.shape[0], emb.shape[1], device=emb.device, dtype=f32)
    L.call("scail_adaln_table", emb.data_ptr(), table.data_ptr(), out.data_ptr(), table.shape[0], emb.shape[0],
           emb.shape[1], _stream())
    return out


def patchify(x, ref, pose, kpad=128, out=None, n_char=1):
    _chk(x, f32, "patchify.x"); _chk(ref, bf16, "patchify.ref"); _chk(pose, bf16, "patchify.pose")
    assert x.is_contiguous() and ref.is_contiguous() and pose.is_contiguous()
    B, T, C, H, W = x.shape
    assert C == 16 and ref.shape[1:] == (n_char, 16, H, W) and pose.shape[1:] == (n_char * T, 16, H // 2, W // 2)
    Ltok = (n_char + T) * (H // 2) * (W // 2) + n_char * T * (H // 4) * (W // 4)
    if out is None:
        out = torch.empty(B, Ltok, kpad, device=x.device, dtype=bf16)
    assert out.is_contiguous() and out.shape == (B, Ltok, kpad)
    if n_char == 1:
        L.call("scail_patchify", x.data_ptr(), ref.data_ptr(), pose.data_ptr(), out.data_ptr(), B, ref.shape[0],
               pose.shape[0], T, H, W, kpad, _stream())
    else:
        L.call("scail_patchify_chars", x.data_ptr(), ref.data_ptr(), pose.data_ptr(), out.data_ptr(), B, ref.shape[0],
               pose.shape[0], n_char, T, H, W, kpad, _stream())
    return out


def unpatchify(tok, T, H, W, out=None):
    _chk(tok, bf16, "unpatchify.tok")
    assert tok.is_contiguous() and tok.shape[-1] == 64
    B = tok.shape[0]
    if out is None:
        out = torch.empty(B, T, 16, H, W, device=tok.device, dtype=f32)
    L.call("scail_unpatchify", tok.data_ptr(), out.data_ptr(), B, T, H, W, _stream())
    return out


def cfg_euler_(x, v, cfg_scale, dsigma):
    _chk(x, f32, "cfg_euler.x"); _chk(v, f32, "cfg_euler.v")
    assert x.is_contiguous() and v.is_contiguous() and v.numel() == 2 * x.numel()
    L.call("scail_cfg_euler", x.data_ptr(), v.data_ptr(), x.numel(), float(cfg_scale), float(dsigma), _stream())
    return x


def _tile_frames(frames):
    import ctypes as C
    fr = [int(f) for f in frames]
    return (C.c_int32 * len(fr))(*fr), len(fr)


def _host_f32(vals):
    import ctypes as C
    vals = vals.detach().cpu().float().tolist() if torch.is_tensor(vals) else [float(v) for v in vals]
    return (C.c_float * len(vals))(*vals), len(vals)


def tile_gather(x, frames, out=None):
    _chk(x, f32, "tile_gather.x")
    assert x.is_contiguous() and x.shape[0] == 1
    fr, Tt = _tile_frames(frames)
# ... 290 lines not shown
```

Baseline: 9067.

## Collapse repeated trailing text keys in cross-attention into log-weighted keys

Adds a detection kernel that finds the run of trailing text keys and values identical to the last key, such as padding. It also adds a templated cross-attention variant that handles that run differently. Each run of c duplicate keys becomes popcount(c) keys, with log2 weights added to their scores. This stays exact under softmax and cuts the number of text key tiles the kernel visits. In exchange there is an extra detection pass per step, or a cached one in the Python path, plus some per-tile branch work in the score loop.

Measured after the change: 9122, median of 6. Within noise of the previous version (+0.6%).

```diff
diff --git a/include/scail_dit.h b/include/scail_dit.h
--- a/include/scail_dit.h
+++ b/include/scail_dit.h
@@ -55,6 +55,8 @@
 
 int scail_dit_create(const scail_dit_config* cfg, const scail_dit_weights* w, scail_dit** out);
 void scail_dit_destroy(scail_dit* h);
+
+int scail_dit_tail_info(const scail_dit* h, int32_t* out, int64_t n_pairs, void* stream);
 
 int64_t scail_dit_workspace_bytes(const scail_dit* h, int64_t B, int64_t T, int64_t H, int64_t W);
 
diff --git a/include/scail_hip.h b/include/scail_hip.h
--- a/include/scail_hip.h
+++ b/include/scail_hip.h
@@ -103,6 +103,16 @@
                            scail_bf16* o, int64_t o_bs, int64_t o_rs,
                            int64_t n_batch, int64_t heads, int64_t Lq, float scale, void* stream);
 
+int scail_key_tail_runs(const scail_bf16* k, int64_t k_bs, int64_t k_rs, const scail_bf16* vt, int64_t vt_bs, int64_t Lk,
+                        int64_t heads, int64_t n, int32_t* info, void* stream);
+int scail_cross_attn2_tail_for(int64_t q_rs, int64_t k1_rs, int64_t k2_rs, int64_t o_rs, int64_t Lq, int64_t Lk1, int64_t Lk2,
+                               int64_t n_batch, int64_t heads);
+int scail_cross_attn2_tail_bf16(const scail_bf16* q, int64_t q_bs, int64_t q_rs,
+                                const scail_bf16* k1, int64_t k1_bs, int64_t k1_rs, const scail_bf16* vt1, int64_t vt1_bs, int64_t Lk1,
+                                const scail_bf16* k2, int64_t k2_bs, int64_t k2_rs, const scail_bf16* vt2, int64_t vt2_bs, int64_t Lk2,
+                                scail_bf16* o, int64_t o_bs, int64_t o_rs,
+                                int64_t n_batch, int64_t heads, int64_t Lq, float scale, const int32_t* tail_info, void* stream);
+
 int scail_timestep_embedding(const float* t, float* out, int64_t n, int64_t dim, void* stream);
 
 int scail_small_linear(const float* x, const scail_bf16* w, const float* b, float* y, int64_t M,
diff --git a/scail_amd/csrc/attn.hip b/scail_amd/csrc/attn.hip
--- a/scail_amd/csrc/attn.hip
+++ b/scail_amd/csrc/attn.hip
@@ -1,6 +1,7 @@
 #include <algorithm>
 #include <atomic>
 #include <cstring>
+#include <type_traits>
 #include "common.h"
 
 #define HD 128
@@ -283,9 +284,14 @@
     float sl2;
 };
 
+struct Cross2TailParams : Cross2Params {
+    const int* info;
+};
+
 #define X2_THREADS 256
 #define X2_LDS_BYTES (2 * (KVBLK * HD + HD * KVBLK) * 2)
-__global__ __launch_bounds__(X2_THREADS, 2) void cross_attn2_kernel(Cross2Params p) {
+template <bool TAIL>
+__global__ __launch_bounds__(X2_THREADS, 2) void cross_attn2_kernel(typename std::conditional<TAIL, Cross2TailParams, Cross2Params>::type p) {
     extern __shared__ __attribute__((aligned(16))) u16 smem[];
     u16* Ks = smem;
     u16* Vs = smem + 2 * KVBLK * HD;
@@ -310,14 +316,24 @@
     const u16* kb1 = p.k1 + b * p.k1_bs + (int64_t)h * HD;
     const u16* vb0 = p.vt0 + b * p.vt0_bs + (int64_t)h * HD * p.Lkp0;
     const u16* vb1 = p.vt1 + b * p.vt1_bs + (int64_t)h * HD * p.Lkp1;
-    const int n0 = p.Lkp0 / KVBLK, n1 = p.Lkp1 / KVBLK, ntiles = n0 + n1;
+    int Lk0 = p.Lk0, run_c = 1, run0 = 0, npc = 0;
+    if constexpr (TAIL) {
+        const int ne = __builtin_amdgcn_readfirstlane(p.info[2 * b]), c = __builtin_amdgcn_readfirstlane(p.info[2 * b + 1]);
+        if (c >= 1 && c <= p.Lk0 && ne == p.Lk0 - c + __builtin_popcount((unsigned)c)) {
+            Lk0 = ne;
+            run_c = c;
+        }
+        npc = __builtin_popcount((unsigned)run_c);
+        run0 = p.Lk0 - run_c;
+    }
+    const int n0 = TAIL ? (Lk0 + KVBLK - 1) / KVBLK : p.Lkp0 / KVBLK, n1 = p.Lkp1 / KVBLK, ntiles = n0 + n1;
 #define X2_ISSUE(tt_, buf_)                                                                                 \
     {                                                                                                       \
         const bool s1_ = (tt_) >= n0;                                                                       \
         const int key0_ = ((tt_) - (s1_ ? n0 : 0)) * KVBLK;                                                 \
         const u16* kp_ = s1_ ? kb1 : kb0;                                                                   \
         const int64_t krs_ = s1_ ? p.k1_rs : p.k0_rs;                                                       \
-        const int last_ = (s1_ ? p.Lk1 : p.Lk0) - 1;                                                        \
+        const int last_ = (s1_ ? p.Lk1 : Lk0) - 1;                                                          \
         const int lkp_ = s1_ ? p.Lkp1 : p.Lkp0;                                                             \
         const u16* vp_ = (s1_ ? vb1 : vb0) + key0_;                                                         \
         _Pragma("unroll") for (int i_ = 0; i_ < 4; ++i_) {                                                  \
@@ -384,7 +400,7 @@
         {
             const bool s1 = tt >= n0;
             const int t = tt - (s1 ? n0 : 0), ns = s1 ? n1 : n0;
-            const int tail = (s1 ? p.Lk1 : p.Lk0) - (ns - 1) * KVBLK;
+            const int tail = (s1 ? p.Lk1 : Lk0) - (ns - 1) * KVBLK;
             if (t == ns - 1 && tail < KVBLK) {
 #pragma unroll
                 for (int f = 0; f < 2; ++f)
@@ -401,6 +417,23 @@
 #pragma unroll
             for (int r = 0; r < 16; ++r) mx = fmaxf(mx, s[f][r]);
         mx = fmaxf(mx, __shfl_xor(mx, 32, 64));
+        if constexpr (TAIL) {
+            const int rel = run0 - tt * KVBLK;
+            if (tt < n0 && rel < KVBLK && rel + npc > 0) {
+                unsigned bits = (unsigned)run_c;
+                for (int i = 0; i < npc; ++i) {
+                    const float w = (float)__builtin_ctz(bits);
+                    bits &= bits - 1;
+#pragma unroll
+                    for (int f = 0; f < 2; ++f)
+#pragma unroll
+                        for (int r = 0; r < 16; ++r) {
+                            const int key = 32 * f + (r & 3) + 8 * (r >> 2) + 4 * g;
+                            if (key == rel + i) s[f][r] += w;
+                        }
+                }
+            }
+        }
         const float m_new = fmaxf(m_run, mx);
         const float alpha = __builtin_amdgcn_exp2f((m_run - m_new) * sl2);
         const float msc = m_new * sl2;
@@ -733,6 +766,7 @@
 static std::atomic<int> g_attn4_mode{1};
 static std::atomic<int> g_attn_vrows{1};
 static std::atomic<int> g_cross4{2};
+static std::atomic<int> g_cross_tail{1};
 constexpr int64_t k_cross4_min_tiles = 21;
 static std::atomic<int> g_attn4_rows{0};
 static std::atomic<int> g_attn4_cus{0};
@@ -967,6 +1001,7 @@
     const std::string k(name ? name : "");
     if (k == "attn4") { g_attn4_mode = value != 0; return 0; }
     if (k == "attn_vrows") { g_attn_vrows = value != 0; return 0; }
+    if (k == "cross_tail") { g_cross_tail = value != 0; return 0; }
     if (k == "cross4") {
         SCAIL_REQUIRE(value >= 0 && value <= 2, "cross4 must be 0, 1 or 2");
         g_cross4 = value;
@@ -1185,11 +1220,24 @@
     return 0;
 }
 
-extern "C" int scail_cross_attn2_bf16(const scail_bf16* q, int64_t q_bs, int64_t q_rs,
-                                      const scail_bf16* k1, int64_t k1_bs, int64_t k1_rs, const scail_bf16* vt1, int64_t vt1_bs, int64_t Lk1,
-                                      const scail_bf16* k2, int64_t k2_bs, int64_t k2_rs, const scail_bf16* vt2, int64_t vt2_bs, int64_t Lk2,
-                                      scail_bf16* o, int64_t o_bs, int64_t o_rs,
-                                      int64_t n_batch, int64_t heads, int64_t Lq, float scale, void* stream) {
+static bool cross_tail_shape(int64_t q_rs, int64_t k1_rs, int64_t k2_rs, int64_t o_rs, int64_t Lq, int64_t Lk1, int64_t Lk2, int64_t n_batch,
+                             int64_t heads) {
+    if (Lk1 < 1 || Lk2 < 1 || Lk1 >= (1ll << 30) || Lk2 >= (1ll << 30)) return false;
+    return (Lk1 + 63) / 64 + (Lk2 + 63) / 64 < k_cross4_min_tiles && !cross_choose(q_rs, k1_rs, k2_rs, o_rs, Lq, Lk1, Lk2, n_batch, heads, false).generated;
+}
+int scail_cross_tail_wanted(int64_t Lk1, int64_t Lk2) {
+    return g_cross_tail != 0 && Lk1 >= 1 && Lk2 >= 1 && (Lk1 + 63) / 64 + (Lk2 + 63) / 64 < k_cross4_min_tiles;
+}
+extern "C" int scail_cross_attn2_tail_for(int64_t q_rs, int64_t k1_rs, int64_t k2_rs, int64_t o_rs, int64_t Lq, int64_t Lk1, int64_t Lk2,
+                                          int64_t n_batch, int64_t heads) {
+    return g_cross_tail != 0 && cross_tail_shape(q_rs, k1_rs, k2_rs, o_rs, Lq, Lk1, Lk2, n_batch, heads) ? 1 : 0;
+}
+
+static int cross_attn2_impl(const scail_bf16* q, int64_t q_bs, int64_t q_rs,
+                            const scail_bf16* k1, int64_t k1_bs, int64_t k1_rs, const scail_bf16* vt1, int64_t vt1_bs, int64_t Lk1,
+                            const scail_bf16* k2, int64_t k2_bs, int64_t k2_rs, const scail_bf16* vt2, int64_t vt2_bs, int64_t Lk2,
+                            scail_bf16* o, int64_t o_bs, int64_t o_rs,
+                            int64_t n_batch, int64_t heads, int64_t Lq, float scale, const int32_t* tail_info, void* stream) {
     SCAIL_REQUIRE(Lk1 >= 1 && Lk2 >= 1 && Lk1 < (1ll << 30) && Lk2 < (1ll << 30), "cross_attn2: each key set needs at least one key");
     SCAIL_REQUIRE(heads >= 1 && heads < 65536 && n_batch < 65536 && Lq < (1ll << 31) - 256, "cross_attn2: grid limits");
     SCAIL_REQUIRE(q_rs % 8 == 0 && k1_rs % 8 == 0 && k2_rs % 8 == 0 && o_rs % 4 == 0 && q_bs % 8 == 0 && k1_bs % 8 == 0 && k2_bs % 8 == 0 &&
@@ -1201,6 +1249,13 @@
     if (n_batch == 0 || Lq == 0) return 0;
     const bool prescaled = scale == SCAIL_ATTN_Q_PRESCALED;
     SCAIL_REQUIRE(prescaled || (scale > 0.0f && scale < 3.0e38f), "cross_attn2: scale must be a positive finite number or SCAIL_ATTN_Q_PRESCALED");
+    if (tail_info != nullptr) {
+        SCAIL_REQUIRE(prescaled, "cross_attn2_tail: the key weights are added to scores in log2 units: scale must be SCAIL_ATTN_Q_PRESCALED");
+        SCAIL_REQUIRE((reinterpret_cast<uintptr_t>(tail_info) & 3) == 0, "cross_attn2_tail: the run info must be 4-byte aligned");
+        SCAIL_REQUIRE(cross_tail_shape(q_rs, k1_rs, k2_rs, o_rs, Lq, Lk1, Lk2, n_batch, heads),
+                      "cross_attn2_tail: 21 or more key tiles, or a shape of the generated kernel: this call takes all keys (scail_cross_attn2_bf16; "
+                      "scail_cross_attn2_tail_for)");
+    }
     const CrossChoice c = cross_choose(q_rs, k1_rs, k2_rs, o_rs, Lq, Lk1, Lk2, n_batch, heads, true);
     if (c.generated) {
         hipFunction_t fn;
@@ -1224,5 +1279,30 @@
     p.heads = (int)heads; p.Lq = (int)Lq;
     p.sl2 = prescaled ? 1.0f : scale * 1.44269504088896340736f;
     const dim3 grid((unsigned)((Lq + 127) / 128), (unsigned)heads, (unsigned)n_batch);
-    return scail_launch_lds<cross_attn2_kernel>("cross_attn2", X2_LDS_BYTES, grid, dim3(X2_THREADS), X2_LDS_BYTES, stream, p);
-}
+    if (tail_info != nullptr) {
+        Cross2TailParams pt;
+        static_cast<Cross2Params&>(pt) = p;
+        pt.info = tail_info;
+        return scail_launch_lds<cross_attn2_kernel<true>>("cross_attn2_tail", X2_LDS_BYTES, grid, dim3(X2_THREADS), X2_LDS_BYTES, stream, pt);
+    }
+    return scail_launch_lds<cross_attn2_kernel<false>>("cross_attn2", X2_LDS_BYTES, grid, dim3(X2_THREADS), X2_LDS_BYTES, stream, p);
+}
+
+extern "C" int scail_cross_attn2_bf16(const scail_bf16* q, int64_t q_bs, int64_t q_rs,
+                                      const scail_bf16* k1, int64_t k1_bs, int64_t k1_rs, const scail_bf16* vt1, int64_t vt1_bs, int64_t Lk1,
+                                      const scail_bf16* k2, int64_t k2_bs, int64_t k2_rs, const scail_bf16* vt2, int64_t vt2_bs, int64_t Lk2,
+                                      scail_bf16* o, int64_t o_bs, int64_t o_rs,
+                                      int64_t n_batch, int64_t heads, int64_t Lq, float scale, void* stream) {
+    return cross_attn2_impl(q, q_bs, q_rs, k1, k1_bs, k1_rs, vt1, vt1_bs, Lk1, k2, k2_bs, k2_rs, vt2, vt2_bs, Lk2, o, o_bs, o_rs, n_batch, heads, Lq,
+                            scale, nullptr, stream);
+}
+
+extern "C" int scail_cross_attn2_tail_bf16(const scail_bf16* q, int64_t q_bs, int64_t q_rs,
+                                           const scail_bf16* k1, int64_t k1_bs, int64_t k1_rs, const scail_bf16* vt1, int64_t vt1_bs, int64_t Lk1,
+                                           const scail_bf16* k2, int64_t k2_bs, int64_t k2_rs, const scail_bf16* vt2, int64_t vt2_bs, int64_t Lk2,
+                                           scail_bf16* o, int64_t o_bs, int64_t o_rs,
+                                           int64_t n_batch, int64_t heads, int64_t Lq, float scale, const int32_t* tail_info, void* stream) {
+    SCAIL_REQUIRE(tail_info != nullptr, "cross_attn2_tail: null run info (scail_key_tail_runs)");
+    return cross_attn2_impl(q, q_bs, q_rs, k1, k1_bs, k1_rs, vt1, vt1_bs, Lk1, k2, k2_bs, k2_rs, vt2, vt2_bs, Lk2, o, o_bs, o_rs, n_batch, heads, Lq,
+                            scale, tail_info, stream);
+}
diff --git a/scail_amd/csrc/dit_step.hip b/scail_amd/csrc/dit_step.hip
--- a/scail_amd/csrc/dit_step.hip
+++ b/scail_amd/csrc/dit_step.hip
@@ -7,6 +7,7 @@
 int scail_attn4_preload();
 void scail_attn4_rows_hint(int rows);
 int scail_gemm4_preload();
+int scail_cross_tail_wanted(int64_t Lk1, int64_t Lk2);
 #include "../../include/scail_dit.h"
 
 constexpr int PROF_CATS = 5;
@@ -31,7 +32,10 @@
     double* probe_table = nullptr;
     scail_bf16 *probe_y16 = nullptr, *probe_y8 = nullptr;
     int64_t probe_rows = 0;
+    int32_t* tail_info = nullptr;
+    bool tail_on = false;
 };
+constexpr int64_t TAIL_MAX_B = 8;
 
 namespace {
 
@@ -297,6 +301,15 @@
     DIT_PROF(SCAIL_DIT_PROF_GEMM, dit_gemm(h, i, G_O, bf, att, D, lw.o_b, hid, D, nb * rpb, D, D, SCAIL_EPI_RESID, hid, D, m + 2 * D, 6 * D, rpb, stream));
     return 0;
 }
+static int tail_detect(scail_dit* h, const scail_dit_cond* cond, int64_t B, int64_t layer0, int64_t n_layers, void* stream) {
+    h->tail_on = false;
+    if (h->tail_info == nullptr || B > TAIL_MAX_B || cond->Lt < 1 || cond->Lc < 1 || !scail_cross_tail_wanted(cond->Lt, cond->Lc)) return 0;
+    const int64_t D = h->cfg.hidden_size, nh = h->cfg.num_heads, Ltp = (cond->Lt + 63) / 64 * 64;
+    DIT_TRY(scail_key_tail_runs(cond->k_text + layer0 * B * cond->Lt * D, cond->Lt * D, D, cond->vt_text + layer0 * B * nh * 128 * Ltp, nh * 128 * Ltp,
+                                cond->Lt, nh, n_layers * B, h->tail_info + layer0 * B * 2, stream));
+    h->tail_on = true;
+    return 0;
+}
 static int block_cross_mlp(scail_dit* h, int64_t i, scail_bf16* hid, scail_bf16* att, scail_bf16* q3, scail_bf16* xn, scail_bf16* ff,
                            const float* m, const scail_dit_cond* cond, int64_t Btot, int64_t b0, int64_t nb, int64_t rpb, const BlockBufs& bf,
                            void* stream) {
@@ -314,9 +327,16 @@
     const scail_bf16* vtt = cond->vt_text + (i * Btot + b0) * nh * 128 * Ltp;
     const scail_bf16* kc = cond->k_clip + (i * cond->Bc + (shared_clip ? 0 : b0)) * cond->Lc * D;
     const scail_bf16* vtc = cond->vt_clip + (i * cond->Bc + (shared_clip ? 0 : b0)) * nh * 128 * Lcp;
-    DIT_PROF(SCAIL_DIT_PROF_CROSS_ATTN, scail_cross_attn2_bf16(q3, rpb * 3 * D, 3 * D, kt, cond->Lt * D, D, vtt, nh * 128 * Ltp, cond->Lt,
-                                                               kc, shared_clip ? 0 : cond->Lc * D, D, vtc, shared_clip ? 0 : nh * 128 * Lcp, cond->Lc,
-                                                               att, rpb * D, D, nb, nh, rpb, SCAIL_ATTN_Q_PRESCALED, stream));
+    if (h->tail_on && scail_cross_attn2_tail_for(3 * D, D, D, D, rpb, cond->Lt, cond->Lc, nb, nh)) {
+        DIT_PROF(SCAIL_DIT_PROF_CROSS_ATTN, scail_cross_attn2_tail_bf16(q3, rpb * 3 * D, 3 * D, kt, cond->Lt * D, D, vtt, nh * 128 * Ltp, cond->Lt,
+                                                                        kc, shared_clip ? 0 : cond->Lc * D, D, vtc, shared_clip ? 0 : nh * 128 * Lcp, cond->Lc,
+                                                                        att, rpb * D, D, nb, nh, rpb, SCAIL_ATTN_Q_PRESCALED,
+                                                                        h->tail_info + (i * Btot + b0) * 2, stream));
+    } else {
+        DIT_PROF(SCAIL_DIT_PROF_CROSS_ATTN, scail_cross_attn2_bf16(q3, rpb * 3 * D, 3 * D, kt, cond->Lt * D, D, vtt, nh * 128 * Ltp, cond->Lt,
+                                                                   kc, shared_clip ? 0 : cond->Lc * D, D, vtc, shared_clip ? 0 : nh * 128 * Lcp, cond->Lc,
+                                                                   att, rpb * D, D, nb, nh, rpb, SCAIL_ATTN_Q_PRESCALED, stream));
+    }
     DIT_PROF(SCAIL_DIT_PROF_GEMM, dit_gemm(h, i, G_CO, bf, att, D, lw.co_b, hid, D, M, D, D, SCAIL_EPI_RESID, hid, D, nullptr, 0, 0, stream));
     DIT_TRY(scail_ln_modulate(hid, D, xn, D, m + 3 * D, m + 4 * D, 6 * D, nb, rpb, rpb, 0, D, eps, stream));
     DIT_PROF(SCAIL_DIT_PROF_GEMM, dit_gemm(h, i, G_W1, bf, xn, D, lw.b1, ff, FF, M, FF, D, SCAIL_EPI_GELU_TANH, nullptr, 0, nullptr, 0, 0, stream));
@@ -535,6 +555,7 @@
     const BlockWs s = block_ws(h, B, Ltok, sp->mode, sp->ranks);
     SCAIL_REQUIRE(workspace != nullptr && workspace_bytes >= s.end && (reinterpret_cast<uintptr_t>(workspace) & 255) == 0,
                   "workspace too small or not 256-byte aligned (scail_dit_block_sp_workspace_bytes)");
+    DIT_TRY(tail_detect(h, cond, B, layer, 1, stream));
     return dit_block_sp(h, layer, hidden, mod, cond, rope_cos, rope_sin, B, Ltok, s.bufs(workspace), sp, 0, Ltok, false, stream);
 }
 extern "C" int scail_dit_block(scail_dit* h, int64_t layer, scail_bf16* hidden, const float* mod, const scail_dit_cond* cond,
@@ -546,6 +567,7 @@
     SCAIL_REQUIRE(workspace != nullptr && workspace_bytes >= s.end && (reinterpret_cast<uintptr_t>(workspace) & 255) == 0,
                   "workspace too small or not 256-byte aligned (scail_dit_block_workspace_bytes)");
     DIT_TRY(probe_check(h, B * Ltok));
+    DIT_TRY(tail_detect(h, cond, B, layer, 1, stream));
     return dit_block(h, layer, hidden, mod, cond, rope_cos, rope_sin, B, Ltok, s.bufs(workspace), 0, Ltok, false, stream);
 }
 
@@ -563,6 +585,13 @@
     if (int rc = scail_gemm4_preload()) { delete h; return rc; }
     h->layers.assign(w->layers, w->layers + cfg->num_layers);
     h->w.layers = h->layers.data();
+    const size_t tail_bytes = (size_t)cfg->num_layers * TAIL_MAX_B * 2 * sizeof(int32_t);
+    if (hipMalloc(&h->tail_info, tail_bytes) != hipSuccess || hipMemset(h->tail_info, 0, tail_bytes) != hipSuccess) {
+        scail_set_error("scail_dit_create: no device memory for the key-run info (" + std::to_string(tail_bytes) + " bytes)");
+        if (h->tail_info != nullptr) (void)hipFree(h->tail_info);
+        delete h;
+        return 2;
+    }
     *out = h;
     return 0;
 }
@@ -574,8 +603,22 @@
         for (hipEvent_t e : h->sp_ev)
             if (e != nullptr) (void)hipEventDestroy(e);
         if (h->restart_ctr != nullptr) (void)hipFree(h->restart_ctr);
+        if (h->tail_info != nullptr) (void)hipFree(h->tail_info);
     }
     delete h;
+}
+
+extern "C" int scail_dit_tail_info(const scail_dit* h, int32_t* out, int64_t n_pairs, void* stream) {
+    SCAIL_REQUIRE(h != nullptr && out != nullptr, "null argument");
+    SCAIL_REQUIRE(n_pairs >= 0 && n_pairs <= h->cfg.num_layers * TAIL_MAX_B, "scail_dit_tail_info: the handle keeps layers * 8 pairs");
+    const size_t bytes = (size_t)n_pairs * 2 * sizeof(int32_t);
+    const hipError_t e = h->tail_on ? hipMemcpyAsync(out, h->tail_info, bytes, hipMemcpyDeviceToDevice, (hipStream_t)stream)
+                                    : hipMemsetAsync(out, 0, bytes, (hipStream_t)stream);
+    if (e != hipSuccess) {
+        scail_set_error("scail_dit_tail_info: the copy failed");
+        return 2;
+    }
+    return 0;
 }
 
 static int64_t fp8_scale_bytes(int scaling, int64_t N, int64_t K) { return scaling == SCAIL_DIT_FP8_SCALE_MX ? N * (K / 32) : N * 4; }
@@ -791,6 +834,7 @@
     SCAIL_REQUIRE(workspace != nullptr && workspace_bytes >= s.total, "workspace too small (scail_dit_workspace_bytes)");
     SCAIL_REQUIRE((reinterpret_cast<uintptr_t>(workspace) & 255) == 0, "workspace must be 256-byte aligned");
     if (sp == nullptr && !reuse) DIT_TRY(probe_check(h, B * tok_lens(n_char, T, H, W).Ltok));
+    if (!reuse) DIT_TRY(tail_detect(h, cond, B, 0, h->cfg.num_layers, stream));
 
     const int64_t D = c.hidden_size, nl = c.num_layers;
     const float eps = c.layernorm_epsilon;
diff --git a/scail_amd/csrc/rowops.hip b/scail_amd/csrc/rowops.hip
--- a/scail_amd/csrc/rowops.hip
+++ b/scail_amd/csrc/rowops.hip
@@ -1076,6 +1076,66 @@
     return scail_check_launch("abs_diff_sums");
 }
 
+#define KTR_THREADS 1024
+__device__ __forceinline__ int ktr_col(int j) { return (j & ~12) | (((j >> 3) & 1) << 2) | (((j >> 2) & 1) << 3); }
+__global__ __launch_bounds__(KTR_THREADS) void key_tail_runs_kernel(const u16* __restrict__ k, int64_t k_bs, int64_t k_rs,
+                                                                    const u16* __restrict__ vt, int64_t vt_bs, int Lk, int Lkp, int D,
+                                                                    int* __restrict__ info) {
+    __shared__ int sm[KTR_THREADS];
+    const int t = threadIdx.x;
+    const u16* kb = k + (int64_t)blockIdx.x * k_bs;
+    const u16* vb = vt + (int64_t)blockIdx.x * vt_bs;
+    const u16* kl = kb + (int64_t)(Lk - 1) * k_rs;
+    int hi = -1;
+    const int cpr = D >> 3;
+    for (int64_t i = t; i < (int64_t)(Lk - 1) * cpr; i += KTR_THREADS) {
+        const int j = (int)(i / cpr), cc = (int)(i - (int64_t)j * cpr);
+        const uint4 a = *reinterpret_cast<const uint4*>(kb + (int64_t)j * k_rs + cc * 8);
+        const uint4 r = *reinterpret_cast<const uint4*>(kl + cc * 8);
+        if (a.x != r.x || a.y != r.y || a.z != r.z || a.w != r.w) hi = max(hi, j);
+    }
+    const int cpv = Lkp >> 3;
+    for (int64_t i = t; i < (int64_t)D * cpv; i += KTR_THREADS) {
+        const int64_t row = i / cpv;
+        const int cc = (int)(i - row * cpv);
+        if ((cc * 8 & ~15) >= Lk - 1) continue;
+        const u16 ref = vb[row * Lkp + ktr_col(Lk - 1)];
+        const uint4 a = *reinterpret_cast<const uint4*>(vb + row * Lkp + cc * 8);
+        const uint32_t w[4] = {a.x, a.y, a.z, a.w};
+#pragma unroll
+        for (int e = 0; e < 8; ++e) {
+            const u16 v = (u16)(w[e >> 1] >> (16 * (e & 1)));
+            const int j = ktr_col(cc * 8 + e);
+            if (j < Lk - 1 && v != ref) hi = max(hi, j);
+        }
+    }
+    sm[t] = hi;
+    __syncthreads();
+    for (int s = KTR_THREADS / 2; s > 0; s >>= 1) {
+        if (t < s) sm[t] = max(sm[t], sm[t + s]);
+        __syncthreads();
+    }
+    if (t == 0) {
+        const int c = Lk - 1 - sm[0];
+        info[2 * blockIdx.x] = Lk - c + __popc((unsigned)c);
+        info[2 * blockIdx.x + 1] = c;
+    }
+}
+
+extern "C" int scail_key_tail_runs(const scail_bf16* k, int64_t k_bs, int64_t k_rs, const scail_bf16* vt, int64_t vt_bs, int64_t Lk,
+                                   int64_t heads, int64_t n, int32_t* info, void* stream) {
+    SCAIL_REQUIRE(Lk >= 1 && Lk < (1ll << 30) && heads >= 1 && heads < 65536 && n >= 0 && n < (1ll << 31), "key_tail_runs: bad key / head / element count");
+    if (n == 0) return 0;
+    SCAIL_REQUIRE(k != nullptr && vt != nullptr && info != nullptr, "key_tail_runs: null pointer");
+    const int64_t D = heads * 128, Lkp = (Lk + 63) / 64 * 64;
+    SCAIL_REQUIRE(k_rs >= D && k_rs % 8 == 0 && k_bs >= 0 && k_bs % 8 == 0 && vt_bs >= 0 && vt_bs % 8 == 0,
+                  "key_tail_runs: k_rs must cover heads * 128 columns; strides must keep 16-byte alignment");
+    SCAIL_REQUIRE(aligned16(k) && aligned16(vt) && (reinterpret_cast<uintptr_t>(info) & 3) == 0, "key_tail_runs: pointer alignment");
+    hipLaunchKernelGGL(key_tail_runs_kernel, dim3((unsigned)n), dim3(KTR_THREADS), 0, (hipStream_t)stream, k, k_bs, k_rs, vt, vt_bs, (int)Lk, (int)Lkp,
+                       (int)D, info);
+    return scail_check_launch("key_tail_runs");
+}
+
 #define SA_ROWS 32
 __global__ __launch_bounds__(256) void attn_small_kernel(
     const u16* __restrict__ q, const u16* __restrict__ k, const u16* __restrict__ v, u16* __restrict__ o,
diff --git a/scail_amd/cstep.py b/scail_amd/cstep.py
--- a/scail_amd/cstep.py
+++ b/scail_amd/cstep.py
@@ -148,6 +148,12 @@
         L.call("scail_dit_profile_read", self._h, category, C.byref(ms), C.byref(n))
         return ms.value, n.value
 
+    def tail_info(self, n: int, device):
+        out = torch.empty(n, 2, dtype=torch.int32, device=device)
+        L.call("scail_dit_tail_info", self._h, out.data_ptr(), n, torch.cuda.current_stream(device).cuda_stream)
+        out = out.cpu()
+        return out if bool((out[:, 1] > 0).all()) else None
+
     def _ws_for(self, need: int, device, what: str) -> torch.Tensor:
         if need < 0:
             raise L.ScailHipError(f"{what}: the executor has no workspace for this request (bad shape / mode)")
diff --git a/scail_amd/dit.py b/scail_amd/dit.py
--- a/scail_amd/dit.py
+++ b/scail_amd/dit.py
@@ -597,6 +597,8 @@
 
         xn, qkv, att, ff, vt = ws["xn"], ws["qkv"], ws["att"], ws["ff"], ws["vt"]
         q, k, v = (None, None, None) if use_c else (qkv[..., :D], qkv[..., D:2 * D], qkv[..., 2 * D:])
+        if not use_c and "tail_info" not in cond:
+            cond["tail_info"] = ops.key_tail_runs(cond["k_text"], cond["vt_text"])
         for i, lw in enumerate(W["layers"]):
             m = mod[i]
             if use_c:
@@ -621,7 +623,8 @@
             cq = qkv[..., :D]
             ops.gemm(xn, lw["cq_w"], lw["cq_b"], out=cq)
             ops.rmsnorm_rope(cq, lw["cqn"], eps=eps, out_scale=ops.ATTN_LOG2_SCALE)
-            ops.cross_attn2(cq, cond["k_text"][i], cond["vt_text"][i], cond["k_clip"][i], cond["vt_clip"][i], out=att, q_prescaled=True)
+            ops.cross_attn2(cq, cond["k_text"][i], cond["vt_text"][i], cond["k_clip"][i], cond["vt_clip"][i], out=att, q_prescaled=True,
+                            tail_info=cond["tail_info"][i])
             ops.gemm(att, lw["co_w"], lw["co_b"], out=h, epilogue=L.EPI_RESID, resid=h)
             ops.ln_modulate(h, sh_m, sc_m, out=xn, eps=eps)
             ops.gemm(xn, lw["w1"], lw["b1"], out=ff, epilogue=L.EPI_GELU_TANH)
diff --git a/scail_amd/lib.py b/scail_amd/lib.py
--- a/scail_amd/lib.py
+++ b/scail_amd/lib.py
@@ -40,6 +40,10 @@
     "scail_conv3d_kernel_name_for": [_p, _i64, _i64, _i, _p, _i64],
     "scail_cross_attn2_bf16": [_p, _i64, _i64, _p, _i64, _i64, _p, _i64, _i64, _p, _i64, _i64, _p, _i64, _i64, _p, _i64, _i64,
                                _i64, _i64, _i64, _f, _p],
+    "scail_cross_attn2_tail_bf16": [_p, _i64, _i64, _p, _i64, _i64, _p, _i64, _i64, _p, _i64, _i64, _p, _i64, _i64, _p, _i64, _i64,
+                                    _i64, _i64, _i64, _f, _p, _p],
+    "scail_cross_attn2_tail_for": [_i64, _i64, _i64, _i64, _i64, _i64, _i64, _i64, _i64],
+    "scail_key_tail_runs": [_p, _i64, _i64, _p, _i64, _i64, _i64, _i64, _p, _p],
     "scail_timestep_embedding": [_p, _p, _i64, _i64, _p],
     "scail_small_linear": [_p, _p, _p, _p, _i64, _i64, _i64, _i, _i, _p],
     "scail_adaln_table": [_p, _p, _p, _i64, _i64, _i64, _p],
@@ -80,6 +84,7 @@
     "scail_pose_half": [_p, _p, _i64, _i64, _p, _i64, _i64, _i64, _i64, _p],
     "scail_dit_create": [_p, _p, _p],
     "scail_dit_destroy": [_p],
+    "scail_dit_tail_info": [_p, _p, _i64, _p],
     "scail_dit_workspace_bytes": [_p, _i64, _i64, _i64, _i64],
     "scail_dit_step": [_p, _p, _p, _p, _p, _i64, _p, _i64, _p, _p, _p, _i64, _i64, _i64, _i64, C.c_uint32, _p, _i64, _p],
     "scail_dit_chars_workspace_bytes": [_p, _i64, _i64, _i64, _i64, _i64],
diff --git a/scail_amd/ops.py b/scail_amd/ops.py
--- a/scail_amd/ops.py
+++ b/scail_amd/ops.py
@@ -341,7 +341,21 @@
     return out
 
 
-def cross_attn2(q, k1, vt1, k2, vt2, out=None, scale=None, q_prescaled=False):
+def key_tail_runs(k, vt, out=None):
+    _chk(k, bf16, "key_tail_runs.k"); _chk(vt, bf16, "key_tail_runs.vt")
+    Lk, D = k.shape[-2:]
+    H = D // 128
+    lead = k.shape[:-2]
+    assert D == H * 128 and k.is_contiguous() and vt.is_contiguous() and vt.shape == (*lead, H, 128, (Lk + 63) // 64 * 64), (k.shape, vt.shape)
+    n = math.prod(lead)
+    if out is None:
+        out = torch.empty(*lead, 2, device=k.device, dtype=torch.int32)
+    assert out.dtype == torch.int32 and out.is_contiguous() and out.shape == (*lead, 2) and out.is_cuda
+    L.call("scail_key_tail_runs", k.data_ptr(), Lk * D, D, vt.data_ptr(), D * vt.shape[-1], Lk, H, n, out.data_ptr(), _stream())
+    return out
+
+
+def cross_attn2(q, k1, vt1, k2, vt2, out=None, scale=None, q_prescaled=False, tail_info=None):
     _chk(q, bf16, "cross_attn2.q")
     B, Lq, D = q.shape
     H = D // 128
@@ -361,6 +375,12 @@
         scale = 1.0 / math.sqrt(128)
     if q_prescaled:
         scale = ATTN_Q_PRESCALED
+    if tail_info is not None and q_prescaled and k1.shape[0] == B and L.load().scail_cross_attn2_tail_for(
+            q.stride(1), k1.stride(1), k2.stride(1), out.stride(1), Lq, k1.shape[1], k2.shape[1], B, H):
+        assert tail_info.dtype == torch.int32 and tail_info.shape == (B, 2) and tail_info.is_contiguous() and tail_info.is_cuda
+        L.call("scail_cross_attn2_tail_bf16", q.data_ptr(), q.stride(0), q.stride(1), *sets, out.data_ptr(), out.stride(0), out.stride(1),
+               B, H, Lq, scale, tail_info.data_ptr(), _stream())
+        return out
     L.call("scail_cross_attn2_bf16", q.data_ptr(), q.stride(0), q.stride(1), *sets, out.data_ptr(), out.stride(0), out.stride(1),
            B, H, Lq, scale, _stream())
     return out
```
